# viscom-ulm/MCCNN

Hardware: AMD Instinct MI355X
Metric: MC-convolved points/sec (fwd+bwd), 100k-pt cloud r=0.1 (higher is better)
Workload: dtype f32; 1 GPU; ScanNet-like non-uniform room, 100000 pts/room, 1 room(s) on rank 0, absolute radius 0.1, KDE window 0.2, same-level conv 1to64 (Fin=1, Fout=64, combin), avg on; points_total=100000, points_per_gpu=100000, edges_per_gpu=4543198, layer=1to64, parallelism=cloud-per-GPU dp1, headline_mode=pipelined, rccl_world_size=1, collectives_warmed_before_warmup=False

## Files before the change

include/mccnn.h:

```cpp
#ifndef MCCNN_H_
#define MCCNN_H_

#include <stddef.h>

#ifdef __cplusplus
extern "C" {
#endif

typedef void* mccnn_stream_t;

#define MCCNN_OK 0
#define MCCNN_E_BADARG (-1)
#define MCCNN_E_BATCHID (-2)
#define MCCNN_E_TOOLARGE (-3)
#define MCCNN_E_WORKSPACE (-4)
#define MCCNN_E_SHAPE (-5)

int mccnn_block_size(void);
int mccnn_abi_version(void);
const char* mccnn_arch(void);
const char* mccnn_error_string(int code);

int mccnn_check_batch_ids(const int* batch_ids, int n, int batch_size, int* bad_count_dev,
                          mccnn_stream_t stream);
// ... 183 lines not shown
                        int avg, const int* order, void* rec_edges, int rec_ready, int* start_t, int* perm_t,
                        int tlist_ready, void* plan_buffer, void* ws, size_t ws_bytes, mccnn_stream_t stream);

int mccnn_spatial_conv_fwd_rows(const float* sorted_pts, const void* sorted_feats,
                                const int* sorted_batch_ids, const float* pdfs, const float* samples,
                                const int* start_idx, const int* packed, const float* aabb_min,
                                const float* aabb_max, const float* w1, const float* b1, const float* w2,
                                const float* b2, const float* w3, const float* b3, int n, int m, int e,
                                int num_feats, int batch_size, float radius, int scale_inv, int avg,
                                int bf16, const int* plan_vrow, const int* plan_vcode,
                                const int* slice_off, const int* vpos_row, const void* plan_rec,
                                const int* plan_other, void* out, float* scratch, const int* feat_index,
                                mccnn_stream_t stream);
size_t mccnn_spatial_conv_bwd_rows_workspace_bytes(int n, int e, int num_feats);
int mccnn_spatial_conv_bwd_rows(const float* sorted_pts, const void* sorted_feats,
                                const int* sorted_batch_ids, const float* pdfs, const float* samples,
                                const int* start_idx, const int* packed, const float* aabb_min,
                                const float* aabb_max, const float* w1, const float* b1, const float* w2,
                                const float* b2, const float* w3, const float* b3, const void* out_grad,
                                int n, int m, int e, int num_feats, int batch_size, float radius,
                                int scale_inv, int avg, int bf16, const int* start_t,
                                const int* plan_vrow, const int* plan_vcode, const int* slice_off,
                                const int* vpos_row, const void* plan_rec, const int* plan_other,
                                void* feat_grad, float* scratch, float* dw1, float* db1, float* dw2,
                                float* db2, float* dw3, float* db3, const int* feat_index, void* ws,
                                size_t ws_bytes, mccnn_stream_t stream);

#define MCCNN_E_CAPACITY (-6)
typedef struct mccnn_geometry mccnn_geometry_t;
mccnn_geometry_t* mccnn_geometry_create(void);
void mccnn_geometry_destroy(mccnn_geometry_t* g);
size_t mccnn_geometry_bytes(int n, int m, int batch_size, int num_cells, int e_capacity, int with_grid);
int mccnn_geometry_build(mccnn_geometry_t* g, const float* pts, const int* batch_ids, int n, const float* centres,
                         const int* centre_batch_ids, int m, const float* aabb_min, const float* aabb_max,
                         int batch_size, int num_cells, float radius, int scale_inv, float window, int use_pdf,
                         int e_capacity, const mccnn_geometry_t* grid_from, void* buffer, size_t buffer_bytes,
                         int* total_host, mccnn_stream_t stream);

typedef struct mccnn_geometry_request {
    mccnn_geometry_t* geometry;
    const float* pts; const int* batch_ids; int n;
    const float* centres; const int* centre_batch_ids; int m;
    const float* aabb_min; const float* aabb_max;
    int batch_size, num_cells;
    float radius; int scale_inv; float window; int use_pdf; int e_capacity;
    const mccnn_geometry_t* grid_from;
    void* buffer; size_t buffer_bytes;
    int* total_host;
} mccnn_geometry_request;
int mccnn_geometry_build_batch(const mccnn_geometry_request* requests, int count, mccnn_stream_t stream);
int mccnn_geometry_edges(mccnn_geometry_t* g, int wait_us);
int mccnn_geometry_info(const mccnn_geometry_t* g, long long out[16]);
int mccnn_geometry_attach(mccnn_geometry_t* g, int what, void* buffer, size_t bytes);
int mccnn_geometry_piece_bytes(mccnn_geometry_t* g, int what, long long* bytes, long long* ws_bytes);
int mccnn_geometry_piece_bound(int n, int m, int e_cap, int what, long long* bytes, long long* ws_bytes);
int mccnn_geometry_prebuild(mccnn_geometry_t* g, int what, int avg, void* ws, size_t ws_bytes, mccnn_stream_t stream);

size_t mccnn_geometry_prebuild_batch_ws_bytes(mccnn_geometry_t* const* geoms, const int* what, int count);
int mccnn_geometry_prebuild_batch(mccnn_geometry_t* const* geoms, const int* what, int count, int avg, void* ws, size_t ws_bytes,
                                  mccnn_stream_t stream);
int mccnn_conv_prepare(mccnn_geometry_t* g, const void* feats, int num_in_feats, int num_out_feats, int combin, int bf16,
                       int backward, int flags, int* need_mask, long long need_bytes[4], long long* ws_bytes,
                       long long* saved_bytes, int* edges);
int mccnn_conv_forward(mccnn_geometry_t* g, const void* feats, int num_in_feats, int num_out_feats, int combin, int avg,
                       int bf16, int flags, const float* w1, const float* b1, const float* w2, const float* b2,
                       const float* w3, const float* b3, void* out, void* saved, size_t saved_bytes, void* ws,
                       size_t ws_bytes, mccnn_stream_t stream);
int mccnn_conv_backward(mccnn_geometry_t* g, const void* feats, const void* saved, size_t saved_bytes,
                        const void* out_grad, int num_in_feats, int num_out_feats, int combin, int avg, int bf16,
                        int flags, const float* w1, const float* b1, const float* w2, const float* b2, const float* w3,
                        const float* b3, void* feat_grad, float* dw1, float* db1, float* dw2, float* db2, float* dw3,
                        float* db3, void* ws, size_t ws_bytes, mccnn_stream_t stream);

int mccnn_debug_conv_impl(int mask);

long long mccnn_debug_launch_count(void);
long long mccnn_debug_wait_ns(void);
int mccnn_debug_wait_accounting(int on);
int mccnn_background_launches(int on);
int mccnn_debug_f1_x4_min_edges(int edges);
int mccnn_debug_small_kernels(int on);

#ifdef __cplusplus
}
#endif
#endif
```

mccnn_amd/MCConvBuilder.py:

```python
import math

import os
import sys
import time
import torch

from . import _env


_NATIVE = None
_HIPOPS = None


def _native_mod():
    global _NATIVE
    if _NATIVE is None:
        from . import native
        _NATIVE = native
    return _NATIVE


def _hip_ops_mod():
    global _HIPOPS
    if _HIPOPS is None:
# ... 281 lines not shown
            self.register_parameter(name, p)
        elif tuple(p.shape) != tuple(shape):
            raise RuntimeError("variable %s exists with shape %s, requested %s" % (name, tuple(p.shape), shape))
        return p

    def forward(self, *args, **kwargs):
        return self.create_convolution(*args, **kwargs)

    def _add_to_collection(self, name, p):
        lst = self.collections_.setdefault(name, [])
        seen = self.__dict__.setdefault("_collection_ids", {}).setdefault(name, set())
        if id(p) not in seen:
            seen.add(id(p))
            lst.append(p)

    def __compute_dic_keys__(self, inPointHierarchy, outPointHierarchy, inPointLevel, outPointLevel, convRadius,
                             KDEWindow, relativeRadius, usePDF):
        memo = self.__dict__.setdefault("_keyMemo", {})
        k = (inPointHierarchy.hierarchyName_, outPointHierarchy.hierarchyName_, inPointLevel, outPointLevel, convRadius, KDEWindow,
             relativeRadius, usePDF)
        try:
            hit = memo.get(k)
        except TypeError:
            hit, k = None, None
        if hit is not None:
            return hit
        keyGrid = inPointHierarchy.hierarchyName_ + '|' + str(inPointLevel) + '|' + str(convRadius) + '|' + \
            str(relativeRadius)
        keyNeighs = keyGrid + '|' + outPointHierarchy.hierarchyName_ + '|' + str(outPointLevel)
        keyPDF = keyNeighs + '|' + str(KDEWindow) + '|' + str(usePDF)
        if k is not None and len(memo) < 4096:
            memo[k] = (keyGrid, keyNeighs, keyPDF)
        return keyGrid, keyNeighs, keyPDF

    def reset(self):
        state = self.__dict__
        k = state.get("hostStepsAhead_", None)
        if k is not None and _cuda_ok():
            evs = state.setdefault("stepEvents_", [])
            evs.append(_record_event())
            del evs[:-8]
            if len(evs) > k:
                _M = _hip_ops_mod()
                t0 = time.perf_counter()
                evs[-(int(k) + 1)].synchronize()
                dt = time.perf_counter() - t0
                _M.HOST_WAIT_S[0] += dt
                _M.HOST_LAG_WAIT_S[0] += dt
        state["cacheGrids_"], state["cacheNeighs_"], state["cachePDFs_"] = {}, {}, {}
        if self.geoSeen_:
            plan = []
            for key, ent in self.geoSeen_.items():
                geo = self.cacheGeo_.get(key)
                plan.append(ent + ((geo.have & 7) if geo is not None else 0, key))
            state["geoPlan_"], state["geoSeen_"] = plan, {}
        state["cacheGeo_"], state["cacheGeoGrid_"] = {}, {}
        if self.prefetchedGeo_:
            self.__install_prefetched_geometries__()
        pf, state["prefetched_"] = self.prefetched_, None
        if pf is not None:
            grids, neighs, pdfs, event = pf
            main = torch.cuda.current_stream()
            main.wait_event(event)
            for kN, h in list(neighs.items()):
                if hasattr(h, "finalize"):
                    st, pk, pdf = h.finalize()
                    neighs[kN] = (st, pk)
                    pdfs[h.keyPDF] = pdf
            for d in (grids, neighs, pdfs):
                for v in d.values():
                    for t in (v if isinstance(v, tuple) else (v,)):
                        t.record_stream(main)
            self.cacheGrids_, self.cacheNeighs_, self.cachePDFs_ = grids, neighs, pdfs
        state["resetEvent_"] = _record_event() if (_SIDE_EVENTS[0] and _cuda_ok()) else None
        if pf is not None:
            for kN, (kG, kP, centres, mn, mx, B, radius, rel) in self.prefetchTransposed_.items():
                if kN in neighs and kG in grids and getattr(self.ops_, "_ops", 0) is None:
                    _hip_ops = _hip_ops_mod()
                    self.sideStream_.wait_event(self.resetEvent_)
                    g = grids[kG]
                    _hip_ops.prefetch_transposed(neighs[kN][1], g[0].shape[0], self.sideStream_)
                    if kP in pdfs:
                        _hip_ops.prefetch_rowplan(neighs[kN][1], True, self.sideStream_, g[0], g[1], pdfs[kP], centres,
                                                  neighs[kN][0], neighs[kN][1], mn, mx, g[0].shape[0], centres.shape[0],
                                                  neighs[kN][1].shape[0], B, radius, rel, self.useAVG_)
            self.prefetchTransposed_ = {}

    def prefetch_geometry(self, inPointHierarchy, inPointLevel, convRadius, outPointHierarchy=None, outPointLevel=None,
                          KDEWindow=None, relativeRadius=None, usePDF=None, transposed=False):
        currKDEWindow = self.KDEWindow_ if KDEWindow is None else KDEWindow
        currRelativeRadius = self.relativeRadius_ if relativeRadius is None else relativeRadius
        currUsePDF = self.usePDF_ if usePDF is None else usePDF
        outPH = inPointHierarchy if outPointHierarchy is None else outPointHierarchy
        outLevel = inPointLevel if outPointLevel is None else outPointLevel
        keyGrid, keyNeighs, keyPDF = self.__compute_dic_keys__(inPointHierarchy, outPH, inPointLevel, outLevel, convRadius,
                                                               currKDEWindow, currRelativeRadius, currUsePDF)
        pts, bids = inPointHierarchy.points_[inPointLevel], inPointHierarchy.batchIds_[inPointLevel]
        mn, mx, B = inPointHierarchy.aabbMin_, inPointHierarchy.aabbMax_, inPointHierarchy.batchSize_
        if not pts.is_cuda:
            return
        if self.__prefetch_native__(inPointHierarchy, inPointLevel, convRadius, outPH, outLevel, currKDEWindow,
                                    currRelativeRadius, currUsePDF, keyGrid, keyNeighs, keyPDF, transposed):
            return
        if self.sideStream_ is None:
            self.sideStream_ = torch.cuda.Stream(device=pts.device)
        _SIDE_EVENTS[0] = True
        pf = self.prefetched_
# ... 67 lines not shown
            event.record(side)
        self.prefetched_ = (grids, neighs, pdfs, event)

    def _trace(self, *rec):
        if self.opTrace_ is not None:
            self.opTrace_.append(rec)

    def __layer_variables__(self, convName, inNumFeatures, currNumOutFeatures, currMultiFeatureConv, dev):
        blockSize = self.ops_.get_block_size()
        numOutNeurons = inNumFeatures * currNumOutFeatures if currMultiFeatureConv else inNumFeatures
        numBlocks = int(numOutNeurons / blockSize)
        if numOutNeurons % blockSize != 0:
            numBlocks = numBlocks + 1
        zeros = lambda t: t.zero_()
        nn = blockSize * numBlocks
        weights = self._get_variable(convName + '_weights', (3, nn), dev, lambda t: _fan_avg_uniform_(t, 3, nn))
        self._add_to_collection(self.decayLossCollection_, weights)
        biases = self._get_variable(convName + '_biases', (nn,), dev, zeros)
        weights2v = self._get_variable(convName + '_weights2', (numBlocks, blockSize, blockSize), dev,
                                       lambda t: _fan_avg_uniform_(t, numBlocks * blockSize, numBlocks * blockSize))
        self._add_to_collection(self.decayLossCollection_, weights2v)
        biases2v = self._get_variable(convName + '_biases2', (numBlocks, blockSize), dev, zeros)
        weights3v = self._get_variable(convName + '_weights3', (numBlocks, blockSize, blockSize), dev,
                                       lambda t: _fan_avg_uniform_(t, numBlocks * blockSize, numBlocks * blockSize))
        self._add_to_collection(self.decayLossCollection_, weights3v)
        biases3v = self._get_variable(convName + '_biases3', (numBlocks, blockSize), dev, zeros)
        return weights, biases, weights2v, biases2v, weights3v, biases3v, nn

    def __prefetch_native__(self, inPH, inLevel, convRadius, outPH, outLevel, KDEWindow, relativeRadius, usePDF, keyGrid,
                            keyNeighs, keyPDF, transposed, fork=True, pieces=0):
        _native = _native_mod()
        _hip_ops = _hip_ops_mod()
        if not (self.native_ and self.fuseSort_ and getattr(self.ops_, "_ops", 0) is None and _native.side_streams_available()
                and int(_hip_ops.PDF_MODE) == 1 and self.prefetched_ is None
                and _env.debug("native_prefetch", True)):
            return False
        inPts, inBids = inPH.points_[inLevel], inPH.batchIds_[inLevel]
        centres, cBids = outPH.points_[outLevel], outPH.batchIds_[outLevel]
        if inPts.requires_grad or inPts.shape[0] == 0 or centres.shape[0] == 0:
            return False
        for t, dt in ((inPts, torch.float32), (centres, torch.float32), (inBids, torch.int32), (cBids, torch.int32)):
            if t.dtype != dt or not t.is_contiguous() or not t.is_cuda:
                return False
        want = 0 if not transposed else (1 if transposed == "list" else 2)
        if keyPDF in self.prefetchedGeo_:
            ent = self.prefetchedGeo_[keyPDF]
            self.prefetchedGeo_[keyPDF] = ent[:4] + (max(ent[4], want),)
            return True
        mn, mx, B = inPH.aabbMin_, inPH.aabbMax_, inPH.batchSize_
        nc = _hip_ops._num_cells(mn, mx, B, convRadius, relativeRadius)
        owners = self.__dict__.setdefault("prefetchedGridOwner_", {})
        owner = owners.get(keyGrid)
        k = len(self.prefetchedGeo_)
        geo = _native.build_geometry(inPts, inBids, centres, cBids, mn, mx, B, nc, convRadius, relativeRadius, KDEWindow,
                                     usePDF, owner, side=k, fork=fork, background=True,
                                     after=(inPH.prefetchFuture_ if inPH is outPH else None))
        geo.uses = 0
        if owner is None:
            owners[keyGrid] = geo
        if pieces:
            geo.prebuild_async(pieces, self.useAVG_)
        self.prefetchedGeo_[keyPDF] = (geo, keyGrid, keyNeighs, usePDF, want)
        return True

    def prefetch_step(self, pointHierarchy):
        started = 0
        name, levels = pointHierarchy.hierarchyName_, len(pointHierarchy.points_)
        pieces = _env.debug("plan_prefetch", True)
        _native = _native_mod()
        _native.begin_batch()
        try:
            started = self.__prefetch_step_entries__(pointHierarchy, name, levels, pieces)
        finally:
            _native.end_batch()
        return started

    def __prefetch_step_entries__(self, pointHierarchy, name, levels, pieces):
        started = 0
        for ent in self.geoPlan_:
            hname, inLevel, outLevel, radius, window, rel, usePDF, have = ent[:8]
            if hname != name or inLevel >= levels or outLevel >= levels:
                continue
            keyGrid, keyNeighs, keyPDF = self.__compute_dic_keys__(pointHierarchy, pointHierarchy, inLevel, outLevel, radius,
                                                                   window, rel, usePDF)
            if keyPDF in self.prefetchedGeo_:
                continue
            if self.__prefetch_native__(pointHierarchy, inLevel, radius, pointHierarchy, outLevel, window, rel, usePDF, keyGrid,
                                        keyNeighs, keyPDF, False, fork=(started == 0), pieces=(have if pieces else 0)):
                started += 1
        return started

    def __install_prefetched_geometries__(self):
        _native = _native_mod()
        parked, self.prefetchedGeo_ = self.prefetchedGeo_, {}
        self.__dict__["prefetchedGridOwner_"] = {}
        for keyPDF, (geo, keyGrid, keyNeighs, usePDF, transposed) in parked.items():
            geo.unverified = True
            self.cacheGeo_[keyPDF] = geo
            if geo.grid_owner is None:
                self.cacheGeoGrid_[keyGrid] = geo
                self.cacheGrids_[keyGrid] = _LazyEntry(geo, geo.grid)
            self.cacheNeighs_[keyNeighs] = _LazyEntry(geo, geo.neighbors)
            self.cachePDFs_[keyPDF] = _LazyEntry(geo, geo.pdfs)
            if transposed:
                geo.prebuild((_native.NEED_PLAN_FWD | _native.NEED_PLAN_TR) if transposed == 2 else _native.NEED_TLIST,
                             self.useAVG_, 0, geo.buf)

    def __prebuild_geometries__(self, ph):
        _native = _native_mod()
        _hip_ops = _hip_ops_mod()
        plan, name = self.geoPlan_, ph.hierarchyName_
        levels = len(ph.points_)
        mn, mx, B = ph.aabbMin_, ph.aabbMax_, ph.batchSize_
        if int(_hip_ops.PDF_MODE) != 1:
            return
        k = 0
        pieces = _env.debug("plan_prefetch", True)
        for (hname, inLevel, outLevel, radius, window, rel, usePDF, have, _key) in plan:
            if hname != name or inLevel >= levels or outLevel >= levels:
                continue
            keyGrid, keyNeighs, keyPDF = self.__compute_dic_keys__(ph, ph, inLevel, outLevel, radius, window, rel, usePDF)
            if keyPDF in self.cacheGeo_:
                continue
            inPts, inBids = ph.points_[inLevel], ph.batchIds_[inLevel]
            centres, cBids = ph.points_[outLevel], ph.batchIds_[outLevel]
            if inPts.shape[0] == 0 or centres.shape[0] == 0 or inPts.requires_grad:
                continue
            ok = True
            for t, dt in ((inPts, torch.float32), (centres, torch.float32), (inBids, torch.int32), (cBids, torch.int32)):
                if t.dtype != dt or not t.is_contiguous() or not t.is_cuda:
                    ok = False
            if not ok:
                continue
            nc = _hip_ops._num_cells(mn, mx, B, radius, rel)
            owner = self.cacheGeoGrid_.get(keyGrid)
            geo = _native.build_geometry(inPts, inBids, centres, cBids, mn, mx, B, nc, radius, rel, window, usePDF, owner,
                                         side=k, fork=(k == 0), after=ph.prefetchFuture_)
            k += 1
            geo.uses = 0
            if have and pieces and geo.e_cap <= _PLAN_PREFETCH_MAX_E:
                geo.prebuild_async(have, self.useAVG_)
            self.cacheGeo_[keyPDF] = geo
            if owner is None:
                self.cacheGeoGrid_[keyGrid] = geo
                self.cacheGrids_[keyGrid] = _LazyEntry(geo, geo.grid)
                self._trace("sort_points_step1", keyGrid)
                self._trace("sort_points_step2", keyGrid)
            self.cacheNeighs_[keyNeighs] = _LazyEntry(geo, geo.neighbors)
            self.cachePDFs_[keyPDF] = _LazyEntry(geo, geo.pdfs)
            self._trace("find_neighbors", keyNeighs)
            if usePDF:
                self._trace("compute_pdf", keyPDF)

    def __native_convolution__(self, convName, inPH, inLevel, inFeatures, inNumFeatures, convRadius, outPH, outLevel,
                               multiFeatureConv, numOutFeatures, KDEWindow, relativeRadius, usePDF, useAVG, keyGrid,
                               keyNeighs, keyPDF):
        _native = _native_mod()
        _hip_ops = _hip_ops_mod()
        if (not self.cacheGeo_ and self.geoPrefetch_ and len(self.geoPlan_) >= _GEO_PREFETCH_MIN and inPH is outPH and self.prefetched_ is None
                and not self.cacheGrids_ and _native.side_streams_available()):
            self.__prebuild_geometries__(inPH)
        geo = self.cacheGeo_.get(keyPDF)
        if geo is not None and getattr(geo, "unverified", False):
            a = geo.args
            cen = outPH.points_[outLevel]
            pin = inPH.points_[inLevel]
            if (a[0] is pin or (a[0].data_ptr() == pin.data_ptr() and a[0].shape == pin.shape)) and \
                    (a[2] is cen or (a[2].data_ptr() == cen.data_ptr() and a[2].shape == cen.shape)):
                geo.unverified = False
            else:
                if _GEO_TRACE:
                    print("native conv %s: parked geometry %s not for this hierarchy (built from %s / %s, asked %s / %s)" % (
                        convName, keyPDF, tuple(a[0].shape), tuple(a[2].shape), tuple(pin.shape), tuple(cen.shape)), file=sys.stderr)
                self.cacheGeo_.pop(keyPDF, None)
                self.cachePDFs_.pop(keyPDF, None)
                self.cacheNeighs_.pop(keyNeighs, None)
                if self.cacheGeoGrid_.get(keyGrid) is geo:
                    self.cacheGeoGrid_.pop(keyGrid, None)
                    self.cacheGrids_.pop(keyGrid, None)
                geo = None
        if geo is None:
            if keyGrid in self.cacheGrids_ and keyGrid not in self.cacheGeoGrid_:
                if _GEO_TRACE:
                    print("native conv %s: grid %s owned by the op path" % (convName, keyGrid), file=sys.stderr)
                return None
            if keyNeighs in self.cacheNeighs_ or keyPDF in self.cachePDFs_:
                if _GEO_TRACE:
                    print("native conv %s: list %s / pdf %s cached without a geometry (%s %s); geometries: %s" % (
                        convName, keyNeighs, keyPDF, keyNeighs in self.cacheNeighs_, keyPDF in self.cachePDFs_,
                        sorted(self.cacheGeo_)), file=sys.stderr)
# ... 194 lines not shown
```

mccnn_amd/_lib.py:

```python
import ctypes as C
import os

import torch

_PKG = os.path.dirname(os.path.abspath(__file__))
LIB_PATH = os.path.join(_PKG, "lib", os.environ.get("MCCNN_LIB_NAME", "libmccnn_hip.so"))

_vp, _i, _f, _sz = C.c_void_p, C.c_int, C.c_float, C.c_size_t

SIGNATURES = {
    "mccnn_block_size": (_i, []),
    "mccnn_abi_version": (_i, []),
    "mccnn_arch": (C.c_char_p, []),
    "mccnn_error_string": (C.c_char_p, [_i]),
    "mccnn_check_batch_ids": (_i, [_vp, _i, _i, _vp, _vp]),
    "mccnn_debug_conv_impl": (_i, [_i]),
    "mccnn_debug_launch_count": (C.c_longlong, []),
    "mccnn_debug_wait_ns": (C.c_longlong, []),
    "mccnn_debug_wait_accounting": (_i, [_i]),
    "mccnn_debug_small_kernels": (_i, [_i]),
    "mccnn_debug_f1_x4_min_edges": (_i, [_i]),
    "mccnn_background_launches": (_i, [_i]),
    "mccnn_compute_aabb_workspace_bytes": (_sz, [_i]),
    "mccnn_compute_aabb": (_i, [_vp, _vp, _i, _i, _i, _vp, _vp, _vp, _sz, _vp]),
# ... 15 lines not shown
    "mccnn_transform_indexs_dn": (_i, [_vp, _i, _vp, _vp, _i, _vp, _vp, _vp, _sz, _vp]),
    "mccnn_permute_gather": (_i, [_vp, _vp, _i, _i, _vp, _vp]),
    "mccnn_permute_scatter": (_i, [_vp, _vp, _i, _i, _vp, _i, _i, _vp]),
    "mccnn_transform_indexs_workspace_bytes": (_sz, [_i]),
    "mccnn_transform_indexs": (_i, [_vp, _i, _vp, _i, _vp, _vp, _sz, _vp]),
    "mccnn_find_neighbors_workspace_bytes": (_sz, [_i, _i]),
    "mccnn_find_neighbors_count": (_i, [_vp, _vp, _i, _vp, _i, _vp, _vp, _vp, _i, _i, _f, _i, _vp, _vp, _vp, _vp, _sz, _vp]),
    "mccnn_find_neighbors_count2": (_i, [_vp, _vp, _i, _vp, _i, _vp, _vp, _vp, _i, _i, _f, _i, _vp, _vp, _vp, _vp, _vp, _sz, _vp]),
    "mccnn_find_neighbors_fill": (_i, [_vp, _vp, _i, _vp, _i, _vp, _vp, _vp, _i, _i, _f, _i, _vp, _vp, _i, _vp, _vp, _sz, _vp]),
    "mccnn_invert_permutation": (_i, [_vp, _i, _vp, _vp]),
    "mccnn_compute_pdf_workspace_bytes": (_sz, [_i, _i]),
    "mccnn_compute_pdf": (_i, [_vp, _vp, _vp, _i, _vp, _i, _vp, _vp, _i, _f, _f, _i, _i, _vp, _vp, _sz, _vp]),
    "mccnn_compute_pdf_dn": (_i, [_vp, _vp, _vp, _i, _vp, _i, _vp, _vp, _vp, _i, _f, _f, _i, _vp, _vp, _sz, _vp]),
    "mccnn_poisson_sampling_workspace_bytes": (_sz, [_i, _i, _i]),
    "mccnn_poisson_sampling_count": (_i, [_vp, _vp, _i, _vp, _vp, _vp, _i, _i, _f, _i, _i, _vp, _vp, _sz, _vp]),
    "mccnn_poisson_sampling_fill": (_i, [_vp, _i, _vp, _i, _i, _i, _vp, _vp, _vp, _vp, _sz, _vp]),
    "mccnn_spatial_conv_fwd_workspace_bytes": (_sz, [_i, _i, _i, _i, _i]),
    "mccnn_spatial_conv_state_bytes": (_sz, [_i, _i, _i, _i, _i]),
    "mccnn_spatial_conv_fwd": (_i, [_vp] * 15 + [_i, _i, _i, _i, _i, _i, _i, _f, _i, _i, _vp, _vp, _vp, _sz, _vp]),
    "mccnn_spatial_conv_bwd_workspace_bytes": (_sz, [_i, _i, _i, _i, _i, _i]),
    "mccnn_spatial_conv_bwd": (_i, [_vp] * 16 + [_i, _i, _i, _i, _i, _i, _i, _f, _i, _i] + [_vp] * 10 + [_vp, _sz, _vp]),
    "mccnn_spatial_conv_fwd_bf16": (_i, [_vp] * 15 + [_i, _i, _i, _i, _i, _f, _i, _i, _vp, _vp, _sz, _vp]),
    "mccnn_spatial_conv_bwd_bf16": (_i, [_vp] * 16 + [_i, _i, _i, _i, _i, _f, _i, _i] + [_vp] * 9 + [_vp, _sz, _vp]),
    "mccnn_rowplan_sizes": (_i, [_i, _i, C.POINTER(_i), C.POINTER(C.c_longlong), C.POINTER(C.c_longlong)]),
    "mccnn_rowplan_workspace_bytes": (_sz, [_i, _i]),
    "mccnn_rowplan_layout": (_i, [_vp, _i, _i, _vp, _vp, _vp, _vp, _vp, _vp, _sz, _vp]),
    "mccnn_edge_records": (_i, [_vp] * 8 + [_i, _i, _i, _i, _f, _i, _i, _vp, _vp]),
    "mccnn_rowplan_fill": (_i, [_i, _vp, _vp, _i, _i] + [_vp] * 6 + [_vp, _vp, _vp]),
    "mccnn_rowplan_buffer": (_i, [_i, _i, C.POINTER(C.c_longlong), C.POINTER(C.c_longlong), C.POINTER(_i),
                                  C.POINTER(C.c_longlong), C.POINTER(C.c_longlong)]),
    "mccnn_rowplan_build_workspace_bytes": (_sz, [_i, _i, _i]),
    "mccnn_rowplan_bound": (_i, [_i, _i, _i, C.POINTER(C.c_longlong), C.POINTER(C.c_longlong)]),
    "mccnn_rowplan_inline_records": (_i, [_i, _i]),
    "mccnn_rowplan_build": (_i, [_i] + [_vp] * 8 + [_i, _i, _i, _i, _f, _i, _i, _vp, _vp, _i, _vp, _vp, _i, _vp, _vp, _sz, _vp]),
    "mccnn_spatial_conv_fwd_rows": (_i, [_vp] * 15 + [_i, _i, _i, _i, _i, _f, _i, _i, _i] + [_vp] * 6 + [_vp, _vp, _vp, _vp]),
    "mccnn_spatial_conv_bwd_rows_workspace_bytes": (_sz, [_i, _i, _i]),
    "mccnn_spatial_conv_bwd_rows": (_i, [_vp] * 16 + [_i, _i, _i, _i, _i, _f, _i, _i, _i] + [_vp] * 7 + [_vp] * 8 + [_vp, _vp, _sz, _vp]),
    "mccnn_transpose_neighbors_workspace_bytes": (_sz, [_i, _i]),
    "mccnn_transpose_neighbors": (_i, [_vp, _i, _i, _vp, _vp, _vp, _sz, _vp]),
    "mccnn_spatial_conv_bwd_points_workspace_bytes": (_sz, [_i, _i]),
    "mccnn_spatial_conv_bwd_points": (_i, [_vp, _vp, _i] + [_vp] * 14 + [_i, _i, _i, _i, _i, _i, _i, _f, _i, _i]
                                      + [_vp] * 5 + [_sz, _vp]),
    "mccnn_compute_pdf_bwd_points_workspace_bytes": (_sz, [_i, _i]),
    "mccnn_compute_pdf_bwd_points": (_i, [_vp, _vp, _vp, _i, _vp, _i, _vp, _vp, _i, _f, _f, _i, _vp, _i, _vp, _vp, _vp, _sz,
                                          _vp]),
    "mccnn_edge_grad_reduce": (_i, [_vp, _vp, _vp, _i, _i, _vp, _vp]),
    "mccnn_geometry_create": (_vp, []),
    "mccnn_geometry_destroy": (None, [_vp]),
    "mccnn_geometry_bytes": (_sz, [_i, _i, _i, _i, _i, _i]),
    "mccnn_geometry_build": (_i, [_vp, _vp, _vp, _i, _vp, _vp, _i, _vp, _vp, _i, _i, _f, _i, _f, _i, _i, _vp, _vp, _sz, _vp, _vp]),
    "mccnn_geometry_edges": (_i, [_vp, _i]),
    "mccnn_geometry_info": (_i, [_vp, C.POINTER(C.c_longlong)]),
    "mccnn_geometry_attach": (_i, [_vp, _i, _vp, _sz]),
    "mccnn_geometry_piece_bytes": (_i, [_vp, _i, C.POINTER(C.c_longlong), C.POINTER(C.c_longlong)]),
    "mccnn_geometry_piece_bound": (_i, [_i, _i, _i, _i, C.POINTER(C.c_longlong), C.POINTER(C.c_longlong)]),
    "mccnn_geometry_prebuild": (_i, [_vp, _i, _i, _vp, _sz, _vp]),
    "mccnn_conv_prepare": (_i, [_vp, _vp, _i, _i, _i, _i, _i, _i, C.POINTER(_i), C.POINTER(C.c_longlong),
                                C.POINTER(C.c_longlong), C.POINTER(C.c_longlong), C.POINTER(_i)]),
    "mccnn_conv_forward": (_i, [_vp, _vp, _i, _i, _i, _i, _i, _i] + [_vp] * 6 + [_vp, _vp, _sz, _vp, _sz, _vp]),
    "mccnn_conv_backward": (_i, [_vp, _vp, _vp, _sz, _vp, _i, _i, _i, _i, _i, _i] + [_vp] * 6 + [_vp] * 7 + [_vp, _sz, _vp]),
}


class MCCNNError(RuntimeError):
    """Raised for any non-zero return code of the C-ABI (the reference raised
    errors::InvalidArgument for shape errors and exit()ed on CUDA errors)."""


_lib = None


def load():
    global _lib
    if _lib is not None:
        return _lib
    if not os.path.exists(LIB_PATH):
        raise MCCNNError(
            "libmccnn_hip.so not found at %s -- build it with `python -m mccnn_amd.build` "
            "(there is no CPU / PyTorch fallback for the MC-convolution ops)" % LIB_PATH)
    mode = C.RTLD_GLOBAL if os.environ.get("MCCNN_LIB_NAME") else C.DEFAULT_MODE
    lib = C.CDLL(LIB_PATH, mode=mode)
    for name, (res, args) in SIGNATURES.items():
        fn = getattr(lib, name)
        fn.restype = res
        fn.argtypes = args
    _lib = lib
    return lib


def check(rc, what):
    if rc != 0:
        msg = load().mccnn_error_string(rc).decode()
        raise MCCNNError("%s failed: %s (code %d)" % (what, msg, rc))


def ptr(t):
    return None if t is None else t.data_ptr()


_raw_stream = getattr(torch._C, "_cuda_getCurrentRawStream", None)
_cur_device = getattr(torch._C, "_cuda_getDevice", None)


def stream_handle():
    if _raw_stream is not None and _cur_device is not None:
        return _raw_stream(_cur_device())
# ... 2 lines not shown
```

mccnn_amd/csrc/conv.hip:

```cpp
#include "conv_mfma.h"
#include "batch.h"
#include <cstdlib>
#include <type_traits>

namespace mccnn {

__device__ __forceinline__ float relu(float x) { return fmaxf(x, 0.0f); }
__device__ __forceinline__ float wave_sum(float v) {
#pragma unroll
    for (int d = 32; d >= 1; d >>= 1) v += __shfl_xor(v, d, 64);
    return v;
}

struct EdgeCtx {
    int j, i;
    float d0, d1, d2, inv;
};

__device__ __forceinline__ EdgeCtx load_edge(const ConvArgs& a, int t) {
    EdgeCtx c;
    int2 pr = a.packed[t];
    c.j = pr.x;
    c.i = pr.y;
    int b = clamp_batch(a.bids[c.j], a.B);
// ... 985 lines not shown

std::atomic<int>& conv_impl_override() {
    static std::atomic<int> v{(debug_int("force_valu", 0) ? 1 : 0) | (debug_int("no_f1", 0) ? 2 : 0)};
    return v;
}

bool transpose_small(int e, int n) {
    return e <= MCCNN_TR_SMALL_E && n <= MCCNN_TR_SMALL_N && (long long)e * e / n <= (1LL << 20) && small_kernels_on();
}
size_t transpose_count_bytes(int n) { return align_up((size_t)n * 4) + scan_workspace_bytes(n); }
int transpose_count(const int2* pk, int e, int n, int* start_t, char* blk, int* slot, hipStream_t s) {
    const size_t cntBytes = align_up((size_t)n * 4);
    int* cnt = (int*)blk;
    {
        int rc = launch_clear_spans(clear_span(blk, cntBytes + scan_status_bytes(n)), no_span(), no_span(), s);
        if (rc) return rc;
    }
    if (n <= MCCNN_TR_LDS_BINS && e >= 4 * n) tr_count_lds<<<ceil_div(e, 256), 256, 0, s>>>(pk, e, n, cnt, slot);
    else tr_count<<<ceil_div(e, 256), 256, 0, s>>>(pk, e, cnt, slot);
    MCCNN_LAUNCHED();
    return exclusive_scan_i32(cnt, start_t, n, start_t + n, blk + cntBytes, s, true);
}
int transpose_fill(const int2* pk, int e, const int* start_t, const int* slot, int* tmp, hipStream_t s) {
    tr_fill<<<ceil_div(e, 256), 256, 0, s>>>(pk, e, start_t, slot, tmp);
    MCCNN_LAUNCHED();
    return 0;
}

}

using namespace mccnn;

template <bool TR>
static int launch_conv_stream(const ConvArgs& a, bool combin, bool vec, bool bf16, float* out, const float4* rec,
                              const int* permT, hipStream_t s, float4* recOut = nullptr) {
    typedef void (*Kern)(ConvArgs, float*, int, const float4*, const int*, float4*);
    Kern fn;
    if (bf16) fn = TR ? conv_stream<false, 4, true> : conv_stream<false, 4, false>;
    else if (TR) fn = vec ? conv_stream<false, 2, true> : conv_stream<false, 0, true>;
    else if (combin) fn = (a.Fin == 1) ? conv_stream<true, 1, false> : (a.Fin <= 4 ? conv_stream<true, 3, false> : conv_stream<true, 0, false>);
    else fn = vec ? conv_stream<false, 2, false> : conv_stream<false, 0, false>;
    const size_t lds = ((size_t)a.nb * MCCNN_WQ_FWD + 4 * (size_t)a.nb * 8) * sizeof(float);
    const int numCU = num_cus();
    const int perCU = cached_blocks_per_cu(reinterpret_cast<const void*>(fn), lds);
    const long long chunks = ((long long)a.e + 63) / 64;
    long long W = (long long)numCU * perCU * 4;
    if (W > (chunks + 1) / 2) W = (chunks + 1) / 2;
    if (W < 1) W = 1;
    fn<<<(int)((W + 3) / 4), 256, lds, s>>>(a, out, (int)W, rec, permT, recOut);
    MCCNN_LAUNCHED();
    return 0;
}

extern "C" {

int mccnn_debug_conv_impl(int mask) { return conv_impl_override().exchange(mask & 3); }

static bool f1_shape(int num_in_feats, int num_out_feats, int combin) {
    return combin && num_in_feats == 1 && num_out_feats > 0 && (num_out_feats + 7) / 8 <= MCCNN_LDS_MAX_NB &&
           (conv_impl_override().load(std::memory_order_relaxed) & 3) == 0;
}

static size_t state_record_bytes(int e) { return align_up((size_t)(e > 0 ? e : 0) * sizeof(float4)); }
size_t mccnn_spatial_conv_state_bytes(int m, int e, int num_in_feats, int num_out_feats, int combin) {
    if (m <= 0 || e <= 0 || num_in_feats <= 0 || num_out_feats <= 0) return 0;
    if (f1_shape(num_in_feats, num_out_feats, combin)) return state_record_bytes(e) + f1_state_bytes(m, (num_out_feats + 7) / 8);
    const long long neurons = combin ? (long long)num_in_feats * num_out_feats : num_in_feats;
    const bool mfma = (!combin || (neurons + 7) / 8 <= MCCNN_LDS_MAX_NB) && (conv_impl_override().load(std::memory_order_relaxed) & 1) == 0;
    return mfma ? state_record_bytes(e) : 0;
}

size_t mccnn_spatial_conv_fwd_workspace_bytes(int m, int e, int num_in_feats, int num_out_feats, int combin) {
    (void)e;
    if (m > 0 && f1_shape(num_in_feats, num_out_feats, combin)) return f1_fwd_workspace_bytes(m, (num_out_feats + 7) / 8);
    return 256;
}

static bool use_mfma(const ConvArgs& a, bool combin) {
    return (a.nb <= MCCNN_LDS_MAX_NB || !combin) && (conv_impl_override().load(std::memory_order_relaxed) & 1) == 0;
}
#define MCCNN_TILE_FWD 64
#define MCCNN_TILE_BWD 48
static void tile_split(int nb, int maxTile, int& tiles, int& per) {
    tiles = (nb + maxTile - 1) / maxTile;
    per = (nb + tiles - 1) / tiles;
}
static ConvArgs tile_args(const ConvArgs& a, int q0, int nbT, size_t elem) {
    ConvArgs t = a;
    t.feats = reinterpret_cast<const float*>(reinterpret_cast<const char*>(a.feats) + (size_t)q0 * 8 * elem);
    t.w1 = a.w1 + (size_t)q0 * 24; t.b1 = a.b1 + (size_t)q0 * 8;
    t.w2 = a.w2 + (size_t)q0 * 64; t.b2 = a.b2 + (size_t)q0 * 8;
    t.w3 = a.w3 + (size_t)q0 * 64; t.b3 = a.b3 + (size_t)q0 * 8;
    t.nb = nbT;
    t.neuronsOut = a.neuronsOut - q0 * 8 < nbT * 8 ? a.neuronsOut - q0 * 8 : nbT * 8;
    return t;
}
static float* col_offset(float* p, int q0, size_t elem) { return reinterpret_cast<float*>(reinterpret_cast<char*>(p) + (size_t)q0 * 8 * elem); }
static const float* col_offset_c(const float* p, int q0, size_t elem) { return col_offset(const_cast<float*>(p), q0, elem); }

static bool bf16_shape_ok(const ConvArgs& a, int combin, const void* p0, const void* p1) {
    return !combin && a.Fin % 8 == 0 && ((((uintptr_t)p0 | (uintptr_t)p1) & 15) == 0) &&
           (conv_impl_override().load(std::memory_order_relaxed) & 1) == 0;
}

static int conv_fwd_impl(const float* sorted_pts, const float* sorted_feats, const int* sorted_batch_ids,
                         const float* pdfs, const float* samples, const int* start_idx, const int* packed,
                         const float* aabb_min, const float* aabb_max, const float* w1, const float* b1,
                         const float* w2, const float* b2, const float* w3, const float* b3, int n, int m, int e,
                         int num_in_feats, int num_out_feats, int combin, int batch_size, float radius,
                         int scale_inv, int avg, float* out, void* state, void* ws, size_t ws_bytes,
                         mccnn_stream_t stream, int bf16) {
    ConvArgs a;
    int rc = fill_args(a, sorted_pts, sorted_feats, sorted_batch_ids, pdfs, samples, start_idx, packed, aabb_min,
                       aabb_max, w1, b1, w2, b2, w3, b3, n, m, e, num_in_feats, num_out_feats, combin, batch_size,
                       radius, scale_inv, avg);
    if (rc) return rc;
    if (m == 0) return 0;
    if (!out) return MCCNN_E_BADARG;
    hipStream_t s = (hipStream_t)stream;
    bool vec = !combin && (a.Fin % 8 == 0) && ((((uintptr_t)sorted_feats) & 15) == 0);
    if (bf16 && !bf16_shape_ok(a, combin, sorted_feats, out)) return MCCNN_E_SHAPE;
    float4* recOut = state ? reinterpret_cast<float4*>(state) : nullptr;
    if (e > 0 && f1_shape(num_in_feats, num_out_feats, combin))
        return f1_forward(a, out, recOut, state ? (char*)state + state_record_bytes(e) : nullptr, ws, ws_bytes, s);
    if (use_mfma(a, combin != 0) && e > 0) {
        if (combin || a.nb <= MCCNN_TILE_FWD) return launch_conv_stream<false>(a, combin != 0, vec, bf16 != 0, out, nullptr, nullptr, s, recOut);
        int tiles, per;
        tile_split(a.nb, MCCNN_TILE_FWD, tiles, per);
        const size_t elem = bf16 ? 2 : sizeof(float);
        for (int q0 = 0; q0 < a.nb; q0 += per) {
            const ConvArgs t = tile_args(a, q0, a.nb - q0 < per ? a.nb - q0 : per, elem);
            int rc2 = launch_conv_stream<false>(t, false, vec, bf16 != 0, col_offset(out, q0, elem), nullptr, nullptr, s,
                                                q0 == 0 ? recOut : nullptr);
            if (rc2) return rc2;
        }
        return 0;
    }
    if (e == 0) {
        return launch_zero_words(out, (size_t)m * a.outF * (bf16 ? 2 : sizeof(float)) / 4, s);
    }
    int G = 2048 / a.outF;
    if (G > 32) G = 32;
    if (G < 1) G = 1;
    a.G = G;
    size_t lds = (size_t)4 * G * a.outF * sizeof(float);
    if (lds > 64 * 1024) return MCCNN_E_TOOLARGE;
    int blocks = ceil_div(m, 4 * G);
    if (combin) {
        if (a.Fin == 1) conv_fwd_valu<true, 1><<<blocks, 256, lds, s>>>(a, out);
        else conv_fwd_valu<true, 0><<<blocks, 256, lds, s>>>(a, out);
    } else {
        if (vec) conv_fwd_valu<false, 2><<<blocks, 256, lds, s>>>(a, out);
        else conv_fwd_valu<false, 0><<<blocks, 256, lds, s>>>(a, out);
    }
    MCCNN_LAUNCHED();
    return 0;
}

int mccnn_spatial_conv_fwd(const float* sorted_pts, const float* sorted_feats, const int* sorted_batch_ids,
                           const float* pdfs, const float* samples, const int* start_idx, const int* packed,
                           const float* aabb_min, const float* aabb_max, const float* w1, const float* b1,
                           const float* w2, const float* b2, const float* w3, const float* b3, int n, int m, int e,
                           int num_in_feats, int num_out_feats, int combin, int batch_size, float radius,
                           int scale_inv, int avg, float* out, void* state, void* ws, size_t ws_bytes,
                           mccnn_stream_t stream) {
    return conv_fwd_impl(sorted_pts, sorted_feats, sorted_batch_ids, pdfs, samples, start_idx, packed, aabb_min, aabb_max,
                         w1, b1, w2, b2, w3, b3, n, m, e, num_in_feats, num_out_feats, combin, batch_size, radius, scale_inv,
                         avg, out, state, ws, ws_bytes, stream, 0);
}

int mccnn_spatial_conv_fwd_bf16(const float* sorted_pts, const void* sorted_feats_bf16, const int* sorted_batch_ids,
                                const float* pdfs, const float* samples, const int* start_idx, const int* packed,
                                const float* aabb_min, const float* aabb_max, const float* w1, const float* b1,
                                const float* w2, const float* b2, const float* w3, const float* b3, int n, int m, int e,
                                int num_feats, int batch_size, float radius, int scale_inv, int avg, void* out_bf16,
                                void* ws, size_t ws_bytes, mccnn_stream_t stream) {
    return conv_fwd_impl(sorted_pts, (const float*)sorted_feats_bf16, sorted_batch_ids, pdfs, samples, start_idx, packed,
// ... 27 lines not shown
int mccnn_transpose_neighbors(const int* packed, int e, int n, int* start_t, int* perm_t, void* ws, size_t ws_bytes,
                              mccnn_stream_t stream) {
    if (e < 0 || n < 0 || !start_t) return MCCNN_E_BADARG;
    hipStream_t s = (hipStream_t)stream;
    if (e == 0 || n == 0) {
        return launch_zero_words(start_t, (size_t)n + 1, s);
    }
    if (!packed || !perm_t) return MCCNN_E_BADARG;
    if (!ws || ws_bytes < mccnn_transpose_neighbors_workspace_bytes(n, e)) return MCCNN_E_WORKSPACE;
    Arena ar(ws, ws_bytes);
    const size_t cntBytes = align_up((size_t)n * 4);
    char* blk = ar.take<char>(cntBytes + scan_workspace_bytes(n));
    int* slot = ar.take<int>((size_t)e);
    int* tmp = ar.take<int>((size_t)e);
    if (!blk || !slot || !tmp) return MCCNN_E_WORKSPACE;
    int* cnt = (int*)blk;
    const int2* pk = reinterpret_cast<const int2*>(packed);
    if (transpose_small(e, n)) {
        tr_small<<<1, 1024, 0, s>>>(pk, e, n, cnt, slot, tmp, start_t, perm_t);
        MCCNN_LAUNCHED();
        return 0;
    }
    int rc = transpose_count(pk, e, n, start_t, blk, slot, s);
    if (rc) return rc;
    rc = transpose_fill(pk, e, start_t, slot, tmp, s);
    if (rc) return rc;
    tr_rank<<<ceil_div(e, 256), 256, 0, s>>>(pk, e, start_t, tmp, perm_t);
    MCCNN_LAUNCHED();
    return 0;
}

size_t mccnn_spatial_conv_bwd_workspace_bytes(int n, int m, int e, int num_in_feats, int num_out_feats, int combin) {
    if (e <= 0 || num_in_feats <= 0 || num_out_feats <= 0) return 256;
    long long neurons = combin ? (long long)num_in_feats * num_out_feats : num_in_feats;
    long long nb = (neurons + 7) / 8;
    if (m > 0 && f1_shape(num_in_feats, num_out_feats, combin)) return f1_bwd_workspace_bytes(m, e, (int)nb);
    int cpw, waves;
    bwd_partition(e, cpw, waves);
    size_t bytes = align_up((size_t)(((long long)waves + 3) / 4 * 4 * nb * 176) * sizeof(float));
    bytes += align_up((size_t)e * sizeof(float4));
    if (combin) bytes += align_up((size_t)e * num_in_feats * df_planes(num_in_feats, (int)nb) * sizeof(float));
    else bytes += align_up((size_t)(n + 1) * 4) + align_up((size_t)e * 4) +
                  mccnn_transpose_neighbors_workspace_bytes(n, e);
    return bytes + 256;
}

static int conv_bwd_impl(const float* sorted_pts, const float* sorted_feats, const int* sorted_batch_ids,
                         const float* pdfs, const float* samples, const int* start_idx, const int* packed,
                         const float* aabb_min, const float* aabb_max, const float* w1, const float* b1,
                         const float* w2, const float* b2, const float* w3, const float* b3, const float* out_grad,
                         int n, int m, int e, int num_in_feats, int num_out_feats, int combin, int batch_size,
                         float radius, int scale_inv, int avg, const void* state, const int* start_t,
                         const int* perm_t, float* feat_grad, float* dw1, float* db1, float* dw2, float* db2, float* dw3, float* db3,
                         void* ws, size_t ws_bytes, mccnn_stream_t stream, int bf16) {
    ConvArgs a;
    int rc = fill_args(a, sorted_pts, sorted_feats, sorted_batch_ids, pdfs, samples, start_idx, packed, aabb_min,
                       aabb_max, w1, b1, w2, b2, w3, b3, n, m, e, num_in_feats, num_out_feats, combin, batch_size,
                       radius, scale_inv, avg);
    if (rc) return rc;
    if (!dw1 || !db1 || !dw2 || !db2 || !dw3 || !db3 || (n > 0 && !feat_grad)) return MCCNN_E_BADARG;
    hipStream_t s = (hipStream_t)stream;
    size_t nn = (size_t)a.nb * 8;
    bool vec = !combin && (a.Fin % 8 == 0) && ((((uintptr_t)sorted_feats | (uintptr_t)out_grad) & 15) == 0);
    int tilesB = 1, perB = a.nb;
    if (!combin) tile_split(a.nb, MCCNN_TILE_BWD, tilesB, perB);
    size_t lds = ((size_t)perB * MCCNN_WQ_BWD + 4 * 192) * sizeof(float);
    bool mfma = use_mfma(a, combin != 0) && lds <= 64 * 1024 && m > 0 && e > 0;
    if (bf16 && (!bf16_shape_ok(a, combin, sorted_feats, out_grad) || (((uintptr_t)feat_grad) & 15))) return MCCNN_E_SHAPE;
    bool dfeatT = mfma && !combin;
    const bool f1Clears = mfma && m > 0 && e > 0 && f1_shape(num_in_feats, num_out_feats, combin);
    const bool gatherT = mfma && combin && a.Fin >= 2 && a.Fin <= 4 && start_t && perm_t && m > 0 && e > 0;
    const size_t fgBytes = (size_t)n * a.Fin * (bf16 ? 2 : sizeof(float));
    ClearSpan fgSpan = no_span();
    if (n > 0 && !dfeatT && !f1Clears && !gatherT) {
        const bool scatterPath = mfma && m > 0 && e > 0 && combin && a.Fin > 1;
        if (scatterPath && (((uintptr_t)feat_grad) & 15) == 0 && fgBytes % 16 == 0) {
            fgSpan = clear_span(feat_grad, fgBytes);
        } else {
            int rc = launch_zero_words(feat_grad, fgBytes / 4, s);
            if (rc) return rc;
        }
    }
    if (!mfma || m == 0 || e == 0) {
        float* gp[6] = {dw1, db1, dw2, db2, dw3, db3};
        const size_t gn[6] = {3 * nn, nn, 8 * nn, nn, 8 * nn, nn};
        for (int k = 0; k < 6; ++k) {
            int rc = launch_zero_words(gp[k], gn[k], s);
            if (rc) return rc;
        }
    }
    if (m == 0 || e == 0) return 0;
    if (!out_grad) return MCCNN_E_BADARG;
    const float4* recIn = state ? reinterpret_cast<const float4*>(state) : nullptr;
    if (mfma && f1_shape(num_in_feats, num_out_feats, combin))
        return f1_backward(a, out_grad, recIn, state ? (const char*)state + state_record_bytes(e) : nullptr, feat_grad, dw1, db1,
                           dw2, db2, dw3, db3, ws, ws_bytes, s);
    if (mfma) {
        if (!ws || ws_bytes < mccnn_spatial_conv_bwd_workspace_bytes(n, m, e, num_in_feats, num_out_feats, combin))
            return MCCNN_E_WORKSPACE;
        int cpw, waves;
        bwd_partition(e, cpw, waves);
        int blocks = (waves + 3) / 4;
        Arena ar(ws, ws_bytes);
        float* partials = ar.take<float>((size_t)blocks * 4 * a.nb * 176);
        float4* rec = ar.take<float4>((size_t)e);
        float* dfE = combin ? ar.take<float>((size_t)e * a.Fin * df_planes(a.Fin, a.nb)) : nullptr;
        if (!partials || !rec || (combin && !dfE)) return MCCNN_E_WORKSPACE;
        a.G = 0;
        if (recIn) {
            rec = const_cast<float4*>(recIn);
        } else {
            edge_records<<<ceil_div(e, 256), 256, 0, s>>>(a, rec);
            MCCNN_LAUNCHED();
        }
        const size_t elem = bf16 ? 2 : sizeof(float);
        for (int q0 = 0; q0 < a.nb; q0 += perB) {
            const int nbT = a.nb - q0 < perB ? a.nb - q0 : perB;
            const ConvArgs t = combin ? a : tile_args(a, q0, nbT, elem);
            const float* og = combin ? out_grad : col_offset_c(out_grad, q0, elem);
            const size_t ldsT = ((size_t)nbT * MCCNN_WQ_BWD + 4 * 192) * sizeof(float);
            const bool coop = !combin && nbT >= 4;
            const int rows = coop ? blocks : waves;
            if (combin) {
                if (a.Fin == 1) conv_bwd_mfma<true, 1, false><<<blocks, 256, ldsT, s>>>(t, rec, og, feat_grad, dfE, cpw, partials);
                else if (a.Fin <= 4) conv_bwd_mfma<true, 3, false><<<blocks, 256, ldsT, s>>>(t, rec, og, feat_grad, dfE, cpw, partials);
                else conv_bwd_mfma<true, 0, false><<<blocks, 256, ldsT, s>>>(t, rec, og, feat_grad, dfE, cpw, partials);
            } else if (bf16) {
                if (coop) conv_bwd_mfma<false, 4, true><<<blocks, 256, ldsT, s>>>(t, rec, og, feat_grad, dfE, cpw, partials);
                else conv_bwd_mfma<false, 4, false><<<blocks, 256, ldsT, s>>>(t, rec, og, feat_grad, dfE, cpw, partials);
            } else if (coop) {
                if (vec) conv_bwd_mfma<false, 2, true><<<blocks, 256, ldsT, s>>>(t, rec, og, feat_grad, dfE, cpw, partials);
                else conv_bwd_mfma<false, 0, true><<<blocks, 256, ldsT, s>>>(t, rec, og, feat_grad, dfE, cpw, partials);
            } else {
                if (vec) conv_bwd_mfma<false, 2, false><<<blocks, 256, ldsT, s>>>(t, rec, og, feat_grad, dfE, cpw, partials);
                else conv_bwd_mfma<false, 0, false><<<blocks, 256, ldsT, s>>>(t, rec, og, feat_grad, dfE, cpw, partials);
            }
            MCCNN_LAUNCHED();
            reduce_partials<<<ceil_div((long long)nbT * 176, 16), 1024, 0, s>>>(
                partials, rows, nbT, dw1 + (size_t)q0 * 24, db1 + (size_t)q0 * 8, dw2 + (size_t)q0 * 64, db2 + (size_t)q0 * 8,
                dw3 + (size_t)q0 * 64, db3 + (size_t)q0 * 8, q0 == 0 ? fgSpan : no_span());
            MCCNN_LAUNCHED();
        }
        if (combin && a.Fin > 1) {
            long long total = (long long)e * a.Fin;
            const int planes = df_planes(a.Fin, a.nb);
            if (start_t && perm_t && a.Fin <= 4) {
                const int gblocks = ceil_div((long long)n * 16, 256);
                if (a.Fin == 2) gather_edge_featgrad<2><<<gblocks, 256, 0, s>>>(start_t, perm_t, dfE, total, planes, n, e, feat_grad);
                else if (a.Fin == 3) gather_edge_featgrad<3><<<gblocks, 256, 0, s>>>(start_t, perm_t, dfE, total, planes, n, e, feat_grad);
// ... 18 lines not shown
            bool vecD = (a.Fin % 8 == 0) && ((((uintptr_t)out_grad) & 15) == 0);
            int tilesF, perF;
            tile_split(a.nb, MCCNN_TILE_FWD, tilesF, perF);
            for (int q0 = 0; q0 < a.nb; q0 += perF) {
                ConvArgs t = a;
                t.feats = out_grad;
                t = tile_args(t, q0, a.nb - q0 < perF ? a.nb - q0 : perF, elem);
                t.start = start_t;
                t.m = n;
                int rc3 = launch_conv_stream<true>(t, false, vecD, bf16 != 0, col_offset(feat_grad, q0, elem), rec, perm_t, s);
                if (rc3) return rc3;
            }
        } else {
            return MCCNN_E_TOOLARGE;
        }
        return 0;
    }
    a.G = 32;
    int blocks = ceil_div(m, 4 * a.G);
    if (combin) conv_bwd_valu<true><<<blocks, 256, 0, s>>>(a, out_grad, feat_grad, dw1, db1, dw2, db2, dw3, db3);
    else conv_bwd_valu<false><<<blocks, 256, 0, s>>>(a, out_grad, feat_grad, dw1, db1, dw2, db2, dw3, db3);
    MCCNN_LAUNCHED();
    return 0;
}

int mccnn_spatial_conv_bwd(const float* sorted_pts, const float* sorted_feats, const int* sorted_batch_ids,
                           const float* pdfs, const float* samples, const int* start_idx, const int* packed,
                           const float* aabb_min, const float* aabb_max, const float* w1, const float* b1,
                           const float* w2, const float* b2, const float* w3, const float* b3, const float* out_grad,
                           int n, int m, int e, int num_in_feats, int num_out_feats, int combin, int batch_size,
                           float radius, int scale_inv, int avg, const void* state, const int* start_t,
                           const int* perm_t, float* feat_grad, float* dw1, float* db1, float* dw2, float* db2, float* dw3, float* db3,
                           void* ws, size_t ws_bytes, mccnn_stream_t stream) {
    return conv_bwd_impl(sorted_pts, sorted_feats, sorted_batch_ids, pdfs, samples, start_idx, packed, aabb_min, aabb_max,
                         w1, b1, w2, b2, w3, b3, out_grad, n, m, e, num_in_feats, num_out_feats, combin, batch_size, radius,
                         scale_inv, avg, state, start_t, perm_t, feat_grad, dw1, db1, dw2, db2, dw3, db3, ws, ws_bytes, stream, 0);
}

int mccnn_spatial_conv_bwd_bf16(const float* sorted_pts, const void* sorted_feats_bf16, const int* sorted_batch_ids,
                                const float* pdfs, const float* samples, const int* start_idx, const int* packed,
                                const float* aabb_min, const float* aabb_max, const float* w1, const float* b1,
                                const float* w2, const float* b2, const float* w3, const float* b3,
                                const void* out_grad_bf16, int n, int m, int e, int num_feats, int batch_size, float radius,
                                int scale_inv, int avg, const int* start_t, const int* perm_t, void* feat_grad_bf16,
                                float* dw1, float* db1, float* dw2, float* db2, float* dw3, float* db3, void* ws,
                                size_t ws_bytes, mccnn_stream_t stream) {
    return conv_bwd_impl(sorted_pts, (const float*)sorted_feats_bf16, sorted_batch_ids, pdfs, samples, start_idx, packed,
                         aabb_min, aabb_max, w1, b1, w2, b2, w3, b3, (const float*)out_grad_bf16, n, m, e, num_feats, num_feats,
                         0, batch_size, radius, scale_inv, avg, nullptr, start_t, perm_t, (float*)feat_grad_bf16, dw1, db1,
                         dw2, db2, dw3, db3, ws, ws_bytes, stream, 1);
}

}
```

mccnn_amd/csrc/conv_f1.hip:

```cpp
#include "conv_mfma.h"

namespace mccnn {

__device__ __forceinline__ float wave_seg_scan1(float v, float m1, float m2, float m4, float m8, float mA, float mB) {
    asm("s_nop 1\n"
        "v_fmac_f32_dpp %0, %0, %1 row_shr:1 row_mask:0xf bank_mask:0xf bound_ctrl:1\n s_nop 1\n"
        "v_fmac_f32_dpp %0, %0, %2 row_shr:2 row_mask:0xf bank_mask:0xf bound_ctrl:1\n s_nop 1\n"
        "v_fmac_f32_dpp %0, %0, %3 row_shr:4 row_mask:0xf bank_mask:0xf bound_ctrl:1\n s_nop 1\n"
        "v_fmac_f32_dpp %0, %0, %4 row_shr:8 row_mask:0xf bank_mask:0xf bound_ctrl:1\n s_nop 1\n"
        "v_fmac_f32_dpp %0, %0, %5 row_bcast:15 row_mask:0xa bank_mask:0xf\n s_nop 1\n"
        "v_fmac_f32_dpp %0, %0, %6 row_bcast:31 row_mask:0xc bank_mask:0xf\n s_nop 1\n"
        : "+v"(v)
        : "v"(m1), "v"(m2), "v"(m4), "v"(m8), "v"(mA), "v"(mB));
    return v;
}

__global__ __launch_bounds__(256) void f1_fwd_edges(ConvArgs a, float* __restrict__ A, float* __restrict__ S,
                                                    int numWaves, float4* __restrict__ recOut) {
    extern __shared__ float lds[];
    const int wave = threadIdx.x >> 6, lane = threadIdx.x & 63, i4 = lane & 3;
    const int rowA = a.nb * 8;
    float* wl = lds;
    float* carry = lds + a.nb * MCCNN_WQ_FWD + (size_t)wave * rowA;
    stage_weights<MCCNN_WQ_FWD>(a, wl);
    __syncthreads();
    const int w = blockIdx.x * 4 + wave;
    if (w >= numWaves) return;
    const int tA = (int)(((long long)a.e * w) / numWaves);
    const int tB = (int)(((long long)a.e * (w + 1)) / numWaves);
    const int cA = (w == 0) ? 0 : wave_lower_bound(a.start, a.m, a.e, tA, lane);
    const int cB = (w == numWaves - 1) ? a.m : wave_lower_bound(a.start, a.m, a.e, tB, lane);
    if (cA >= cB) return;
    const int eBeg = a.start[cA];
    const int eEnd = (cB < a.m) ? a.start[cB] : a.e;

    auto zero_rows = [&](int c0, int c1) {
        for (int c = c0; c < c1; ++c) {
            for (int f = 0; f < rowA; ++f) A[(size_t)c * rowA + f] = 0.0f;
            S[c] = 0.0f;
        }
    };

    int keyLast = cA;
    int carryKey = -1;
    float carryS = 0.f;
    int2 prN = make_int2(0, cA);
    float pdfN = 1.0f;
    if (eBeg + lane < eEnd) { prN = a.packed[eBeg + lane]; pdfN = a.pdfs[eBeg + lane]; }
    for (int base = eBeg; base < eEnd; base += 64) {
        const int t = base + lane;
        const int nIn = min(64, eEnd - base);
        const bool in = lane < nIn;
        const int2 pr = prN;
        const float pdf = pdfN;
        if (t + 64 < eEnd) { prN = a.packed[t + 64]; pdfN = a.pdfs[t + 64]; }
        const int ci = pr.y, j = pr.x;
        float invR = a.invRadius;
        if (a.scaleInv) invR = 1.0f / (a.radius * max_extent(a.mn, a.mx, clamp_batch(a.bids[j], a.B)));
        const float* pp = a.pts + (size_t)j * 3;
        const float* cc = a.samples + (size_t)ci * 3;
        const float R = a.scaleInv ? a.radius * max_extent(a.mn, a.mx, clamp_batch(a.bids[j], a.B)) : a.radius;
        const float d0 = div_exact(pp[0] - cc[0], R, invR), d1 = div_exact(pp[1] - cc[1], R, invR), d2 = div_exact(pp[2] - cc[2], R, invR);
        float K = 1.0f;
        if (a.avg) K = (float)(((ci + 1 < a.m) ? a.start[ci + 1] : a.e) - a.start[ci]);
        const float inv = in ? __builtin_amdgcn_rcpf(pdf * K) : 0.0f;
        const float s = in ? a.feats[j] * inv : 0.0f;
        if (recOut && in) recOut[t] = make_float4(d0, d1, d2, inv);
        const int key = in ? ci + 1 : 0;
        const int cLast = __builtin_amdgcn_readlane(ci, nIn - 1);
        const int rowEnd = (cLast + 1 < a.m) ? a.start[cLast + 1] : a.e;
        const bool cont = rowEnd > base + 64;
        int keyPrev = __shfl_up(key, 1, 64);
        if (lane == 0) keyPrev = keyLast;
        int keyNext = __shfl_down(key, 1, 64);
        const bool tail = in && ((lane == nIn - 1) ? !cont : (key != keyNext));
        if (in && key - keyPrev > 1) zero_rows(keyPrev, ci);
        const float m1 = (key != 0 && dpp_i<DPP_ROW_SHR(1)>(key) == key) ? 1.f : 0.f;
        const float m2 = (key != 0 && dpp_i<DPP_ROW_SHR(2)>(key) == key) ? 1.f : 0.f;
        const float m4 = (key != 0 && dpp_i<DPP_ROW_SHR(4)>(key) == key) ? 1.f : 0.f;
        const float m8 = (key != 0 && dpp_i<DPP_ROW_SHR(8)>(key) == key) ? 1.f : 0.f;
        const float mA = (key != 0 && dpp_rows_i<DPP_ROW_BCAST15, 0xA>(key) == key) ? 1.f : 0.f;
        const float mB = (key != 0 && dpp_rows_i<DPP_ROW_BCAST31, 0xC>(key) == key) ? 1.f : 0.f;
        const bool haveCarry = carryKey >= 0;
        const float mC = (haveCarry && key == carryKey) ? 1.f : 0.f;

        float sv = wave_seg_scan1(s, m1, m2, m4, m8, mA, mB);
        sv = fmaf(mC, carryS, sv);
        if (tail) S[ci] = sv;
        carryS = __shfl(sv, 63, 64);
        float* arow = A + (size_t)ci * rowA;

        for (int q = 0; q < a.nb; ++q) {
            float pre1[8], a1[8], pre2[8], a2[8], c[8];
            MCCNN_PHASE();
            mlp_block_l12(wl + q * MCCNN_WQ_FWD, i4, d0, d1, d2, pre1, a1, pre2, a2);
#pragma unroll
            for (int k = 0; k < 8; ++k) c[k] = s * a2[k];
            float* cq = carry + q * 8;
            f32x4 cv0 = {0.f, 0.f, 0.f, 0.f}, cv1 = cv0;
            if (haveCarry) { cv0 = *reinterpret_cast<f32x4*>(cq); cv1 = *reinterpret_cast<f32x4*>(cq + 4); }
            wave_seg_scan8(c, m1, m2, m4, m8, mA, mB);
#pragma unroll
            for (int k = 0; k < 8; ++k) c[k] = fmaf(mC, k < 4 ? cv0[k & 3] : cv1[k & 3], c[k]);
            if (cont && lane == 63) {
                *reinterpret_cast<f32x4*>(cq) = (f32x4){c[0], c[1], c[2], c[3]};
                *reinterpret_cast<f32x4*>(cq + 4) = (f32x4){c[4], c[5], c[6], c[7]};
            }
            if (tail) {
                float4* dst = reinterpret_cast<float4*>(arow + q * 8);
                dst[0] = make_float4(c[0], c[1], c[2], c[3]);
                dst[1] = make_float4(c[4], c[5], c[6], c[7]);
            }
        }
        carryKey = cont ? cLast + 1 : -1;
        keyLast = cLast + 1;
    }
    if (lane == 0) zero_rows(keyLast, cB);
}

#define DPP_WAVE_SHR1 0x138
#define DPP_WAVE_SHL1 0x130
struct L12Regs {
    f32x4 w1lo, w1hi;
    float w2lo[8], w2hi[8], b2lo, b2hi;
};
__device__ __forceinline__ void load_l12(const float* __restrict__ wq, int i4, L12Regs& w) {
    const f32x4* w4 = reinterpret_cast<const f32x4*>(wq);
    w.w1lo = w4[i4];
    w.w1hi = w4[4 + i4];
    const f32x4 a0 = w4[10 + 2 * i4], a1 = w4[10 + 2 * i4 + 1], b0 = w4[10 + 2 * (4 + i4)], b1 = w4[10 + 2 * (4 + i4) + 1];
    w.w2lo[0] = a0.x; w.w2lo[1] = a0.y; w.w2lo[2] = a0.z; w.w2lo[3] = a0.w; w.w2lo[4] = a1.x; w.w2lo[5] = a1.y; w.w2lo[6] = a1.z; w.w2lo[7] = a1.w;
    w.w2hi[0] = b0.x; w.w2hi[1] = b0.y; w.w2hi[2] = b0.z; w.w2hi[3] = b0.w; w.w2hi[4] = b1.x; w.w2hi[5] = b1.y; w.w2hi[6] = b1.z; w.w2hi[7] = b1.w;
    w.b2lo = wq[104 + i4];
    w.b2hi = wq[104 + 4 + i4];
}

#ifndef MCCNN_F1_X4_OCC
#define MCCNN_F1_X4_OCC 1
#endif
#ifndef MCCNN_F1_X4_GROUP
#define MCCNN_F1_X4_GROUP 4
#endif
#ifdef MCCNN_F1_X4_NOPHASE
#define X4_PHASE()
#else
#define X4_PHASE() MCCNN_PHASE()
#endif
__global__ __launch_bounds__(256, MCCNN_F1_X4_OCC) void f1_fwd_edges4(ConvArgs a, float* __restrict__ A, float* __restrict__ S,
                                                     int numWaves, float4* __restrict__ recOut) {
    extern __shared__ float lds[];
    const int wave = threadIdx.x >> 6, lane = threadIdx.x & 63, i4 = lane & 3;
    const int rowA = a.nb * 8;
    float* wl = lds;
    float* carry = lds + a.nb * MCCNN_WQ_FWD + (size_t)wave * rowA;
    float4* recStage = reinterpret_cast<float4*>(lds + a.nb * MCCNN_WQ_FWD + 4 * (size_t)rowA) + (size_t)wave * 256;
    stage_weights<MCCNN_WQ_FWD>(a, wl);
    __syncthreads();
    const int w = blockIdx.x * 4 + wave;
    if (w >= numWaves) return;
    const int tA = (int)(((long long)a.e * w) / numWaves);
    const int tB = (int)(((long long)a.e * (w + 1)) / numWaves);
    const int cA = (w == 0) ? 0 : wave_lower_bound(a.start, a.m, a.e, tA, lane);
    const int cB = (w == numWaves - 1) ? a.m : wave_lower_bound(a.start, a.m, a.e, tB, lane);
    if (cA >= cB) return;
    const int eBeg = a.start[cA];
    const int eEnd = (cB < a.m) ? a.start[cB] : a.e;

    auto zero_rows = [&](int c0, int c1) {
        for (int c = c0; c < c1; ++c) {
            for (int f = 0; f < rowA; ++f) A[(size_t)c * rowA + f] = 0.0f;
            S[c] = 0.0f;
        }
    };

    int keyLast = cA;
    int carryKey = -1;
    float carryS = 0.f;
    int2 prN[4];
    float pdfN[4];
#pragma unroll
    for (int u = 0; u < 4; ++u) {
        const int t = min(eBeg + 4 * lane + u, a.e - 1);
        prN[u] = a.packed[t];
        pdfN[u] = a.pdfs[t];
    }
    for (int base = eBeg; base < eEnd; base += 256) {
        const int lastPos = min(base + 256, eEnd) - 1;
        float d0[4], d1[4], d2[4], sE[4];
        int key[4], ci[4];
        bool in[4];
#pragma unroll
        for (int u = 0; u < 4; ++u) {
            const int t = base + 4 * lane + u;
            in[u] = t < eEnd;
            const int2 pr = prN[u];
            const float pdf = pdfN[u];
            const int j = pr.x;
            ci[u] = pr.y;
            float invR = a.invRadius, R = a.radius;
            if (a.scaleInv) {
                R = a.radius * max_extent(a.mn, a.mx, clamp_batch(a.bids[j], a.B));
                invR = 1.0f / R;
            }
            const float* pp = a.pts + (size_t)j * 3;
            const float* cc = a.samples + (size_t)pr.y * 3;
            d0[u] = div_exact(pp[0] - cc[0], R, invR);
            d1[u] = div_exact(pp[1] - cc[1], R, invR);
            d2[u] = div_exact(pp[2] - cc[2], R, invR);
            float K = 1.0f;
            if (a.avg) K = (float)(((pr.y + 1 < a.m) ? a.start[pr.y + 1] : a.e) - a.start[pr.y]);
            const float inv = in[u] ? __builtin_amdgcn_rcpf(pdf * K) : 0.0f;
            sE[u] = in[u] ? a.feats[j] * inv : 0.0f;
            if (recOut) recStage[4 * lane + u] = make_float4(d0[u], d1[u], d2[u], inv);
            key[u] = in[u] ? pr.y + 1 : 0;
        }
        if (recOut) {
#pragma unroll
            for (int k = 0; k < 4; ++k) {
                const int t = base + 64 * k + lane;
                if (t < eEnd) recOut[t] = recStage[64 * k + lane];
            }
        }
        if (base + 256 < eEnd) {
#pragma unroll
            for (int u = 0; u < 4; ++u) {
                const int t = min(base + 256 + 4 * lane + u, a.e - 1);
                prN[u] = a.packed[t];
                pdfN[u] = a.pdfs[t];
            }
        }
        const int lp = lastPos - base;
        const int lu = lp & 3;
        const int kSel = (lu == 0) ? key[0] : (lu == 1) ? key[1] : (lu == 2) ? key[2] : key[3];
        const int keyEnd = __builtin_amdgcn_readlane(kSel, lp >> 2);
        const int rowEnd = (keyEnd < a.m) ? a.start[keyEnd] : a.e;
        const bool cont = rowEnd > lastPos + 1;
        const int kPrev = __builtin_amdgcn_update_dpp(keyLast, key[3], DPP_WAVE_SHR1, 0xf, 0xf, false);
        const int kNext = __builtin_amdgcn_update_dpp(0, key[0], DPP_WAVE_SHL1, 0xf, 0xf, true);
        const bool haveCarry = carryKey >= 0;
        float nh[4], op[4];
        bool tail[4];
#pragma unroll
        for (int u = 0; u < 4; ++u) {
            const int kp = (u == 0) ? kPrev : key[u - 1];
            const int kn = (u == 3) ? kNext : key[u + 1];
            if (in[u] && key[u] - kp > 1) zero_rows(kp, ci[u]);
            nh[u] = (key[u] != 0 && key[u] == kp) ? 1.f : 0.f;
            op[u] = (key[u] != 0 && key[u] == kPrev && lane != 0) ? 1.f : 0.f;
            const int t = base + 4 * lane + u;
            tail[u] = in[u] && ((t == lastPos) ? !cont : (key[u] != kn));
        }
        const int k3 = key[3];
        const float m1 = (k3 != 0 && dpp_i<DPP_ROW_SHR(1)>(k3) == k3) ? 1.f : 0.f;
        const float m2 = (k3 != 0 && dpp_i<DPP_ROW_SHR(2)>(k3) == k3) ? 1.f : 0.f;
        const float m4 = (k3 != 0 && dpp_i<DPP_ROW_SHR(4)>(k3) == k3) ? 1.f : 0.f;
        const float m8 = (k3 != 0 && dpp_i<DPP_ROW_SHR(8)>(k3) == k3) ? 1.f : 0.f;
        const float mA = (k3 != 0 && dpp_rows_i<DPP_ROW_BCAST15, 0xA>(k3) == k3) ? 1.f : 0.f;
        const float mB = (k3 != 0 && dpp_rows_i<DPP_ROW_BCAST31, 0xC>(k3) == k3) ? 1.f : 0.f;
        const float mC = (haveCarry && lane == 0) ? 1.f : 0.f;

        {
            float r0 = fmaf(mC, carryS, sE[0]);
            float r1 = fmaf(r0, nh[1], sE[1]);
            float r2 = fmaf(r1, nh[2], sE[2]);
            float r3 = fmaf(r2, nh[3], sE[3]);
            r3 = wave_seg_scan1(r3, m1, m2, m4, m8, mA, mB);
            const float cin = __builtin_bit_cast(float, __builtin_amdgcn_update_dpp(0, __builtin_bit_cast(int, r3), DPP_WAVE_SHR1, 0xf, 0xf, true));
            r0 = fmaf(op[0], cin, r0);
            r1 = fmaf(op[1], cin, r1);
            r2 = fmaf(op[2], cin, r2);
            if (tail[0]) S[ci[0]] = r0;
            if (tail[1]) S[ci[1]] = r1;
            if (tail[2]) S[ci[2]] = r2;
            if (tail[3]) S[ci[3]] = r3;
            carryS = __shfl(r3, 63, 64);
        }

        for (int q = 0; q < a.nb; ++q) {
            L12Regs wr;
            load_l12(wl + q * MCCNN_WQ_FWD, i4, wr);
            float c[4][8];
// ... 343 lines not shown
        int w = sl;
        for (; w + 192 < rows; w += 256) {
            s0 += src[(size_t)w * stride];
            s1 += src[(size_t)(w + 64) * stride];
            s2 += src[(size_t)(w + 128) * stride];
            s3 += src[(size_t)(w + 192) * stride];
        }
        for (; w < rows; w += 64) s0 += src[(size_t)w * stride];
    }
    acc[sl][kk] = (s0 + s1) + (s2 + s3);
    __syncthreads();
    if (sl == 0 && k < K) {
        float v = 0.f;
#pragma unroll
        for (int i = 0; i < 64; ++i) v += acc[i][kk];
        if (r < 24) dw1[q * 24 + r] = v;
        else if (r < 32) db1[q * 8 + r - 24] = v;
        else if (r < 96) dw2[q * 64 + r - 32] = v;
        else if (r < 104) db2[q * 8 + r - 96] = v;
        else if (r < 168) dw3[q * 64 + r - 104] = v;
        else db3[q * 8 + r - 168] = v;
    }
}

static void f1_bwd_partition(int e, int& cpw, int& waves) {
    const long long chunks = ((long long)e + 63) / 64;
    const long long resident = (long long)num_cus() * 4 * MCCNN_F1_OCC;
    cpw = (int)((chunks + resident - 1) / resident);
    if (cpw > 48) {
        const long long rounds = (cpw + 31) / 32;
        cpw = (int)((chunks + resident * rounds - 1) / (resident * rounds));
    }
    static const int minChunks = debug_int("bwd_min_chunks", 2);
    if (cpw < minChunks) cpw = minChunks < 1 ? 1 : minChunks;
    waves = (int)((chunks + cpw - 1) / cpw);
    if (waves < 1) waves = 1;
}
#ifndef MCCNN_F1_CENTRE_WAVES
#define MCCNN_F1_CENTRE_WAVES 1024
#endif
static void f1_centre_partition(int m, int& cPerWave, int& waves) {
    cPerWave = (m + MCCNN_F1_CENTRE_WAVES - 1) / MCCNN_F1_CENTRE_WAVES;
    cPerWave = (cPerWave + 63) / 64 * 64;
    waves = (m + cPerWave - 1) / cPerWave;
}

size_t f1_state_bytes(int m, int nb) { return align_up((size_t)m * nb * 8 * sizeof(float)) + align_up((size_t)m * sizeof(float)); }

static void f1_state_split(void* state, int m, int nb, float*& A, float*& S) {
    A = (float*)state;
    S = (float*)((char*)state + align_up((size_t)m * nb * 8 * sizeof(float)));
}

static int f1_run_edges(const ConvArgs& a, float* A, float* S, float4* recOut, hipStream_t s) {
    const size_t lds = ((size_t)a.nb * MCCNN_WQ_FWD + 4 * (size_t)a.nb * 8) * sizeof(float);
    if (a.e >= g_f1_x4_min_edges.load(std::memory_order_relaxed)) {
        const size_t lds4 = lds + 4 * 256 * sizeof(float4);
        const int perCU4 = cached_blocks_per_cu(reinterpret_cast<const void*>(f1_fwd_edges4), lds4);
        const long long iters = ((long long)a.e + 255) / 256;
        static const int wpc = debug_int("f1_x4_waves_per_cu", 0);
        long long W4 = (long long)num_cus() * (wpc > 0 ? wpc : perCU4 * 4);
        if (W4 > (iters + 1) / 2) W4 = (iters + 1) / 2;
        if (W4 < 1) W4 = 1;
        f1_fwd_edges4<<<(int)((W4 + 3) / 4), 256, lds4, s>>>(a, A, S, (int)W4, recOut);
        MCCNN_LAUNCHED();
        return 0;
    }
    const int perCU = cached_blocks_per_cu(reinterpret_cast<const void*>(f1_fwd_edges), lds);
    const long long chunks = ((long long)a.e + 63) / 64;
    long long W = (long long)num_cus() * perCU * 4;
    if (W > (chunks + 1) / 2) W = (chunks + 1) / 2;
    if (W < 1) W = 1;
    f1_fwd_edges<<<(int)((W + 3) / 4), 256, lds, s>>>(a, A, S, (int)W, recOut);
    MCCNN_LAUNCHED();
    return 0;
}

size_t f1_fwd_workspace_bytes(int m, int nb) { return f1_state_bytes(m, nb) + 256; }

int f1_forward(const ConvArgs& a, float* out, float4* rec_out, void* state, void* ws, size_t ws_bytes, hipStream_t s) {
    if (!state) {
        if (!ws || ws_bytes < f1_fwd_workspace_bytes(a.m, a.nb)) return MCCNN_E_WORKSPACE;
        state = ws;
    }
    float *A, *S;
    f1_state_split(state, a.m, a.nb, A, S);
    int rc = f1_run_edges(a, A, S, rec_out, s);
    if (rc) return rc;
    f1_fwd_centres<<<ceil_div((long long)a.m * a.nb, 256), 256, (size_t)a.nb * 72 * sizeof(float), s>>>(a, A, S, out);
    MCCNN_LAUNCHED();
    return 0;
}

size_t f1_bwd_workspace_bytes(int m, int e, int nb) {
    int cpw, wavesE, cpwC, wavesC;
    f1_bwd_partition(e, cpw, wavesE);
    f1_centre_partition(m, cpwC, wavesC);
    size_t b = f1_state_bytes(m, nb);
    b += align_up((size_t)m * nb * 8 * sizeof(float)) + align_up((size_t)m * sizeof(float));
    b += align_up((size_t)e * sizeof(float4)) + align_up((size_t)e * sizeof(float));
    b += align_up((size_t)(wavesE + 3) / 4 * 4 * nb * MCCNN_F1_ROW * sizeof(float));
    b += align_up((size_t)(wavesC + 3) / 4 * 4 * nb * MCCNN_F1_ROWC * sizeof(float));
    return b + 256;
}

int f1_backward(const ConvArgs& a, const float* out_grad, const float4* rec_in, const void* state, float* feat_grad, float* dw1, float* db1,
                float* dw2, float* db2, float* dw3, float* db3, void* ws, size_t ws_bytes, hipStream_t s) {
    if (!ws || ws_bytes < f1_bwd_workspace_bytes(a.m, a.e, a.nb)) return MCCNN_E_WORKSPACE;
    int cpw, wavesE, cPerWave, wavesC;
    f1_bwd_partition(a.e, cpw, wavesE);
    f1_centre_partition(a.m, cPerWave, wavesC);
    const int blocksE = (wavesE + 3) / 4, blocksC = (wavesC + 3) / 4;
    Arena ar(ws, ws_bytes);
    void* own = ar.take<char>(f1_state_bytes(a.m, a.nb));
    float* G = ar.take<float>((size_t)a.m * a.nb * 8);
    float* gb = ar.take<float>((size_t)a.m);
    float4* rec = ar.take<float4>((size_t)a.e);
    float* dfE = ar.take<float>((size_t)a.e);
    float* pe = ar.take<float>((size_t)blocksE * 4 * a.nb * MCCNN_F1_ROW);
    float* pc = ar.take<float>((size_t)blocksC * 4 * a.nb * MCCNN_F1_ROWC);
    if (!own || !G || !gb || !rec || !dfE || !pe || !pc) return MCCNN_E_WORKSPACE;
    float *A, *S;
    if (state) {
        f1_state_split(const_cast<void*>(state), a.m, a.nb, A, S);
    } else {
        f1_state_split(own, a.m, a.nb, A, S);
        int rc = f1_run_edges(a, A, S, nullptr, s);
        if (rc) return rc;
    }
    f1_bwd_centres<<<ceil_div((long long)wavesC * (a.nb + 1), 4), 256, 0, s>>>(a, out_grad, A, S, cPerWave, wavesC, G, gb, pc, feat_grad);
    MCCNN_LAUNCHED();
    const float4* recUse = rec;
    if (rec_in) {
        recUse = rec_in;
    } else {
        f1_edge_records<<<ceil_div(a.e, 256), 256, 0, s>>>(a, rec);
        MCCNN_LAUNCHED();
    }
    const size_t ldsE = (size_t)a.nb * MCCNN_WQ_BWD * sizeof(float);
    f1_bwd_edges<<<blocksE, 256, ldsE, s>>>(a, recUse, G, gb, feat_grad, dfE, cpw, pe);
    MCCNN_LAUNCHED();
    f1_reduce<<<ceil_div((long long)a.nb * 176, 16), 1024, 0, s>>>(pe, wavesE, pc, wavesC, a.nb, dw1, db1, dw2, db2, dw3, db3);
    MCCNN_LAUNCHED();
    return 0;
}

}
```

mccnn_amd/csrc/conv_mfma.h:

```cpp
#pragma once
#include "common.h"
#include <atomic>
#include <mutex>

namespace mccnn {

struct ConvArgs {
    const float* pts;
    const float* feats;
    const int* bids;
    const float* pdfs;
    const float* samples;
    const int* start;
    const int2* packed;
    const float* mn;
    const float* mx;
    const float *w1, *b1, *w2, *b2, *w3, *b3;
    int n, m, e, Fin, Fout, nb, neuronsOut, outF;
    float radius, invRadius;
    int scaleInv, avg, G, B;
};

#define MCCNN_LDS_MAX_NB 64
#define MCCNN_WQ_FWD 184
// ... 309 lines not shown

template <int FIN, int R0>
__device__ __forceinline__ void combin_fold_t(const float* g, const float* o, float* sf) {
#pragma unroll
    for (int n = 0; n < 8; ++n) sf[(R0 + n) % FIN] = fmaf(g[n], o[n], sf[(R0 + n) % FIN]);
}
__device__ __forceinline__ void combin_fold(int Fin, int r0, const float* g, const float* o, float* sf) {
    switch (Fin * 4 + r0) {
        case 2 * 4 + 0: combin_fold_t<2, 0>(g, o, sf); break;
        case 2 * 4 + 1: combin_fold_t<2, 1>(g, o, sf); break;
        case 3 * 4 + 0: combin_fold_t<3, 0>(g, o, sf); break;
        case 3 * 4 + 1: combin_fold_t<3, 1>(g, o, sf); break;
        case 3 * 4 + 2: combin_fold_t<3, 2>(g, o, sf); break;
        case 4 * 4 + 0: combin_fold_t<4, 0>(g, o, sf); break;
        case 4 * 4 + 1: combin_fold_t<4, 1>(g, o, sf); break;
        case 4 * 4 + 2: combin_fold_t<4, 2>(g, o, sf); break;
        default: combin_fold_t<4, 3>(g, o, sf); break;
    }
}

inline int cached_blocks_per_cu(const void* fn, size_t lds) {
    struct Entry { const void* fn; size_t lds; int n; };
    static Entry cache[32];
    static int used = 0;
    static std::mutex mu;
    {
        std::lock_guard<std::mutex> g(mu);
        for (int i = 0; i < used; ++i)
            if (cache[i].fn == fn && cache[i].lds == lds) return cache[i].n;
    }
    int n = 0;
    if (hipOccupancyMaxActiveBlocksPerMultiprocessor(&n, fn, 256, lds) != hipSuccess || n < 1) n = 1;
    std::lock_guard<std::mutex> g(mu);
    if (used < 32) cache[used++] = {fn, lds, n};
    return n;
}

inline int num_cus() {
    static const int n = [] {
        int dev = 0, v = 0;
        if (hipGetDevice(&dev) != hipSuccess ||
            hipDeviceGetAttribute(&v, hipDeviceAttributeMultiprocessorCount, dev) != hipSuccess || v < 1)
            v = 256;
        return v;
    }();
    return n;
}

std::atomic<int>& conv_impl_override();

size_t f1_state_bytes(int m, int nb);
size_t f1_fwd_workspace_bytes(int m, int nb);
size_t f1_bwd_workspace_bytes(int m, int e, int nb);
int f1_forward(const ConvArgs& a, float* out, float4* rec_out, void* state, void* ws, size_t ws_bytes, hipStream_t s);
int f1_backward(const ConvArgs& a, const float* out_grad, const float4* rec_in, const void* state, float* feat_grad, float* dw1, float* db1,
                float* dw2, float* db2, float* dw3, float* db3, void* ws, size_t ws_bytes, hipStream_t s);

__device__ __forceinline__ void reduce_partials_body(int bid, const float* __restrict__ partials, int numWaves, int nb,
                                                        float* __restrict__ dw1, float* __restrict__ db1,
                                                        float* __restrict__ dw2, float* __restrict__ db2,
                                                        float* __restrict__ dw3, float* __restrict__ db3) {
    __shared__ float acc[64][17];
    const int K = nb * 176;
    const int kk = threadIdx.x & 15, sl = threadIdx.x >> 4;
    const int k = bid * 16 + kk;
    float s0 = 0.f, s1 = 0.f, s2 = 0.f, s3 = 0.f;
    if (k < K) {
        int w = sl;
        for (; w + 192 < numWaves; w += 256) {
            s0 += partials[(size_t)w * K + k];
            s1 += partials[(size_t)(w + 64) * K + k];
            s2 += partials[(size_t)(w + 128) * K + k];
            s3 += partials[(size_t)(w + 192) * K + k];
        }
        for (; w < numWaves; w += 64) s0 += partials[(size_t)w * K + k];
    }
    acc[sl][kk] = (s0 + s1) + (s2 + s3);
    __syncthreads();
    if (sl == 0 && k < K) {
        float v = 0.f;
#pragma unroll
        for (int i = 0; i < 64; ++i) v += acc[i][kk];
        int q = k / 176, r = k - q * 176;
        if (r < 24) dw1[q * 24 + r] = v;
        else if (r < 32) db1[q * 8 + r - 24] = v;
        else if (r < 96) dw2[q * 64 + r - 32] = v;
        else if (r < 104) db2[q * 8 + r - 96] = v;
        else if (r < 168) dw3[q * 64 + r - 104] = v;
        else db3[q * 8 + r - 168] = v;
    }
}


}
```

mccnn_amd/csrc/exec.hip:

```cpp
#include "batch.h"

#include <chrono>
#include <cstdlib>
#include <cstring>
#include <new>
#include <thread>

namespace mccnn {
std::atomic<int>& conv_impl_override();
ClearSpan grid_head_span(int n, int batch_size, int num_cells, void* ws, size_t ws_bytes);
int build_grid_fused(const float* pts, const int* batch_ids, const float* aabb_min, const float* aabb_max, int n,
                     int batch_size, int num_cells, int* new_idx, float* out_pts, int* out_batch_ids, int* cell_indexs,
                     int* inv_idx, void* ws, size_t ws_bytes, hipStream_t s, const int* n_dev, bool cleared, ClearSpan x1,
                     ClearSpan x2);
size_t visiting_order_workspace_bytes(int m, int batch_size, int num_cells);
ClearSpan visiting_order_head_span(int m, int batch_size, int num_cells, void* ws, size_t ws_bytes);
int visiting_order(const float* pts, const int* batch_ids, const float* aabb_min, const float* aabb_max, int m, int batch_size,
                   int num_cells, int* order, void* ws, size_t ws_bytes, hipStream_t s, bool cleared);
bool plan_batchable(int rows, int e, int transposed);
size_t plan_batch_tr_ws_bytes(int n, int e);
int plan_batch_items(int transposed, const float* sorted_pts, const int* sorted_batch_ids, const float* pdfs, const float* samples,
                     const int* start_idx, const int* packed, const float* aabb_min, const float* aabb_max, int n, int m, int e,
                     int batch_size, float radius, int scale_inv, int avg, const int* order, int* start_t, int* perm_t,
                     int tlist_ready, void* plan_buffer, void* tws, size_t tws_bytes, TrSmallItem* tr, bool* use_tr,
                     PlanSmallItem& lay, SellFillItem& fill);
bool transpose_small(int e, int n);
int find_neighbors_chain(const float* centres, const int* centre_batch_ids, int m, const float* sorted_pts, int n,
                         const int* cell_indexs, const float* aabb_min, const float* aabb_max, int batch_size, int num_cells,
                         float radius, int scale_inv, const int* centre_order, int* start_idx, int e_capacity, int* packed,
                         int* total_dev, int* total_host, void* ws, size_t ws_bytes, mccnn_stream_t stream);
}

using namespace mccnn;

namespace {

struct Plan {
    char* buf = nullptr;
    size_t bytes = 0;
    bool built = false;
    int avg = -1;
    long long off[6] = {0, 0, 0, 0, 0, 0};
    long long total = 0, slots = 0, scratch_rows = 0;
    int S = 0;
};

inline size_t al(size_t x) { return align_up(x); }

}

struct mccnn_geometry {
    const float* pts = nullptr;
    const int* bids = nullptr;
    const float* centres = nullptr;
    const int* cbids = nullptr;
    const float* mn = nullptr;
    const float* mx = nullptr;
    int n = 0, m = 0, B = 0, nc = 0, scale_inv = 0, use_pdf = 1, same_level = 0;
    float radius = 0.f, window = 0.f;
    char* buf = nullptr;
    size_t bytes = 0;
    float* s_pts = nullptr;
    int *s_bids = nullptr, *cells = nullptr, *new_idx = nullptr, *inv_idx = nullptr;
    int *start = nullptr, *packed = nullptr, *total_dev = nullptr, *order = nullptr, *order_buf = nullptr;
    float* pdfs = nullptr;
    void* ws = nullptr;
    size_t ws_bytes = 0;
    const mccnn_geometry* grid_of = nullptr;
    int e_cap = 0;
    int e = -1;
    volatile int* total_host = nullptr;
    bool built = false;
    Plan plan[2];
    char* tl_buf = nullptr;
    size_t tl_bytes = 0;
    bool tl_built = false;
    char* rec_buf = nullptr;
    size_t rec_bytes = 0;
    int rec_avg = -1;
};

namespace {

enum { NEED_PLAN_FWD = 1, NEED_PLAN_TR = 2, NEED_TLIST = 4, NEED_RECORDS = 8 };

struct GeoLayout {
    size_t s_pts, s_bids, cells, new_idx, inv_idx, start, packed, pdfs, total, order, ws, ws_bytes, total_bytes;
};

size_t cells_of(int B, int nc) { return (size_t)B * nc * nc * nc; }
constexpr int MCCNN_ORDER_MIN_M = 16384;

GeoLayout geo_layout(int n, int m, int B, int nc, int e_cap, bool with_grid) {
    GeoLayout L;
    memset(&L, 0, sizeof(L));
    const size_t n1 = n > 0 ? n : 1, m1 = m > 0 ? m : 1, e1 = e_cap > 0 ? e_cap : 1;
    size_t o = 0;
    if (with_grid) {
        L.s_pts = o; o += al(n1 * 12);
        L.s_bids = o; o += al(n1 * 4);
        L.cells = o; o += al(cells_of(B, nc) * 8);
        L.new_idx = o; o += al(n1 * 4);
        L.inv_idx = o; o += al(n1 * 4);
    }
    L.start = o; o += al(m1 * 4);
    L.packed = o; o += al(e1 * 8);
    L.pdfs = o; o += al(e1 * 4);
    L.total = o; o += 256;
    L.order = o; o += al(m1 * 4);
    size_t w = mccnn_find_neighbors_workspace_bytes(m, n);
    size_t head = 0;
    if (with_grid) {
        const size_t g = mccnn_build_grid_workspace_bytes(n, B, nc);
        if (g == 0) return L;
        head += al(g);
    }
    if (m >= MCCNN_ORDER_MIN_M) {
        const size_t c = visiting_order_workspace_bytes(m, B, nc);
        if (c == 0) return L;
        head += al(c);
    }
    if (head > w) w = head;
    if (mccnn_sort_step1_workspace_bytes(m, B, nc) == 0) return L;
    const size_t p = mccnn_compute_pdf_workspace_bytes(e_cap, 1);
    if (p > w) w = p;
    L.ws = o;
    L.ws_bytes = al(w) + 256;
    o += L.ws_bytes;
    L.total_bytes = o;
    return L;
}

// ... 74 lines not shown

int plan_prepare(mccnn_geometry* g, int tr, int e) {
    Plan& p = g->plan[tr];
    const int rows = tr ? g->n : g->m;
    return mccnn_rowplan_buffer(rows, e, p.off, &p.total, &p.S, &p.slots, &p.scratch_rows);
}

size_t tlist_bytes(int n, int e) { return al((size_t)(n + 1) * 4) + al((size_t)(e > 0 ? e : 1) * 4); }
int* tl_start(const mccnn_geometry* g) { return reinterpret_cast<int*>(g->tl_buf); }
int* tl_perm(const mccnn_geometry* g) { return reinterpret_cast<int*>(g->tl_buf + al((size_t)(g->n + 1) * 4)); }

int ensure_tlist(mccnn_geometry* g, int e, void* ws, size_t ws_bytes, mccnn_stream_t stream) {
    if (g->tl_built) return 0;
    if (!g->tl_buf || g->tl_bytes < tlist_bytes(g->n, e)) return MCCNN_E_WORKSPACE;
    int rc = mccnn_transpose_neighbors(g->packed, e, g->n, tl_start(g), tl_perm(g), ws, ws_bytes, stream);
    if (rc) return rc;
    g->tl_built = true;
    return 0;
}

int ensure_plan(mccnn_geometry* g, int tr, int e, int avg, void* ws, size_t ws_bytes, mccnn_stream_t stream) {
    Plan& p = g->plan[tr];
    if (p.built && p.avg == avg) return 0;
    int rc = plan_prepare(g, tr, e);
    if (rc) return rc;
    if (!p.buf || p.bytes < (size_t)p.total) return MCCNN_E_WORKSPACE;
    const int rows = tr ? g->n : g->m;
    const bool inl = mccnn_rowplan_inline_records(rows, e) != 0;
    int rec_ready = 1;
    void* rec = nullptr;
    if (!inl) {
        if (!g->rec_buf || g->rec_bytes < (size_t)e * 16) return MCCNN_E_WORKSPACE;
        rec = g->rec_buf;
        rec_ready = g->rec_avg == avg ? 1 : 0;
    }
    int tready = 1;
    int *st = nullptr, *pt = nullptr;
    if (tr) {
        if (!g->tl_buf || g->tl_bytes < tlist_bytes(g->n, e)) return MCCNN_E_WORKSPACE;
        st = tl_start(g);
        pt = tl_perm(g);
        tready = g->tl_built ? 1 : 0;
    }
    const mccnn_geometry* go = grid_owner(g);
    const int* order = tr ? nullptr : (g->same_level ? go->inv_idx : (g->order ? g->order : nullptr));
    rc = mccnn_rowplan_build(tr, go->s_pts, go->s_bids, g->pdfs, g->centres, g->start, g->packed, g->mn, g->mx, g->n, g->m, e,
                             g->B, g->radius, g->scale_inv, avg, order, rec, rec_ready, st, pt, tready, p.buf, ws, ws_bytes,
                             stream);
    if (rc) return rc;
    if (!inl) g->rec_avg = avg;
    if (tr) g->tl_built = true;
    p.built = true;
    p.avg = avg;
    return 0;
}

size_t max3(size_t a, size_t b, size_t c) { return a > b ? (a > c ? a : c) : (b > c ? b : c); }

}

extern "C" {

mccnn_geometry_t* mccnn_geometry_create(void) { return new (std::nothrow) mccnn_geometry(); }
void mccnn_geometry_destroy(mccnn_geometry_t* g) { delete g; }

size_t mccnn_geometry_bytes(int n, int m, int batch_size, int num_cells, int e_capacity, int with_grid) {
    if (n < 0 || m < 0 || batch_size <= 0 || num_cells <= 0 || e_capacity < 0) return 0;
    if (cells_of(batch_size, num_cells) > 0x7fffffffULL) return 0;
    return geo_layout(n, m, batch_size, num_cells, e_capacity, with_grid != 0).total_bytes;
}

}
namespace {
int geometry_setup(mccnn_geometry_t* g, const float* pts, const int* batch_ids, int n, const float* centres,
                   const int* centre_batch_ids, int m, const float* aabb_min, const float* aabb_max, int batch_size, int num_cells,
                   float radius, int scale_inv, float window, int use_pdf, int e_capacity, const mccnn_geometry_t* grid_from,
                   void* buffer, size_t buffer_bytes, int* total_host, bool in_batch) {
    if (!g || !pts || !batch_ids || !centres || !centre_batch_ids || !aabb_min || !aabb_max || !buffer || !total_host)
        return MCCNN_E_BADARG;
    if (n <= 0 || m <= 0 || batch_size <= 0 || num_cells <= 0 || !(radius > 0.f) || e_capacity <= 0) return MCCNN_E_BADARG;
    if (use_pdf && !(window > 0.f)) return MCCNN_E_BADARG;
    if (grid_from && (grid_from->n != n || grid_from->nc != num_cells || grid_from->B != batch_size ||
                      !(grid_owner(grid_from)->built || (in_batch && grid_owner(grid_from)->s_pts))))
        return MCCNN_E_BADARG;
    const bool with_grid = grid_from == nullptr;
    const GeoLayout L = geo_layout(n, m, batch_size, num_cells, e_capacity, with_grid);
    if (L.total_bytes == 0) return MCCNN_E_TOOLARGE;
    if (buffer_bytes < L.total_bytes || (((uintptr_t)buffer) & 255)) return MCCNN_E_WORKSPACE;
    *g = mccnn_geometry();
    g->pts = pts; g->bids = batch_ids; g->centres = centres; g->cbids = centre_batch_ids; g->mn = aabb_min; g->mx = aabb_max;
    g->n = n; g->m = m; g->B = batch_size; g->nc = num_cells; g->scale_inv = scale_inv ? 1 : 0; g->use_pdf = use_pdf ? 1 : 0;
    g->radius = radius; g->window = window;
    g->same_level = (centres == pts && m == n) ? 1 : 0;
    g->buf = (char*)buffer; g->bytes = buffer_bytes;
    char* b = g->buf;
    if (with_grid) {
        g->s_pts = (float*)(b + L.s_pts); g->s_bids = (int*)(b + L.s_bids); g->cells = (int*)(b + L.cells);
        g->new_idx = (int*)(b + L.new_idx); g->inv_idx = (int*)(b + L.inv_idx);
    } else {
        g->grid_of = grid_owner(grid_from);
    }
    g->start = (int*)(b + L.start); g->packed = (int*)(b + L.packed); g->pdfs = (float*)(b + L.pdfs);
    g->total_dev = (int*)(b + L.total);
    g->order_buf = (int*)(b + L.order);
    g->ws = b + L.ws; g->ws_bytes = L.ws_bytes;
    g->e_cap = e_capacity; g->e = -1; g->total_host = total_host;
// ... 148 lines not shown
    int nc = 0, sorts = 0;
    auto flush = [&]() -> int {
        int rc = nc ? geometry_issue_chunk(chunk, nc, stream) : 0;
        nc = 0; sorts = 0;
        return rc;
    };
    for (int k = 0; k < count; ++k) {
        mccnn_geometry_t* g = req[k].geometry;
        const bool with_grid = g->grid_of == nullptr, own_order = !g->same_level && g->m >= MCCNN_ORDER_MIN_M;
        const bool ok = grid_batch_eligible(with_grid ? g->n : 1, g->B, g->nc) && (!own_order || grid_batch_eligible(g->m, g->B, g->nc)) &&
                        neigh_batch_eligible(g->m, g->n);
        if (!ok) {
            int rc = flush();
            if (!rc) rc = geometry_issue_single(g, stream);
            if (rc) return rc;
            continue;
        }
        const int need = (with_grid ? 1 : 0) + (own_order ? 1 : 0);
        if (nc == MCCNN_BATCH_MAX || sorts + need > MCCNN_BATCH_MAX) {
            int rc = flush();
            if (rc) return rc;
        }
        chunk[nc++] = g;
        sorts += need;
    }
    return flush();
}

long long mccnn_debug_wait_ns(void) { return g_wait_ns.load(std::memory_order_relaxed); }

int mccnn_debug_wait_accounting(int on) {
    const int prev = t_count_waits ? 1 : 0;
    t_count_waits = on != 0;
    return prev;
}

int mccnn_geometry_edges(mccnn_geometry_t* g, int wait_us) {
    if (!g || !g->built) return MCCNN_E_BADARG;
    const int e = wait_edges(g, wait_us);
    return e < 0 ? -1 : e;
}

int mccnn_geometry_info(const mccnn_geometry_t* g, long long out[16]) {
    if (!g || !g->built || !out) return MCCNN_E_BADARG;
    const mccnn_geometry* go = grid_owner(g);
    out[0] = (long long)(uintptr_t)go->s_pts; out[1] = (long long)(uintptr_t)go->s_bids; out[2] = (long long)(uintptr_t)go->cells;
    out[3] = (long long)(uintptr_t)go->new_idx; out[4] = (long long)(uintptr_t)go->inv_idx;
    out[5] = (long long)(uintptr_t)g->start; out[6] = (long long)(uintptr_t)g->packed; out[7] = (long long)(uintptr_t)g->pdfs;
    out[8] = g->n; out[9] = g->m; out[10] = g->nc; out[11] = g->e_cap; out[12] = g->e; out[13] = g->B;
    out[14] = (long long)(uintptr_t)g->total_dev; out[15] = g->grid_of ? 0 : 1;
    return 0;
}

int mccnn_geometry_attach(mccnn_geometry_t* g, int what, void* buffer, size_t bytes) {
    if (!g || !g->built || !buffer || (((uintptr_t)buffer) & 255)) return MCCNN_E_BADARG;
    switch (what) {
        case NEED_PLAN_FWD: g->plan[0] = Plan(); g->plan[0].buf = (char*)buffer; g->plan[0].bytes = bytes; return 0;
        case NEED_PLAN_TR: g->plan[1] = Plan(); g->plan[1].buf = (char*)buffer; g->plan[1].bytes = bytes; return 0;
        case NEED_TLIST: g->tl_buf = (char*)buffer; g->tl_bytes = bytes; g->tl_built = false; return 0;
        case NEED_RECORDS: g->rec_buf = (char*)buffer; g->rec_bytes = bytes; g->rec_avg = -1; return 0;
        default: return MCCNN_E_BADARG;
    }
}

}
namespace {
size_t piece_bytes(mccnn_geometry* g, int what, int e) {
    switch (what) {
        case NEED_PLAN_FWD: return plan_prepare(g, 0, e) ? 0 : (size_t)g->plan[0].total;
        case NEED_PLAN_TR: return plan_prepare(g, 1, e) ? 0 : (size_t)g->plan[1].total;
        case NEED_TLIST: return tlist_bytes(g->n, e);
        case NEED_RECORDS: return al((size_t)e * 16);
        default: return 0;
    }
}
}
extern "C" {

int mccnn_geometry_piece_bytes(mccnn_geometry_t* g, int what, long long* bytes, long long* ws_bytes) {
    if (!g || !g->built || !bytes || !ws_bytes) return MCCNN_E_BADARG;
    const int e = wait_edges(g, -1);
    if (e < 0) return MCCNN_E_BADARG;
    if (e > g->e_cap) return MCCNN_E_CAPACITY;
    *bytes = (long long)piece_bytes(g, what, e);
    size_t w = 256;
    if (what == NEED_TLIST) w = mccnn_transpose_neighbors_workspace_bytes(g->n, e);
    if (what == NEED_PLAN_FWD) w = mccnn_rowplan_build_workspace_bytes(g->m, e, 0);
    if (what == NEED_PLAN_TR) w = mccnn_rowplan_build_workspace_bytes(g->n, e, 1);
    *ws_bytes = (long long)(al(w) + 512);
    return *bytes > 0 ? 0 : MCCNN_E_BADARG;
}

int mccnn_geometry_piece_bound(int n, int m, int e_cap, int what, long long* bytes, long long* ws_bytes) {
    if (n < 0 || m < 0 || e_cap < 0 || !bytes || !ws_bytes) return MCCNN_E_BADARG;
    long long b = 0, w = 256;
    int rc = 0;
    switch (what) {
        case NEED_PLAN_FWD: rc = mccnn_rowplan_bound(m, e_cap, 0, &b, &w); break;
        case NEED_PLAN_TR: rc = mccnn_rowplan_bound(n, e_cap, 1, &b, &w); break;
        case NEED_TLIST: b = (long long)tlist_bytes(n, e_cap); w = (long long)mccnn_transpose_neighbors_workspace_bytes(n, e_cap); break;
        case NEED_RECORDS: b = (long long)al((size_t)(e_cap > 0 ? e_cap : 1) * 16); break;
        default: return MCCNN_E_BADARG;
    }
    if (rc) return rc;
    *bytes = (long long)al((size_t)b);
    *ws_bytes = (long long)(al((size_t)w) + 512);
    return 0;
}

int mccnn_geometry_prebuild(mccnn_geometry_t* g, int what, int avg, void* ws, size_t ws_bytes, mccnn_stream_t stream) {
    if (!g || !g->built || !ws) return MCCNN_E_BADARG;
    const int e = wait_edges(g, -1);
    if (e < 0) return MCCNN_E_BADARG;
    if (e > g->e_cap) return MCCNN_E_CAPACITY;
    if (e == 0) return 0;
    avg = avg ? 1 : 0;
    int rc = 0;
    if (what & NEED_PLAN_FWD) rc = ensure_plan(g, 0, e, avg, ws, ws_bytes, stream);
    if (!rc && (what & NEED_PLAN_TR)) rc = ensure_plan(g, 1, e, avg, ws, ws_bytes, stream);
    if (!rc && (what & NEED_TLIST)) rc = ensure_tlist(g, e, ws, ws_bytes, stream);
    return rc;
}

size_t mccnn_geometry_prebuild_batch_ws_bytes(mccnn_geometry_t* const* geoms, const int* what, int count) {
    if (!geoms || !what || count < 0) return 0;
    size_t single = 256, trs = 0;
    for (int k = 0; k < count; ++k) {
        mccnn_geometry_t* g = geoms[k];
        if (!g || !g->built) return 0;
        const int e = wait_edges(g, -1);
        if (e <= 0 || e > g->e_cap) continue;
        for (int bit = 1; bit <= 4; bit <<= 1) {
            if (!(what[k] & bit)) continue;
            long long b = 0, w = 0;
            if (mccnn_geometry_piece_bytes(g, bit, &b, &w) == 0 && (size_t)w > single) single = (size_t)w;
        }
        if ((what[k] & 6) && !g->tl_built)
            trs += transpose_small(e, g->n) ? al(plan_batch_tr_ws_bytes(g->n, e)) : al(mccnn_transpose_neighbors_workspace_bytes(g->n, e));
        for (int tr = 0; tr < 2; ++tr)
            if ((what[k] & (tr ? 2 : 1)) && plan_large_batchable(tr ? g->n : g->m, e, g->n, tr, 0))
                trs += al(plan_large_ws_bytes(tr ? g->n : g->m, e, g->n, tr, 0));
    }
    return al(single) + trs + 512;
}

int mccnn_geometry_prebuild_batch(mccnn_geometry_t* const* geoms, const int* what, int count, int avg, void* ws, size_t ws_bytes,
                                  mccnn_stream_t stream) {
    if (!geoms || !what || count < 0 || !ws) return MCCNN_E_BADARG;
    hipStream_t s = (hipStream_t)stream;
    avg = avg ? 1 : 0;
    Arena ar(ws, ws_bytes);
    size_t single = 256;
    for (int k = 0; k < count; ++k) {
        mccnn_geometry_t* g = geoms[k];
        if (!g || !g->built) return MCCNN_E_BADARG;
        const int e = wait_edges(g, -1);
        if (e < 0) return MCCNN_E_BADARG;
        if (e == 0 || e > g->e_cap) continue;
        for (int bit = 1; bit <= 4; bit <<= 1) {
            if (!(what[k] & bit)) continue;
            long long b = 0, w = 0;
            if (mccnn_geometry_piece_bytes(g, bit, &b, &w) == 0 && (size_t)w > single) single = (size_t)w;
        }
    }
    char* sws = ar.take<char>(al(single));
    if (!sws) return MCCNN_E_WORKSPACE;
    TrSmallBatch trB;
    TrChainBatch chB;
    ScanBatch chScan;
    SpanBatch chSpans;
    chSpans.count = 0;
    PlanSmallBatch layB;
    SellFillBatch fwdB, trfB;
// ... 98 lines not shown
            if (tr) ++nTrf; else ++nFwd;
            if (tr) g->tl_built = true;
            p.built = true;
            p.avg = avg;
            rest &= ~bit;
            if (tr) rest &= ~4;
        }
        for (int tr = 0; tr < 2; ++tr) {
            const int bit = tr ? 2 : 1;
            if (!(rest & bit)) continue;
            Plan& p = g->plan[tr];
            const int rows = tr ? g->n : g->m;
            if (!plan_large_batchable(rows, e, g->n, tr, g->tl_built ? 1 : 0)) continue;
            if (plan_prepare(g, tr, e)) continue;
            if (!p.buf || p.bytes < (size_t)p.total) continue;
            if (!g->rec_buf || g->rec_bytes < (size_t)e * 16) continue;
            if (tr && (!g->tl_buf || g->tl_bytes < tlist_bytes(g->n, e))) continue;
            if (nLg + 1 > MCCNN_LARGE_BATCH_MAX || nCh + 1 > MCCNN_PLAN_BATCH_MAX || chSpans.count + 3 > 3 * MCCNN_BATCH_MAX) {
                int rc = flush();
                if (rc) return rc;
            }
            const size_t wb = al(plan_large_ws_bytes(rows, e, g->n, tr, g->tl_built ? 1 : 0));
            char* w = ar.take<char>(wb);
            if (!w) continue;
            const int* order = tr ? nullptr : (g->same_level ? go->inv_idx : (g->order ? g->order : nullptr));
            bool use_chain = false;
            const int spans0 = chSpans.count;
            int rc = plan_large_item(tr, go->s_pts, go->s_bids, g->pdfs, g->centres, g->start, g->packed, g->mn, g->mx, g->n, g->m, e, g->B,
                                     g->radius, g->scale_inv, avg, order, g->rec_buf, g->rec_avg == avg ? 1 : 0, tr ? tl_start(g) : nullptr,
                                     tr ? tl_perm(g) : nullptr, g->tl_built ? 1 : 0, p.buf, w, wb, lgB.it[nLg], &chB.it[nCh], &chScan.it[nCh],
                                     &use_chain, chSpans);
            if (rc) { chSpans.count = spans0; continue; }
            ++nLg;
            if (use_chain) ++nCh;
            g->rec_avg = avg;
            if (tr) g->tl_built = true;
            p.built = true;
            p.avg = avg;
            rest &= ~bit;
            if (tr) rest &= ~4;
        }
        if (rest && nLater < 256) later[nLater++] = Later{g, rest};
    }
    int rc = flush();
    if (rc) return rc;
    for (int k = 0; k < nLater; ++k) {
        mccnn_geometry_t* g = later[k].g;
        const int e = g->e, w = later[k].what;
        if (w & NEED_PLAN_FWD) rc = ensure_plan(g, 0, e, avg, sws, al(single), stream);
        if (!rc && (w & NEED_PLAN_TR)) rc = ensure_plan(g, 1, e, avg, sws, al(single), stream);
        if (!rc && (w & NEED_TLIST)) rc = ensure_tlist(g, e, sws, al(single), stream);
        if (rc) return rc;
    }
    return 0;
}

struct Req {
    int mask;
    long long need_bytes[4];
    size_t ws, saved;
};
static int requirements(mccnn_geometry* g, const Shape& s, const void* feats, int backward, int flags, int e, Req& r) {
    const int n = g->n, m = g->m;
    const FwdMode f = fwd_mode(g, s, feats, e);
    int mask = 0;
    for (int k = 0; k < 4; ++k) r.need_bytes[k] = 0;
    size_t ws = 256, saved = 0;
    auto want_plan = [&](int tr) -> int {
        Plan& p = g->plan[tr];
        int rc = plan_prepare(g, tr, e);
        if (rc) return rc;
        if (!p.buf || p.bytes < (size_t)p.total) { mask |= tr ? NEED_PLAN_TR : NEED_PLAN_FWD; r.need_bytes[tr] = p.total; }
        const int rows = tr ? n : m;
        if (!mccnn_rowplan_inline_records(rows, e) && (!g->rec_buf || g->rec_bytes < (size_t)e * 16)) {
            mask |= NEED_RECORDS;
            r.need_bytes[3] = (long long)al((size_t)e * 16);
        }
        const size_t b = mccnn_rowplan_build_workspace_bytes(rows, e, tr);
        if (b > ws) ws = b;
        return 0;
    };
    auto want_tlist = [&]() {
        if (!g->tl_buf || g->tl_bytes < tlist_bytes(n, e)) { mask |= NEED_TLIST; r.need_bytes[2] = (long long)tlist_bytes(n, e); }
        if (!g->tl_built) {
            const size_t b = mccnn_transpose_neighbors_workspace_bytes(n, e);
            if (b > ws) ws = b;
        }
    };
    if (!backward) {
        if (!f.unsorted) saved += al((size_t)n * s.fin * s.elem);
        if (f.rows_fwd) {
            int rc = want_plan(0);
            if (rc) return rc;
            const size_t scratch = al((size_t)g->plan[0].scratch_rows * s.outF * 4);
            ws = max3(ws, scratch, 256);
        } else if (!s.bf16) {
            const size_t w = mccnn_spatial_conv_fwd_workspace_bytes(m, e, s.fin, s.fout, s.combin);
            if (w > ws) ws = w;
            if (flags & 1) saved += al(mccnn_spatial_conv_state_bytes(m, e, s.fin, s.fout, s.combin));
        }
    } else {
        const bool rows_bwd = f.rows_bwd && m > 0;
        size_t fg_sorted = f.unsorted && rows_bwd ? 0 : al((size_t)n * s.fin * s.elem);
        size_t sort_again = 0;
        if (rows_bwd) {
            int rc = want_plan(1);
            if (rc) return rc;
            want_tlist();
            const size_t w = al(mccnn_spatial_conv_bwd_rows_workspace_bytes(n, e, s.fin)) + al((size_t)g->plan[1].scratch_rows * s.fin * 4);
            ws = max3(ws, w + fg_sorted, 256);
            const size_t w2 = al(mccnn_spatial_conv_bwd_workspace_bytes(n, m, e, s.fin, s.fout, s.combin));
            const size_t tb = e > 0 ? al(mccnn_transpose_neighbors_workspace_bytes(n, e)) : 0;
            const size_t full = al((size_t)n * s.fin * s.elem);
            ws = max3(ws, (w2 > tb ? w2 : tb) + full + (f.unsorted ? full : 0), 256);
        } else {
            if (f.unsorted) sort_again = al((size_t)n * s.fin * s.elem);
            size_t tb = 0;
            if (e > 0 && (!s.combin || ((flags & 2) && s.fin >= 2 && s.fin <= 4))) {
                want_tlist();
                tb = al(mccnn_transpose_neighbors_workspace_bytes(n, e));
            }
            const size_t w = al(mccnn_spatial_conv_bwd_workspace_bytes(n, m, e, s.fin, s.fout, s.combin));
            ws = max3(ws, (w > tb ? w : tb) + fg_sorted + sort_again, 256);
        }
    }
    r.mask = mask;
    r.ws = ws + 512;
    r.saved = saved;
    return 0;
}

int mccnn_conv_prepare(mccnn_geometry_t* g, const void* feats, int num_in_feats, int num_out_feats, int combin, int bf16,
                       int backward, int flags, int* need_mask, long long need_bytes[4], long long* ws_bytes,
                       long long* saved_bytes, int* edges) {
    if (!g || !g->built || !need_mask || !need_bytes || !ws_bytes || !saved_bytes || !edges) return MCCNN_E_BADARG;
    Shape s;
    if (!make_shape(s, num_in_feats, num_out_feats, combin, bf16)) return MCCNN_E_SHAPE;
    const int e = wait_edges(g, -1);
    if (e < 0) return MCCNN_E_BADARG;
    *edges = e;
    if (e > g->e_cap) return MCCNN_E_CAPACITY;
    Req r;
    int rc = requirements(g, s, feats, backward, flags, e, r);
    if (rc) return rc;
    *need_mask = r.mask;
    for (int k = 0; k < 4; ++k) need_bytes[k] = r.need_bytes[k];
    *ws_bytes = (long long)r.ws;
    *saved_bytes = (long long)r.saved;
    return 0;
}

int mccnn_conv_forward(mccnn_geometry_t* g, const void* feats, int num_in_feats, int num_out_feats, int combin, int avg,
                       int bf16, int flags, const float* w1, const float* b1, const float* w2, const float* b2,
                       const float* w3, const float* b3, void* out, void* saved, size_t saved_bytes, void* ws,
                       size_t ws_bytes, mccnn_stream_t stream) {
    if (!g || !g->built || !feats || !out || !ws) return MCCNN_E_BADARG;
    Shape s;
    if (!make_shape(s, num_in_feats, num_out_feats, combin, bf16)) return MCCNN_E_SHAPE;
    const int e = wait_edges(g, -1);
    if (e < 0) return MCCNN_E_BADARG;
    if (e > g->e_cap) return MCCNN_E_CAPACITY;
    const int n = g->n, m = g->m;
    const mccnn_geometry* go = grid_owner(g);
    const FwdMode f = fwd_mode(g, s, feats, e);
    avg = avg ? 1 : 0;
    {
        Req r;
        int rc = requirements(g, s, feats, 0, flags, e, r);
        if (rc) return rc;
        if (r.mask || ws_bytes < r.ws || (r.saved && (!saved || saved_bytes < r.saved))) return MCCNN_E_WORKSPACE;
    }
    const void* rows_in = feats;
    char* sv = (char*)saved;
    size_t sv_off = 0;
    if (!f.unsorted) {
        const size_t b = al((size_t)n * s.fin * s.elem);
        if (!saved || saved_bytes < b) return MCCNN_E_WORKSPACE;
        int rc = mccnn_permute_scatter((const float*)feats, go->new_idx, n, s.words, (float*)sv, n, 0, stream);
        if (rc) return rc;
        rows_in = sv;
        sv_off = b;
    }
    if (f.rows_fwd) {
        int rc = ensure_plan(g, 0, e, avg, ws, ws_bytes, stream);
        if (rc) return rc;
        const Plan& p = g->plan[0];
        if (ws_bytes < (size_t)p.scratch_rows * s.outF * 4) return MCCNN_E_WORKSPACE;
        char* pb = p.buf;
        return mccnn_spatial_conv_fwd_rows(go->s_pts, rows_in, go->s_bids, g->pdfs, g->centres, g->start, g->packed, g->mn, g->mx,
                                           w1, b1, w2, b2, w3, b3, n, m, e, s.fin, g->B, g->radius, g->scale_inv, avg, s.bf16,
                                           (const int*)(pb + p.off[0]), (const int*)(pb + p.off[1]), (const int*)(pb + p.off[2]),
                                           (const int*)(pb + p.off[3]), pb + p.off[5], (const int*)(pb + p.off[4]), out,
                                           (float*)ws, f.unsorted ? go->inv_idx : nullptr, stream);
    }
    if (s.bf16)
        return mccnn_spatial_conv_fwd_bf16(go->s_pts, rows_in, go->s_bids, g->pdfs, g->centres, g->start, g->packed, g->mn, g->mx, w1,
                                           b1, w2, b2, w3, b3, n, m, e, s.fin, g->B, g->radius, g->scale_inv, avg, out, ws, ws_bytes,
                                           stream);
    void* state = nullptr;
    if (flags & 1) {
        const size_t sb = mccnn_spatial_conv_state_bytes(m, e, s.fin, s.fout, s.combin);
        if (sb) {
            if (!saved || saved_bytes < sv_off + sb) return MCCNN_E_WORKSPACE;
            state = sv + sv_off;
        }
    }
    return mccnn_spatial_conv_fwd(go->s_pts, (const float*)rows_in, go->s_bids, g->pdfs, g->centres, g->start, g->packed, g->mn,
                                  g->mx, w1, b1, w2, b2, w3, b3, n, m, e, s.fin, s.fout, s.combin, g->B, g->radius, g->scale_inv,
                                  avg, (float*)out, state, ws, ws_bytes, stream);
}

int mccnn_conv_backward(mccnn_geometry_t* g, const void* feats, const void* saved, size_t saved_bytes, const void* out_grad,
                        int num_in_feats, int num_out_feats, int combin, int avg, int bf16, int flags, const float* w1,
                        const float* b1, const float* w2, const float* b2, const float* w3, const float* b3,
                        void* feat_grad, float* dw1, float* db1, float* dw2, float* db2, float* dw3, float* db3, void* ws,
                        size_t ws_bytes, mccnn_stream_t stream) {
    if (!g || !g->built || !feats || !out_grad || !feat_grad || !ws) return MCCNN_E_BADARG;
    Shape s;
    if (!make_shape(s, num_in_feats, num_out_feats, combin, bf16)) return MCCNN_E_SHAPE;
    const int e = wait_edges(g, -1);
    if (e < 0) return MCCNN_E_BADARG;
    if (e > g->e_cap) return MCCNN_E_CAPACITY;
    const int n = g->n, m = g->m;
    const mccnn_geometry* go = grid_owner(g);
    const FwdMode f = fwd_mode(g, s, feats, e);
    avg = avg ? 1 : 0;
    {
        Req r;
        int rc = requirements(g, s, feats, 1, flags, e, r);
        if (rc) return rc;
        if (r.mask || ws_bytes < r.ws) return MCCNN_E_WORKSPACE;
    }
    const size_t rows_b = al((size_t)n * s.fin * s.elem);
    const char* sv = (const char*)saved;
    size_t sv_off = 0;
    const void* rows_in = feats;
    if (!f.unsorted) {
        if (!saved || saved_bytes < rows_b) return MCCNN_E_WORKSPACE;
        rows_in = sv;
        sv_off = rows_b;
    }
    Arena a(ws, ws_bytes);
    const bool rows_bwd = f.rows_bwd && m > 0 && ((((uintptr_t)out_grad) & 15) == 0);
    int rc;
    if (rows_bwd) {
        rc = ensure_plan(g, 1, e, avg, ws, ws_bytes, stream);
        if (rc) return rc;
        const Plan& p = g->plan[1];
        void* fg = feat_grad;
        if (!f.unsorted) {
            fg = a.take<char>(rows_b);
            if (!fg) return MCCNN_E_WORKSPACE;
        }
        float* scratch = a.take<float>((size_t)p.scratch_rows * s.fin);
        const size_t wb = mccnn_spatial_conv_bwd_rows_workspace_bytes(n, e, s.fin);
        char* w = a.take<char>(wb);
        if (!scratch || !w) return MCCNN_E_WORKSPACE;
        char* pb = p.buf;
        rc = mccnn_spatial_conv_bwd_rows(go->s_pts, rows_in, go->s_bids, g->pdfs, g->centres, g->start, g->packed, g->mn, g->mx, w1,
                                         b1, w2, b2, w3, b3, out_grad, n, m, e, s.fin, g->B, g->radius, g->scale_inv, avg, s.bf16,
                                         tl_start(g), (const int*)(pb + p.off[0]), (const int*)(pb + p.off[1]),
                                         (const int*)(pb + p.off[2]), (const int*)(pb + p.off[3]), pb + p.off[5],
                                         (const int*)(pb + p.off[4]), fg, scratch, dw1, db1, dw2, db2, dw3, db3,
                                         f.unsorted ? go->inv_idx : nullptr, w, wb, stream);
        if (rc) return rc;
        if (!f.unsorted)
            return mccnn_permute_gather((const float*)fg, go->new_idx, n, s.words, (float*)feat_grad, stream);
        return 0;
    }
    if (f.unsorted) {
        char* sorted = a.take<char>(rows_b);
        if (!sorted) return MCCNN_E_WORKSPACE;
        rc = mccnn_permute_scatter((const float*)feats, go->new_idx, n, s.words, (float*)sorted, n, 0, stream);
        if (rc) return rc;
        rows_in = sorted;
    }
    char* fg = a.take<char>(rows_b);
    if (!fg) return MCCNN_E_WORKSPACE;
    const int *st = nullptr, *pt = nullptr;
    if (e > 0 && (!s.combin || ((flags & 2) && s.fin >= 2 && s.fin <= 4) || (s.combin && s.fin >= 2 && s.fin <= 4 && g->tl_built))) {
        const size_t tb = mccnn_transpose_neighbors_workspace_bytes(n, e);
        if (!g->tl_built) {
            char* tw = a.base + a.off;
            if (a.cap - a.off < tb) return MCCNN_E_WORKSPACE;
            rc = ensure_tlist(g, e, tw, a.cap - a.off, stream);
            if (rc) return rc;
        }
        st = tl_start(g);
        pt = tl_perm(g);
    }
    const size_t wb = mccnn_spatial_conv_bwd_workspace_bytes(n, m, e, s.fin, s.fout, s.combin);
    char* w = a.take<char>(wb);
    if (!w) return MCCNN_E_WORKSPACE;
    if (s.bf16) {
        rc = mccnn_spatial_conv_bwd_bf16(go->s_pts, rows_in, go->s_bids, g->pdfs, g->centres, g->start, g->packed, g->mn, g->mx, w1,
                                         b1, w2, b2, w3, b3, out_grad, n, m, e, s.fin, g->B, g->radius, g->scale_inv, avg, st, pt,
                                         fg, dw1, db1, dw2, db2, dw3, db3, w, wb, stream);
    } else {
        const void* state = nullptr;
        if (flags & 1) {
            const size_t sb = mccnn_spatial_conv_state_bytes(m, e, s.fin, s.fout, s.combin);
            if (sb && saved && saved_bytes >= sv_off + sb && !f.unsorted && !f.rows_fwd) state = sv + sv_off;
        }
        rc = mccnn_spatial_conv_bwd(go->s_pts, (const float*)rows_in, go->s_bids, g->pdfs, g->centres, g->start, g->packed, g->mn,
                                    g->mx, w1, b1, w2, b2, w3, b3, (const float*)out_grad, n, m, e, s.fin, s.fout, s.combin, g->B,
                                    g->radius, g->scale_inv, avg, state, st, pt, (float*)fg, dw1, db1, dw2, db2, dw3, db3, w, wb,
                                    stream);
    }
    if (rc) return rc;
    return mccnn_permute_gather((const float*)fg, go->new_idx, n, s.words, (float*)feat_grad, stream);
}

}
```

mccnn_amd/csrc/torch_ext.cpp:

```cpp
#include <torch/extension.h>
#include <execinfo.h>
#include <torch/csrc/autograd/function.h>
#include <torch/csrc/autograd/functions/utils.h>
#include <torch/csrc/autograd/saved_variable.h>
#include <c10/hip/HIPStream.h>
#include <ATen/hip/impl/HIPGuardImplMasqueradingAsCUDA.h>
#include <ATen/hip/impl/HIPStreamMasqueradingAsCUDA.h>
#include <hip/hip_runtime_api.h>

#include <atomic>
#include <chrono>
#include <condition_variable>
#include <cstdlib>
#include <deque>
#include <functional>
#include <map>
#include <thread>
#include <memory>
#include <mutex>
#include <string>
#include <vector>

#include "mccnn.h"
#include "debug_opts.h"

namespace {

using at::Tensor;

struct CapacityError : std::runtime_error {
    int edges;
    CapacityError(int e) : std::runtime_error("neighbour list longer than the geometry's capacity"), edges(e) {}
};

void check(int rc, const char* what) {
    if (rc == 0) return;
    throw std::runtime_error(std::string(what) + " failed: " + mccnn_error_string(rc) + " (code " + std::to_string(rc) + ")");
}

struct DevGuard {
    int prev = 0;
    bool changed = false;
    explicit DevGuard(int d) {
        if (hipGetDevice(&prev) == hipSuccess && d != prev && d >= 0) changed = hipSetDevice(d) == hipSuccess;
    }
    ~DevGuard() {
        if (changed) (void)hipSetDevice(prev);
    }
    DevGuard(const DevGuard&) = delete;
    DevGuard& operator=(const DevGuard&) = delete;
};

void* cur_stream(const Tensor& t) { return (void*)c10::hip::getCurrentHIPStream(t.device().index()).stream(); }
c10::Stream as_torch_stream(void* s, int dev) {
    return c10::hip::getStreamFromExternalMasqueradingAsCUDA((hipStream_t)s, (c10::DeviceIndex)dev).unwrap();
}

hipEvent_t take_event_fwd();
void give_event_fwd(hipEvent_t e);

Tensor& scratch(size_t bytes, const Tensor& like, void* stream) {
    thread_local std::map<std::pair<int, void*>, Tensor> pool;
// ... 256 lines not shown
        }
    }
    ~Geo() {
        wait_issued_nothrow();
        const bool total_pending = slot.defined() && e.load(std::memory_order_relaxed) < 0 &&
                                   *reinterpret_cast<volatile int*>(slot.data_ptr()) < 0;
        hipEvent_t slot_ev = nullptr;
        if (event && build_rc == 0 && side >= 0 && grid_owner && grid_owner->own_pool && grid_owner->side != side)
            (void)hipStreamWaitEvent((hipStream_t)grid_owner->alloc_stream, event, 0);
        if (event) {
            if (needs_wait && buf.defined() && build_rc == 0) {
                (void)hipStreamWaitEvent((hipStream_t)alloc_stream, event, 0);
                order_caller_behind(event);
            }
            if (total_pending && build_rc == 0) slot_ev = event;
            else give_event(event);
        } else if (total_pending && build_rc == 0 && buf.defined()) {
            try {
                slot_ev = take_event();
                if (hipEventRecord(slot_ev, (hipStream_t)alloc_stream) != hipSuccess) { give_event(slot_ev); slot_ev = nullptr; }
            } catch (const std::exception&) {
                slot_ev = nullptr;
            }
        }
        if (plan_event) {
            if (plan_wait && buf.defined()) {
                (void)hipStreamWaitEvent((hipStream_t)alloc_stream, plan_event, 0);
                order_caller_behind(plan_event);
            }
            give_event(plan_event);
        }
        if (tr_event) {
            if (tr_wait && buf.defined()) {
                (void)hipStreamWaitEvent((hipStream_t)alloc_stream, tr_event, 0);
                order_caller_behind(tr_event);
            }
            give_event(tr_event);
        }
        if (h) mccnn_geometry_destroy(h);
        if (slot.defined()) {
            if (!total_pending) give_slot(std::move(slot));
            else if (slot_ev) park_slot(std::move(slot), slot_ev);
            else if (build_rc != 0) give_slot(std::move(slot));
            else park_slot(std::move(slot), nullptr);
        }
    }
    hipEvent_t plan_event = nullptr;
    bool plan_wait = false;
    hipEvent_t tr_event = nullptr;
    bool tr_wait = false;
    int pre_avg = -1;
    int have = 0;
    int plan_side = -1;

    int issue_pieces(int what, bool avg, hipStream_t ss, void* ws, size_t wsb) {
        int rc = 0;
        if (what & 1) {
            rc = mccnn_geometry_prebuild(h, 1, avg ? 1 : 0, ws, wsb, (void*)ss);
            if (!rc) {
                if (!plan_event) plan_event = take_event();
                if (hipEventRecord(plan_event, ss) != hipSuccess) rc = (int)hipErrorUnknown;
                plan_wait = true;
            }
        }
        if (!rc && (what & 6)) {
            rc = mccnn_geometry_prebuild(h, what & 6, avg ? 1 : 0, ws, wsb, (void*)ss);
            if (!rc) {
                if (!tr_event) tr_event = take_event();
                if (hipEventRecord(tr_event, ss) != hipSuccess) rc = (int)hipErrorUnknown;
                tr_wait = true;
            }
        }
        pre_avg = avg ? 1 : 0;
        return rc;
    }

    void prebuild(int what, bool avg, int side_k, const Tensor& like) {
        const DevGuard device_guard((int)like.device().index());
        wait_issued();
        const int E = edges(-1);
        if (E <= 0 || E > e_cap) return;
        if (what & 3) what |= 8;
        if (what & 2) what |= 4;
        what &= ~have;
        if (!what) return;
        void* main_stream = cur_stream(like);
        hipStream_t ss = side >= 0 ? side_stream(side) : side_stream(side_k);
        if (!ss) return;
        size_t wsb = 256;
        for (int bit = 1; bit <= 8; bit <<= 1) {
            if (!(what & bit)) continue;
            long long bytes = 0, w = 0;
            check(mccnn_geometry_piece_bytes(h, bit, &bytes, &w), "geometry_piece_bytes");
            Tensor t;
            if (own_pool) {
                const c10::hip::HIPStreamGuardMasqueradingAsCUDA own(as_torch_stream((void*)ss, (int)like.device().index()));
                t = at::empty({(int64_t)(bytes > 256 ? bytes : 256)}, like.options().dtype(at::kByte));
            } else {
                t = at::empty({(int64_t)(bytes > 256 ? bytes : 256)}, like.options().dtype(at::kByte));
            }
            check(mccnn_geometry_attach(h, bit, t.data_ptr(), (size_t)t.numel()), "geometry_attach");
            attached.push_back(std::move(t));
            have |= bit;
            if ((size_t)w > wsb) wsb = (size_t)w;
        }
        Tensor& ws = scratch(wsb, like, (void*)ss);
        if (!own_pool) {
            static thread_local hipEvent_t fork_ev = nullptr;
            if (!fork_ev) hip_check(hipEventCreateWithFlags(&fork_ev, hipEventDisableTiming), "hipEventCreate");
            hip_check(hipEventRecord(fork_ev, (hipStream_t)main_stream), "hipEventRecord");
            hip_check(hipStreamWaitEvent(ss, fork_ev, 0), "hipStreamWaitEvent");
        }
        if (event && side < 0) hip_check(hipStreamWaitEvent(ss, event, 0), "hipStreamWaitEvent");
        check(issue_pieces(what & 7, avg, ss, ws.data_ptr(), (size_t)ws.numel()), "geometry_prebuild");
    }

    int edges(int wait_us) {
        wait_issued();
        if (e < 0 && h) {
            const int v = mccnn_geometry_edges(h, wait_us);
            if (v >= 0) e = v;
        }
        return e;
    }
    std::vector<int64_t> info() {
        wait_issued();
        long long out[16];
        check(mccnn_geometry_info(h, out), "geometry_info");
        return std::vector<int64_t>(out, out + 16);
    }
};

void check_dev(const Tensor& t, at::ScalarType dt, const char* name) {
    TORCH_CHECK(t.defined() && t.is_cuda() && t.scalar_type() == dt && t.is_contiguous(), name,
                ": expected a contiguous device tensor of the op's type");
}

struct HierFuture;
hipEvent_t hierarchy_ready_event(const std::shared_ptr<HierFuture>& f);
bool hierarchy_owns(const std::shared_ptr<HierFuture>& f, const Tensor& t);

struct BatchEntry {
    std::shared_ptr<Geo> g, grid_from;
    mccnn_geometry_request req;
};
struct PieceEntry {
    std::shared_ptr<Geo> g;
    int what;
    bool avg;
    char* base;
    long long off[4], len[4];
};
struct GeoBatch {
    bool active = false;
    int side = -1;
    bool background = false;
    std::vector<BatchEntry> entries;
    std::vector<PieceEntry> pieces;
    Tensor arena[2];
    int64_t arena_off[2] = {0, 0}, taken[2] = {0, 0};
};
thread_local GeoBatch t_geo_batch;
thread_local int64_t t_arena_want[2] = {0, 0};
Tensor arena_take(int k, int64_t bytes, const Tensor& like) {
    GeoBatch& b = t_geo_batch;
    const int64_t need = (bytes + 255) / 256 * 256;
    b.taken[k] += need;
    if (!b.active || t_arena_want[k] <= 0) return Tensor();
    if (!b.arena[k].defined()) {
        b.arena[k] = at::empty({t_arena_want[k] + t_arena_want[k] / 16 + 4096}, like.options().dtype(at::kByte));
        b.arena_off[k] = 0;
    }
    if (b.arena_off[k] + need > b.arena[k].numel()) return Tensor();
    Tensor t = b.arena[k].narrow(0, b.arena_off[k], bytes);
    b.arena_off[k] += need;
    return t;
}
void begin_geometry_batch() {
    t_geo_batch.active = Issuer::enabled();
    t_geo_batch.side = -1;
    t_geo_batch.entries.clear();
    t_geo_batch.pieces.clear();
    for (int k = 0; k < 2; ++k) { t_geo_batch.arena[k] = Tensor(); t_geo_batch.arena_off[k] = t_geo_batch.taken[k] = 0; }
}
void end_geometry_batch() {
    GeoBatch& b = t_geo_batch;
    b.active = false;
    for (int k = 0; k < 2; ++k) {
        if (b.taken[k] > 0) t_arena_want[k] = b.taken[k];
        b.arena[k] = Tensor();
    }
    if (b.entries.empty()) return;
    auto entries = std::make_shared<std::vector<BatchEntry>>(std::move(b.entries));
    b.entries.clear();
    hipStream_t stream = side_stream(b.side);
    const bool background = b.background;
    const int dev = (int)(*entries)[0].g->buf.device().index();
    Issuer::get().push([entries, stream, background, dev] {
        enter_device(dev);
        std::vector<mccnn_geometry_request> reqs;
        reqs.reserve(entries->size());
        for (BatchEntry& e : *entries) {
            bool inside = false;
            if (e.grid_from)
                for (BatchEntry& o : *entries) inside = inside || (o.g.get() == e.grid_from.get());
            if (e.grid_from && !inside) e.grid_from->wait_issued_nothrow();
            reqs.push_back(e.req);
        }
        const int prev = background ? mccnn_background_launches(1) : 0;
        int rc = mccnn_geometry_build_batch(reqs.data(), (int)reqs.size(), (void*)stream);
        if (background) mccnn_background_launches(prev);
        for (BatchEntry& e : *entries) {
            int r = rc;
            if (r == 0 && hipEventRecord(e.g->event, stream) != hipSuccess) r = (int)hipErrorUnknown;
            e.g->build_rc = r;
            e.g->issued.store(1, std::memory_order_release);
        }
    });
    if (b.pieces.empty()) return;
    auto pieces = std::make_shared<std::vector<PieceEntry>>(std::move(b.pieces));
    b.pieces.clear();
    const int pside = (*pieces)[0].g->plan_side;
    Issuer::get(2).push([pieces, pside, dev]() mutable {
        enter_device(dev);
        hipStream_t ss = side_stream(pside);
        std::vector<mccnn_geometry_t*> hs;
        std::vector<int> whats;
        std::vector<PieceEntry*> live;
        bool avg = (*pieces)[0].avg;
        hipEvent_t last = nullptr;
        for (PieceEntry& pe : *pieces) {
            Geo& g = *pe.g;
            g.wait_build_issued_nothrow();
            if (g.build_rc != 0) continue;
            const int prev = mccnn_debug_wait_accounting(0);
            const int E = mccnn_geometry_edges(g.h, -1);
            mccnn_debug_wait_accounting(prev);
            if (E >= 0) g.e.store(E, std::memory_order_relaxed);
            if (E <= 0 || E > g.e_cap) continue;
            int rc = 0;
            for (int k = 0; k < 4 && !rc; ++k)
                if (pe.what & (1 << k)) rc = mccnn_geometry_attach(g.h, 1 << k, pe.base + pe.off[k], (size_t)pe.len[k]);
            if (rc) continue;
            g.have |= pe.what;
            hs.push_back(g.h);
            whats.push_back(pe.what & 7);
            live.push_back(&pe);
            if (g.event) last = g.event;
        }
        int rc = 0;
        if (!hs.empty()) {
            if (last && hipStreamWaitEvent(ss, last, 0) != hipSuccess) rc = (int)hipErrorUnknown;
            if (!rc) {
                try {
                    const size_t wsb = mccnn_geometry_prebuild_batch_ws_bytes(hs.data(), whats.data(), (int)hs.size());
                    Tensor& ws = scratch(wsb, live[0]->g->buf, (void*)ss);
                    rc = mccnn_geometry_prebuild_batch(hs.data(), whats.data(), (int)hs.size(), avg ? 1 : 0, ws.data_ptr(), (size_t)ws.numel(), (void*)ss);
                } catch (const std::exception&) {
                    rc = (int)hipErrorUnknown;
                }
            }
            if (rc) fprintf(stderr, "mccnn: batch of row plans / transposed lists: error %d (the layers build what is missing)\n", rc);
            for (PieceEntry* pe : live) {
                Geo& g = *pe->g;
                if (pe->what & 1) {
                    if (!g.plan_event) g.plan_event = take_event();
                    if (hipEventRecord(g.plan_event, ss) == hipSuccess) g.plan_wait = true;
                }
                if (pe->what & 6) {
                    if (!g.tr_event) g.tr_event = take_event();
                    if (hipEventRecord(g.tr_event, ss) == hipSuccess) g.tr_wait = true;
                }
                g.pre_avg = avg ? 1 : 0;
            }
        }
        for (PieceEntry& pe : *pieces) pe.g->pieces_issued.store(1, std::memory_order_release);
    });
}

std::shared_ptr<Geo> build_geometry(const Tensor& pts, const Tensor& bids, const Tensor& centres, const Tensor& cbids,
                                    const Tensor& mn, const Tensor& mx, int64_t B, int64_t nc, double radius, bool scale_inv,
                                    double window, bool use_pdf, int64_t capacity, std::shared_ptr<Geo> grid_from,
                                    int64_t side, bool fork, bool background, std::shared_ptr<HierFuture> after) {
    check_dev(pts, at::kFloat, "points");
    check_dev(centres, at::kFloat, "sample points");
    check_dev(bids, at::kInt, "batch ids");
    check_dev(cbids, at::kInt, "sample batch ids");
    check_dev(mn, at::kFloat, "aabb_min");
    check_dev(mx, at::kFloat, "aabb_max");
    const DevGuard device_guard((int)pts.device().index());
    const int n = (int)pts.size(0), m = (int)centres.size(0);
    if (grid_from && grid_from->grid_owner) grid_from = grid_from->grid_owner;
    const size_t bytes = mccnn_geometry_bytes(n, m, (int)B, (int)nc, (int)capacity, grid_from ? 0 : 1);
    TORCH_CHECK(bytes > 0, "geometry: batch_size * num_cells^3 does not fit 32-bit keys");
    auto g = std::make_shared<Geo>();
    g->h = mccnn_geometry_create();
    TORCH_CHECK(g->h, "mccnn_geometry_create failed");
    g->slot = take_slot();
    g->keep = {pts, bids, centres, cbids, mn, mx};
    g->grid_owner = grid_from;
    g->n = n; g->m = m; g->nc = (int)nc; g->B = (int)B; g->e_cap = capacity;
    void* stream = cur_stream(pts);
    g->alloc_stream = stream;
    if (side >= 0 && grid_from && grid_from->side >= 0 && grid_from->needs_wait) side = grid_from->side;
    const bool batched = side >= 0 && t_geo_batch.active;
    const int asked_side = side >= 0 ? (int)(((side % kSideStreams) + kSideStreams) % kSideStreams) : -1;
    if (batched) {
        if (t_geo_batch.side < 0) { t_geo_batch.side = (int)(((side % kSideStreams) + kSideStreams) % kSideStreams); t_geo_batch.background = background; }
        side = t_geo_batch.side;
    }
    static const bool own_pools = mccnn::debug_int("geo_own_pool", 1) != 0;
    hipEvent_t ready = (side >= 0 && own_pools && Issuer::enabled()) ? hierarchy_ready_event(after) : nullptr;
    if (ready && grid_from && !grid_from->own_pool) ready = nullptr;
    if (ready)
        for (const Tensor* t : {&pts, &bids, &centres, &cbids, &mn, &mx})
            if (!hierarchy_owns(after, *t)) { ready = nullptr; break; }
    static thread_local bool fork_skipped = false;
    if (ready && side_stream((int)side)) {
        hipStream_t ss = side_stream((int)side);
        if (fork) fork_skipped = true;
        {
            const c10::hip::HIPStreamGuardMasqueradingAsCUDA own(as_torch_stream((void*)ss, (int)pts.device().index()));
            if (batched) g->buf = arena_take(0, (int64_t)bytes, pts);
            if (!g->buf.defined()) g->buf = at::empty({(int64_t)bytes}, pts.options().dtype(at::kByte));
        }
        g->own_pool = true;
        g->caller_stream = stream;
        g->has_caller = true;
        g->alloc_stream = (void*)ss;
        hip_check(hipStreamWaitEvent(ss, ready, 0), "hipStreamWaitEvent");
        const int sk = (int)(((side % kSideStreams) + kSideStreams) % kSideStreams);
        if (grid_from && grid_from->event && grid_from->side != sk) {
            grid_from->wait_issued();
            hip_check(hipStreamWaitEvent(ss, grid_from->event, 0), "hipStreamWaitEvent");
        }
        g->side = sk;
        stream = ss;
    } else if (side >= 0) {
        g->buf = at::empty({(int64_t)bytes}, pts.options().dtype(at::kByte));
        hipStream_t ss = side_stream((int)side);
        if (ss) {
            static thread_local hipEvent_t fork_ev = nullptr;
            if (!fork_ev) {
                hip_check(hipEventCreateWithFlags(&fork_ev, hipEventDisableTiming), "hipEventCreate");
                fork = true;
            }
            if (fork || fork_skipped) hip_check(hipEventRecord(fork_ev, (hipStream_t)stream), "hipEventRecord");
            fork_skipped = false;
            hip_check(hipStreamWaitEvent(ss, fork_ev, 0), "hipStreamWaitEvent");
            if (grid_from && grid_from->event && grid_from->side != (int)(((side % kSideStreams) + kSideStreams) % kSideStreams)) {
                grid_from->wait_issued();
                hip_check(hipStreamWaitEvent(ss, grid_from->event, 0), "hipStreamWaitEvent");
            }
            g->side = (int)(((side % kSideStreams) + kSideStreams) % kSideStreams);
            stream = ss;
        }
    } else {
        g->buf = at::empty({(int64_t)bytes}, pts.options().dtype(at::kByte));
        if (grid_from) grid_from->join(stream);
    }
    if (g->side >= 0 && Issuer::enabled()) {
        g->event = take_event();
        g->needs_wait = true;
        g->issued.store(0, std::memory_order_release);
        const float* p0 = pts.data_ptr<float>();
        const int* p1 = bids.data_ptr<int>();
        const float* p2 = centres.data_ptr<float>();
        const int* p3 = cbids.data_ptr<int>();
        const float* p4 = mn.data_ptr<float>();
        const float* p5 = mx.data_ptr<float>();
        void* bufp = g->buf.data_ptr();
        int* slotp = g->slot.data_ptr<int>();
        const int iB = (int)B, inc = (int)nc, icap = (int)capacity, isi = scale_inv ? 1 : 0, ipdf = use_pdf ? 1 : 0;
        const float fr = (float)radius, fw = (float)window;
        const int dev = (int)pts.device().index();
        if (batched && stream == (void*)side_stream(t_geo_batch.side)) {
            BatchEntry e;
            e.g = g;
            e.grid_from = grid_from;
            e.req = mccnn_geometry_request{g->h, p0, p1, n, p2, p3, m, p4, p5, iB, inc, fr, isi, fw, ipdf, icap,
                                           grid_from ? grid_from->h : nullptr, bufp, bytes, slotp};
            t_geo_batch.entries.push_back(std::move(e));
            g->plan_side = asked_side;
            return g;
        }
        Issuer::get().push([g, grid_from, p0, p1, p2, p3, p4, p5, bufp, slotp, n, m, iB, inc, icap, isi, ipdf, fr, fw, bytes, stream, background, dev] {
            enter_device(dev);
            if (grid_from) grid_from->wait_issued_nothrow();
            const int prev = background ? mccnn_background_launches(1) : 0;
            int rc = mccnn_geometry_build(g->h, p0, p1, n, p2, p3, m, p4, p5, iB, inc, fr, isi, fw, ipdf, icap,
                                          grid_from ? grid_from->h : nullptr, bufp, bytes, slotp, stream);
            if (background) mccnn_background_launches(prev);
            if (rc == 0 && hipEventRecord(g->event, (hipStream_t)stream) != hipSuccess) rc = (int)hipErrorUnknown;
            g->build_rc = rc;
            g->issued.store(1, std::memory_order_release);
        });
        return g;
    }
    if (grid_from) grid_from->wait_issued();
    const int prev_bg = (background && g->side >= 0) ? mccnn_background_launches(1) : 0;
    struct Restore {
        bool on; int prev;
        ~Restore() { if (on) mccnn_background_launches(prev); }
    } restore{background && g->side >= 0, prev_bg};
    check(mccnn_geometry_build(g->h, pts.data_ptr<float>(), bids.data_ptr<int>(), n, centres.data_ptr<float>(),
                               cbids.data_ptr<int>(), m, mn.data_ptr<float>(), mx.data_ptr<float>(), (int)B, (int)nc,
                               (float)radius, scale_inv ? 1 : 0, (float)window, use_pdf ? 1 : 0, (int)capacity,
                               grid_from ? grid_from->h : nullptr, g->buf.data_ptr(), bytes, g->slot.data_ptr<int>(),
                               stream),
          "geometry_build");
    if (g->side >= 0) {
        g->event = take_event();
        hip_check(hipEventRecord(g->event, (hipStream_t)stream), "hipEventRecord");
        g->needs_wait = true;
    }
    return g;
}

void prebuild_async(std::shared_ptr<Geo> g, int what, bool avg) {
    if (!g || g->side < 0 || !Issuer::enabled() || g->e_cap <= 0) return;
    const DevGuard device_guard((int)g->buf.device().index());
    if (what & 3) what |= 8;
    if (what & 2) what |= 4;
    what &= 15 & ~g->have;
    if (!what) return;
    long long off[4] = {0, 0, 0, 0}, len[4] = {0, 0, 0, 0}, total = 0, wsb = 256;
    for (int k = 0; k < 4; ++k) {
        if (!(what & (1 << k))) continue;
        long long b = 0, w = 0;
        check(mccnn_geometry_piece_bound(g->n, g->m, (int)g->e_cap, 1 << k, &b, &w), "geometry_piece_bound");
        off[k] = total;
        len[k] = b;
        total += (b + 255) / 256 * 256;
        if (w > wsb) wsb = w;
    }
    const bool batched = t_geo_batch.active && t_geo_batch.side >= 0 && g->plan_side >= 0;
    if (batched) g->plan_side = (t_geo_batch.side + 1) % kSideStreams;
    const bool other = g->plan_side >= 0 && g->plan_side != g->side;
    hipStream_t ss = side_stream(other ? g->plan_side : g->side);
    Tensor block;
    if (g->own_pool) {
        const c10::hip::HIPStreamGuardMasqueradingAsCUDA own(as_torch_stream((void*)ss, (int)g->buf.device().index()));
        if (batched) block = arena_take(1, (int64_t)total, g->buf);
        if (!block.defined()) block = at::empty({(int64_t)total}, g->buf.options());
    } else {
        block = at::empty({(int64_t)total}, g->buf.options());
    }
    g->attached.push_back(block);
    g->pieces_issued.store(0, std::memory_order_release);
    char* base = (char*)block.data_ptr();
    Tensor like = g->buf;
    if (batched) {
        PieceEntry pe;
        pe.g = g; pe.what = what; pe.avg = avg; pe.base = base;
        for (int k = 0; k < 4; ++k) { pe.off[k] = off[k]; pe.len[k] = len[k]; }
        t_geo_batch.pieces.push_back(std::move(pe));
        return;
    }
    Issuer::get(2).push([g, what, avg, base, off, len, wsb, ss, like, other]() mutable {
        enter_device((int)like.device().index());
        g->wait_build_issued_nothrow();
        if (g->build_rc == 0 && other && g->event && hipStreamWaitEvent(ss, g->event, 0) != hipSuccess) g->build_rc = (int)hipErrorUnknown;
        if (g->build_rc == 0) {
            const int prev = mccnn_debug_wait_accounting(0);
            const int E = mccnn_geometry_edges(g->h, -1);
            mccnn_debug_wait_accounting(prev);
            if (E >= 0) g->e.store(E, std::memory_order_relaxed);
            if (E > 0 && E <= g->e_cap) {
                int rc = 0;
                for (int k = 0; k < 4 && !rc; ++k)
                    if (what & (1 << k)) rc = mccnn_geometry_attach(g->h, 1 << k, base + off[k], (size_t)len[k]);
                if (!rc) {
                    g->have |= what;
                    try {
                        Tensor& ws = scratch((size_t)wsb, like, (void*)ss);
                        rc = g->issue_pieces(what & 7, avg, ss, ws.data_ptr(), (size_t)ws.numel());
                    } catch (const std::exception&) {
                        rc = (int)hipErrorUnknown;
                    }
                }
            }
        }
        g->pieces_issued.store(1, std::memory_order_release);
    });
}

struct Layer {
    int fin, fout, combin, avg, bf16, flags;
};

void prepare(Geo& g, const Tensor& feats, const Layer& L, int backward, int flags, long long& ws_bytes, long long& saved_bytes) {
    int mask = 0, edges = 0;
    long long need[4] = {0, 0, 0, 0};
    int rc = mccnn_conv_prepare(g.h, feats.data_ptr(), L.fin, L.fout, L.combin, L.bf16, backward, flags, &mask, need, &ws_bytes,
                                &saved_bytes, &edges);
    if (rc == MCCNN_E_CAPACITY) {
        g.e = edges;
        throw CapacityError(edges);
    }
    check(rc, "conv_prepare");
    g.e = edges;
    for (int k = 0; k < 4 && mask; ++k) {
        const int bit = 1 << k;
        if (!(mask & bit)) continue;
        Tensor t = at::empty({(int64_t)(need[k] > 256 ? need[k] : 256)}, feats.options().dtype(at::kByte));
        check(mccnn_geometry_attach(g.h, bit, t.data_ptr(), (size_t)t.numel()), "geometry_attach");
        g.attached.push_back(std::move(t));
        g.have |= bit;
    }
}

enum { T_FWD = 0, T_FWD_LIB, T_FWD_ALLOC, T_BWD, T_BWD_LIB, T_BWD_ALLOC, T_BWD_VIEWS, T_BWD_JOIN, T_N };
std::atomic<long long> g_t_ns[T_N], g_t_calls[T_N];
struct Tick {
    int k;
    std::chrono::steady_clock::time_point t0;
    explicit Tick(int k_) : k(k_), t0(std::chrono::steady_clock::now()) {}
    ~Tick() {
        g_t_ns[k].fetch_add(std::chrono::duration_cast<std::chrono::nanoseconds>(std::chrono::steady_clock::now() - t0).count(), std::memory_order_relaxed);
        g_t_calls[k].fetch_add(1, std::memory_order_relaxed);
    }
};

struct ConvBackward : public torch::autograd::Node {
    std::shared_ptr<Geo> geo;
    Tensor feats_, w1_, b1_, w2_, b2_, w3_, b3_;
    uint32_t versions[7] = {0, 0, 0, 0, 0, 0, 0};
    Tensor saved;
    Layer L;
// ... 47 lines not shown
            o += cnt;
            return t;
        };
        torch::autograd::variable_list out(7);
        out[0] = fg;
        out[1] = piece(n1, w1); out[2] = piece(n2, b1); out[3] = piece(n3, w2); out[4] = piece(n4, b2);
        out[5] = piece(n5, w3); out[6] = piece(n6, b3);
        return out;
    }

    void release_variables() override {
        feats_.reset(); w1_.reset(); b1_.reset(); w2_.reset(); b2_.reset(); w3_.reset(); b3_.reset();
        saved.reset();
        geo.reset();
    }
};

Tensor conv(std::shared_ptr<Geo> geo, const Tensor& feats, const Tensor& w1, const Tensor& b1, const Tensor& w2,
            const Tensor& b2, const Tensor& w3, const Tensor& b3, int64_t fout, bool combin, bool avg, bool deterministic) {
    TORCH_CHECK(geo && geo->h, "conv: no geometry");
    const DevGuard device_guard((int)feats.device().index());
    TORCH_CHECK(feats.defined() && feats.is_cuda() && feats.dim() == 2 && feats.size(0) == geo->n && feats.is_contiguous(),
                "SpatialConvOp expects as feature inputs the following dimensions (numPoints, numFeatures)");
    const bool bf = feats.scalar_type() == at::kBFloat16;
    TORCH_CHECK(bf || feats.scalar_type() == at::kFloat, "features must be float32 or bfloat16");
    for (const Tensor* t : {&w1, &b1, &w2, &b2, &w3, &b3}) check_dev(*t, at::kFloat, "kernel-MLP tensor");
    Layer L;
    L.fin = (int)feats.size(1); L.fout = (int)fout; L.combin = combin ? 1 : 0; L.avg = avg ? 1 : 0; L.bf16 = bf ? 1 : 0;
    const bool need_grad = at::GradMode::is_enabled() &&
                           (feats.requires_grad() || w1.requires_grad() || b1.requires_grad() || w2.requires_grad() ||
                            b2.requires_grad() || w3.requires_grad() || b3.requires_grad());
    L.flags = (need_grad ? 1 : 0) | (deterministic ? 2 : 0);
    Tensor out, saved;
    const Tick tick_all(T_FWD);
    {
        at::AutoDispatchBelowADInplaceOrView guard;
        geo->join(cur_stream(feats), geo->pre_avg != L.avg);
        if (geo->grid_owner) geo->grid_owner->join(cur_stream(feats));
        long long wsb = 0, svb = 0;
        prepare(*geo, feats, L, 0, L.flags, wsb, svb);
        {
            const Tick ta(T_FWD_ALLOC);
            out = at::empty({geo->m, combin ? fout : (int64_t)L.fin}, feats.options());
            if (svb > 0) saved = at::empty({(int64_t)svb}, feats.options().dtype(at::kByte));
        }
        void* st = cur_stream(feats);
        Tensor& ws = scratch((size_t)wsb, feats, st);
        const Tick tl(T_FWD_LIB);
        check(mccnn_conv_forward(geo->h, feats.data_ptr(), L.fin, L.fout, L.combin, L.avg, L.bf16, L.flags, w1.data_ptr<float>(),
                                 b1.data_ptr<float>(), w2.data_ptr<float>(), b2.data_ptr<float>(), w3.data_ptr<float>(),
                                 b3.data_ptr<float>(), out.data_ptr(), saved.defined() ? saved.data_ptr() : nullptr,
                                 (size_t)svb, ws.data_ptr(), (size_t)ws.numel(), st),
              "conv_forward");
    }
    if (need_grad) {
        auto node = std::shared_ptr<ConvBackward>(new ConvBackward(), torch::autograd::deleteNode);
        node->set_next_edges(torch::autograd::collect_next_edges(feats, w1, b1, w2, b2, w3, b3));
        node->geo = geo;
        node->feats_ = feats; node->w1_ = w1; node->b1_ = b1; node->w2_ = w2; node->b2_ = b2; node->w3_ = w3; node->b3_ = b3;
        {
            const Tensor* in[7] = {&feats, &w1, &b1, &w2, &b2, &w3, &b3};
            for (int k = 0; k < 7; ++k) node->versions[k] = in[k]->_version();
        }
        node->saved = saved;
        node->L = L;
        torch::autograd::set_history(out, node);
    }
    return out;
}

std::vector<Tensor> compute_aabb(const Tensor& pts, const Tensor& bids, int64_t B, bool scale_inv) {
    check_dev(pts, at::kFloat, "points");
    check_dev(bids, at::kInt, "batch ids");
    TORCH_CHECK(B > 0, "ComputeAabbOp expects a positive batch size");
    const DevGuard device_guard((int)pts.device().index());
    Tensor mn = at::empty({B, 3}, pts.options()), mx = at::empty({B, 3}, pts.options());
    void* st = cur_stream(pts);
    Tensor& ws = scratch(mccnn_compute_aabb_workspace_bytes((int)B), pts, st);
    check(mccnn_compute_aabb(pts.data_ptr<float>(), bids.data_ptr<int>(), (int)pts.size(0), (int)B, scale_inv ? 1 : 0, mn.data_ptr<float>(),
                             mx.data_ptr<float>(), ws.data_ptr(), (size_t)ws.numel(), st),
          "compute_aabb");
    return {mn, mx};
}

std::atomic<long long> g_wait_ns{0};
void count_wait(std::chrono::steady_clock::time_point t0) {
    if (t_helper_thread) return;
    g_wait_ns.fetch_add(std::chrono::duration_cast<std::chrono::nanoseconds>(std::chrono::steady_clock::now() - t0).count(),
                        std::memory_order_relaxed);
}

std::vector<std::vector<Tensor>> hierarchy_levels(const Tensor& pts, const Tensor& bids, const Tensor& mn, const Tensor& mx,
                                                  const std::vector<double>& radii, const std::vector<int64_t>& ncs,
                                                  int64_t B, bool scale_inv, int64_t pmode) {
    check_dev(pts, at::kFloat, "points");
    check_dev(bids, at::kInt, "batch ids");
    check_dev(mn, at::kFloat, "aabb_min");
    check_dev(mx, at::kFloat, "aabb_max");
    const DevGuard device_guard((int)pts.device().index());
    const int L = (int)radii.size();
    const int cap = (int)pts.size(0);
    TORCH_CHECK(L > 0 && (int)ncs.size() == L && cap > 0, "hierarchy_levels: bad arguments");
    void* st = cur_stream(pts);
    auto iopt = pts.options().dtype(at::kInt);
    Tensor sizes = at::empty({L + 1}, iopt);
    hip_check(hipMemcpyAsync(sizes.data_ptr(), &cap, sizeof(int), hipMemcpyHostToDevice, (hipStream_t)st), "hipMemcpyAsync");
// ... 331 lines not shown
        }
    }
    f->alloc_stream = (void*)ss;
    f->event = take_event();
    if (after_mode == 2 && after_event) {
        hip_check(hipStreamWaitEvent(ss, (hipEvent_t)(uintptr_t)after_event, 0), "hipStreamWaitEvent");
    } else if (after_mode != 1) {
        static thread_local hipEvent_t fork_ev = nullptr;
        if (!fork_ev) hip_check(hipEventCreateWithFlags(&fork_ev, hipEventDisableTiming), "hipEventCreate");
        hip_check(hipEventRecord(fork_ev, (hipStream_t)stream), "hipEventRecord");
        hip_check(hipStreamWaitEvent(ss, fork_ev, 0), "hipStreamWaitEvent");
    }
    if (Issuer::enabled()) {
        f->done.store(0, std::memory_order_release);
        Issuer::get(1).push([f, ss] { f->run(ss); });
    } else {
        f->run(ss);
    }
    return f;
}

}

PYBIND11_MODULE(TORCH_EXTENSION_NAME, mod) {
    mod.doc() = "PyTorch-ROCm side of the native step executor of libmccnn_hip.so";
    if (mccnn::debug_int("trace_terminate", 0)) {
        std::set_terminate([] {
            void* frames[64];
            const int n = backtrace(frames, 64);
            backtrace_symbols_fd(frames, n, 2);
            abort();
        });
    }
    static py::exception<CapacityError> cap_exc(mod, "CapacityError");
    py::register_exception_translator([](std::exception_ptr p) {
        try {
            if (p) std::rethrow_exception(p);
        } catch (const CapacityError& e) {
            PyErr_SetObject(cap_exc.ptr(), py::int_(e.edges).ptr());
        }
    });
    py::class_<Geo, std::shared_ptr<Geo>>(mod, "Geometry")
        .def_readonly("buf", &Geo::buf)
        .def_readonly("n", &Geo::n)
        .def_readonly("m", &Geo::m)
        .def_readonly("nc", &Geo::nc)
        .def_readonly("B", &Geo::B)
        .def_readonly("e_cap", &Geo::e_cap)
        .def_property_readonly("e", [](const Geo& g) { return g.e.load(std::memory_order_relaxed); })
        .def_readonly("grid_owner", &Geo::grid_owner)
        .def_readwrite("uses", &Geo::uses)
        .def_readonly("side", &Geo::side)
        .def_readonly("have", &Geo::have)
        .def("join", [](Geo& g, const at::Tensor& like) { g.join(cur_stream(like)); }, py::call_guard<py::gil_scoped_release>())
        .def("prebuild", &Geo::prebuild, py::arg("what"), py::arg("avg"), py::arg("side"), py::arg("like"),
             py::call_guard<py::gil_scoped_release>())
        .def("edges", &Geo::edges, py::arg("wait_us") = -1, py::call_guard<py::gil_scoped_release>())
        .def("info", &Geo::info, py::call_guard<py::gil_scoped_release>());
    mod.def("build_geometry", &build_geometry, py::arg("pts"), py::arg("bids"), py::arg("centres"), py::arg("cbids"),
            py::arg("mn"), py::arg("mx"), py::arg("B"), py::arg("nc"), py::arg("radius"), py::arg("scale_inv"),
            py::arg("window"), py::arg("use_pdf"), py::arg("capacity"), py::arg("grid_from").none(true),
            py::arg("side") = -1, py::arg("fork") = false, py::arg("background") = false,
            py::arg("after").none(true) = py::none(), py::call_guard<py::gil_scoped_release>());
    mod.def("sampled_features", &sampled_features, py::call_guard<py::gil_scoped_release>());
    mod.def("begin_geometry_batch", &begin_geometry_batch);
    mod.def("end_geometry_batch", &end_geometry_batch, py::call_guard<py::gil_scoped_release>());
    mod.def("prebuild_async", &prebuild_async, py::arg("geometry"), py::arg("what"), py::arg("avg"),
            py::call_guard<py::gil_scoped_release>());
    mod.def("conv", &conv, py::arg("geometry"), py::arg("feats"), py::arg("w1"), py::arg("b1"), py::arg("w2"), py::arg("b2"),
            py::arg("w3"), py::arg("b3"), py::arg("fout"), py::arg("combin"), py::arg("avg"), py::arg("deterministic") = false,
            py::call_guard<py::gil_scoped_release>());
    mod.def("compute_aabb", &compute_aabb);
    mod.def("hierarchy_levels", &hierarchy_levels, py::call_guard<py::gil_scoped_release>());
    py::class_<HierFuture, std::shared_ptr<HierFuture>>(mod, "HierarchyFuture")
        .def("result", &HierFuture::result)
        .def("done", [](HierFuture& f) { return f.done.load(std::memory_order_acquire) != 0; });
    mod.def("hierarchy_prefetch", &hierarchy_prefetch, py::arg("pts"), py::arg("bids"), py::arg("radii"), py::arg("B"),
            py::arg("scale_inv"), py::arg("pmode"), py::arg("after_mode") = 0, py::arg("after_event") = 0,
            py::arg("feats") = py::none(), py::call_guard<py::gil_scoped_release>());
    mod.def("shutdown_helpers", [] { for (int k = 0; k < 3; ++k) Issuer::get(k).retire(); },
            py::call_guard<py::gil_scoped_release>());
    mod.def("wait_ns", [] { return (long long)g_wait_ns.load(std::memory_order_relaxed); });
    mod.def("debug_counters", [] {
        py::dict d;
        d["caller_orderings"] = (long long)g_caller_orderings.load(std::memory_order_relaxed);
        return d;
    });
    mod.def("debug_times", [](bool reset) {
        static const char* names[T_N] = {"fwd", "fwd_lib", "fwd_alloc", "bwd", "bwd_lib", "bwd_alloc", "bwd_views", "bwd_join"};
        py::dict d;
        for (int k = 0; k < T_N; ++k) {
            d[names[k]] = py::make_tuple((long long)g_t_ns[k].load(), (long long)g_t_calls[k].load());
            if (reset) { g_t_ns[k].store(0); g_t_calls[k].store(0); }
        }
        return d;
    }, py::arg("reset") = false);
}
```

mccnn_amd/native.py:

```python
import os
import ctypes as C
import threading
import weakref

import torch

from . import _env, _lib
from ._lib import check, ptr, stream_handle

def _load_ext():
    import importlib.util
    import os
    from ._env import flag
    if not flag("TORCH_EXT"):
        return None
    path = os.path.join(os.path.dirname(os.path.abspath(__file__)), "lib", "_mccnn_torch.so")
    if not os.path.exists(path):
        return None
    _lib.load()
    try:
        spec = importlib.util.spec_from_file_location("_mccnn_torch", path)
        mod = importlib.util.module_from_spec(spec)
        spec.loader.exec_module(mod)
    except (ImportError, OSError) as err:
# ... 111 lines not shown
        self.attached = []
        self.grid_owner = None
        self.n = self.m = self.nc = self.B = self.e_cap = 0
        self.e = -1
        self.gkey = None
        self.args = None
        self.uses = 0

    def __del__(self):
        h, self.handle = self.handle, None
        if h is not None:
            try:
                _lib.load().mccnn_geometry_destroy(h)
            except Exception:
                pass
        if self.slot is not None:
            if self.e >= 0:
                _release_slot(self.slot)
            else:
                try:
                    _park_slot(self.slot)
                except Exception:
                    pass

    def edges(self):
        if self.e < 0:
            e = self.core.edges(-1) if self.core is not None else _lib.load().mccnn_geometry_edges(self.handle, -1)
            if e < 0:
                raise _lib.MCCNNError("geometry: edge total not available")
            self.e = e
            _remember(self.gkey, self.m, e)
            if e > self.e_cap:
                self._rebuild(e + e // 16 + 64)
        return self.e

    def _rebuild(self, capacity):
        inPts, inBids, centres, cbids, mn, mx, B, nc, radius, scaleInv, window, usePDF = self.args
        _build_into(self, inPts, inBids, centres, cbids, mn, mx, B, nc, radius, scaleInv, window, usePDF, capacity,
                    self.grid_owner)
        e = self.core.edges(-1) if self.core is not None else _lib.load().mccnn_geometry_edges(self.handle, -1)
        if e < 0 or e > self.e_cap:
            raise _lib.MCCNNError("geometry: rebuilt list still does not fit (%d > %d)" % (e, self.e_cap))
        self.e = e

    def prebuild(self, what, avg, side, like):
        if self.core is not None:
            self.edges()
            self.core.prebuild(int(what), bool(avg), int(side), like)

    @property
    def have(self):
        return int(self.core.have) if self.core is not None else 0

    def prebuild_async(self, what, avg):
        if self.core is not None:
            _EXT.prebuild_async(self.core, int(what), bool(avg))

    def _info(self):
        if self.core is not None:
            return self.core.info()
        out = (C.c_longlong * 16)()
        check(_lib.load().mccnn_geometry_info(self.handle, out), "geometry_info")
        return list(out)

    def _view(self, owner_buf, addr, nbytes, dtype, shape):
        off = addr - owner_buf.data_ptr()
        return owner_buf[off:off + nbytes].view(dtype).view(shape)

    def _join(self):
        for g in (self, self.grid_owner):
            if g is not None and g.core is not None and g.buf is not None:
                g.core.join(g.buf)

    def grid(self):
        self._join()
        i = self._info()
        ob = (self.grid_owner or self).buf
        n, nc, B = self.n, self.nc, self.B
        return (self._view(ob, i[0], n * 12, torch.float32, (n, 3)), self._view(ob, i[1], n * 4, torch.int32, (n, 1)),
                self._view(ob, i[2], B * nc ** 3 * 8, torch.int32, (B, nc, nc, nc, 2)),
                self._view(ob, i[3], n * 4, torch.int32, (n,)), self._view(ob, i[4], n * 4, torch.int32, (n,)))

    def neighbors(self):
        e = self.edges()
        self._join()
        i = self._info()
        return (self._view(self.buf, i[5], self.m * 4, torch.int32, (self.m, 1)),
                self._view(self.buf, i[6], e * 8, torch.int32, (e, 2)))

    def pdfs(self):
        e = self.edges()
        self._join()
        i = self._info()
        return self._view(self.buf, i[7], e * 4, torch.float32, (e, 1))


def _build_into(g, inPts, inBids, centres, cbids, mn, mx, B, nc, radius, scaleInv, window, usePDF, capacity, grid_from,
                side=-1, fork=False, background=False, after=None):
    n, m = inPts.shape[0], centres.shape[0]
    if _EXT is not None:
        uses = g.core.uses if g.core is not None else 0
        g.core = _EXT.build_geometry(inPts, inBids, centres, cbids, mn, mx, B, nc, float(radius), bool(scaleInv), float(window),
                                     bool(usePDF), capacity, grid_from.core if grid_from is not None else None, side, fork,
                                     background, after)
        g.core.uses = uses
        g.buf = g.core.buf
        g.grid_owner = grid_from
        g.n, g.m, g.nc, g.B, g.e_cap, g.e = n, m, nc, B, capacity, -1
        g.args = (inPts, inBids, centres, cbids, mn, mx, B, nc, radius, scaleInv, window, usePDF)
        return
    lib = _lib.load()
    dev = inPts.device
    with_grid = 0 if grid_from is not None else 1
    nbytes = lib.mccnn_geometry_bytes(n, m, B, nc, capacity, with_grid)
    if nbytes == 0:
        raise _lib.MCCNNError("geometry: batch_size * num_cells^3 does not fit 32-bit keys")
    if g.handle is None:
        g.handle = lib.mccnn_geometry_create()
        if not g.handle:
            raise MemoryError("mccnn_geometry_create")
    if g.slot is None:
        g.slot = _slot()
    g.buf = torch.empty(nbytes, dtype=torch.uint8, device=dev)
    g.attached = []
    g.keep = (inPts, inBids, centres, cbids, mn, mx)
    g.grid_owner = grid_from
    g.n, g.m, g.nc, g.B, g.e_cap, g.e = n, m, nc, B, capacity, -1
    g.args = (inPts, inBids, centres, cbids, mn, mx, B, nc, radius, scaleInv, window, usePDF)
    check(lib.mccnn_geometry_build(g.handle, ptr(inPts), ptr(inBids), n, ptr(centres), ptr(cbids), m, ptr(mn), ptr(mx), B, nc,
                                   float(radius), int(bool(scaleInv)), float(window), int(bool(usePDF)), capacity,
                                   grid_from.handle if grid_from is not None else None, g.buf.data_ptr(), nbytes,
                                   g.slot.data_ptr(), stream_handle()), "geometry_build")


def begin_batch():
    if _EXT is not None:
        _EXT.begin_geometry_batch()


def end_batch():
    if _EXT is not None:
        _EXT.end_geometry_batch()


def side_streams_available():
    return _EXT is not None


def build_geometry(inPts, inBids, centres, cbids, mn, mx, B, nc, radius, scaleInv, window, usePDF, grid_from=None,
                   side=-1, fork=False, background=False, after=None):
    n, m = inPts.shape[0], centres.shape[0]
    gkey = (inPts.device.index, n, m, float(radius), int(B), bool(scaleInv))
    g = Geometry()
    g.gkey = gkey
    if grid_from is not None and grid_from.grid_owner is not None:
        grid_from = grid_from.grid_owner
    _build_into(g, inPts, inBids, centres, cbids, mn, mx, B, nc, radius, scaleInv, window, usePDF,
                _capacity_guess(gkey, m), grid_from, side if _EXT is not None else -1, fork, background,
                after if _EXT is not None else None)
    return g


_I0 = C.c_int
_LL = C.c_longlong


def _prepare(geo, feats, fin, fout, combin, bf16, backward, flags):
    lib = _lib.load()
    mask, edges = _I0(0), _I0(0)
    need = (_LL * 4)()
    wsb, svb = _LL(0), _LL(0)
    rc = lib.mccnn_conv_prepare(geo.handle, feats.data_ptr(), fin, fout, combin, bf16, backward, flags, C.byref(mask), need,
                                C.byref(wsb), C.byref(svb), C.byref(edges))
    if rc == E_CAPACITY:
        geo.edges()
        rc = lib.mccnn_conv_prepare(geo.handle, feats.data_ptr(), fin, fout, combin, bf16, backward, flags, C.byref(mask),
                                    need, C.byref(wsb), C.byref(svb), C.byref(edges))
    check(rc, "conv_prepare")
    if geo.e < 0:
        geo.e = edges.value
        _remember(geo.gkey, geo.m, geo.e)
    if mask.value:
        for k, bit in enumerate((NEED_PLAN_FWD, NEED_PLAN_TR, NEED_TLIST, NEED_RECORDS)):
            if mask.value & bit:
                t = torch.empty(max(int(need[k]), 256), dtype=torch.uint8, device=feats.device)
                check(lib.mccnn_geometry_attach(geo.handle, bit, t.data_ptr(), t.numel()), "geometry_attach")
                geo.attached.append(t)
    return wsb.value, svb.value


E_WORKSPACE = -4
_SIZES = {}


class _Conv(torch.autograd.Function):

    @staticmethod
    def forward(ctx, feats, w1, b1, w2, b2, w3, b3, geo, fout, combin, avg, deterministic):
        lib = _lib.load()
        fin = feats.shape[1]
        bf16 = 1 if feats.dtype == torch.bfloat16 else 0
        need_grad = feats.requires_grad or w1.requires_grad or w3.requires_grad or w2.requires_grad or b1.requires_grad \
            or b2.requires_grad or b3.requires_grad
        flags = (1 if need_grad else 0) | (2 if deterministic else 0)
        combin = 1 if combin else 0
        avg = 1 if avg else 0
        dev = feats.device
        out = torch.empty((geo.m, fout if combin else fin), dtype=feats.dtype, device=dev)
        skey = (flags & 1, fin, fout, combin, bf16, geo.n, geo.m)
        wsb, svb = _SIZES.get(skey, (0, -1))
        if svb < 0:
            wsb, svb = _prepare(geo, feats, fin, fout, combin, bf16, 0, flags)
# ... 90 lines not shown
```

Measured before the change: 173.1 million points/s.

## Share per-edge geometry records across Fin=1 conv forward/backward via geometry plan

Adds a per-geometry record piece of normalized offsets and inverse PDF weights that is built during geometry prebuild. The plan remembers that the previous step used records, and the Fin=1 forward kernels then read these precomputed float4 records instead of recomputing distances, radii and neighbour counts. Backward reuses the same records, so the per-call state shrinks. This takes per-edge arithmetic and gathers out of the forward kernel, at the cost of extra side-stream work in the geometry build and more complex buffer management.

```diff
diff --git a/include/mccnn.h b/include/mccnn.h
--- a/include/mccnn.h
+++ b/include/mccnn.h
@@ -259,6 +259,7 @@
 int mccnn_geometry_edges(mccnn_geometry_t* g, int wait_us);
 int mccnn_geometry_info(const mccnn_geometry_t* g, long long out[16]);
 int mccnn_geometry_attach(mccnn_geometry_t* g, int what, void* buffer, size_t bytes);
+int mccnn_geometry_records_used(const mccnn_geometry_t* g);
 int mccnn_geometry_piece_bytes(mccnn_geometry_t* g, int what, long long* bytes, long long* ws_bytes);
 int mccnn_geometry_piece_bound(int n, int m, int e_cap, int what, long long* bytes, long long* ws_bytes);
 int mccnn_geometry_prebuild(mccnn_geometry_t* g, int what, int avg, void* ws, size_t ws_bytes, mccnn_stream_t stream);
diff --git a/mccnn_amd/MCConvBuilder.py b/mccnn_amd/MCConvBuilder.py
--- a/mccnn_amd/MCConvBuilder.py
+++ b/mccnn_amd/MCConvBuilder.py
@@ -357,7 +357,7 @@
             plan = []
             for key, ent in self.geoSeen_.items():
                 geo = self.cacheGeo_.get(key)
-                plan.append(ent + ((geo.have & 7) if geo is not None else 0, key))
+                plan.append(ent + ((((geo.have & 7) | (8 if geo.records_used else 0)) if geo is not None else 0), key))
             state["geoPlan_"], state["geoSeen_"] = plan, {}
         state["cacheGeo_"], state["cacheGeoGrid_"] = {}, {}
         if self.prefetchedGeo_:
@@ -531,9 +531,13 @@
         owners = self.__dict__.setdefault("prefetchedGridOwner_", {})
         owner = owners.get(keyGrid)
         k = len(self.prefetchedGeo_)
+        if not pieces and _env.debug("plan_prefetch", True):
+            for ent in self.geoPlan_:
+                if ent[-1] == keyPDF:
+                    pieces = ent[7] & 8
         geo = _native.build_geometry(inPts, inBids, centres, cBids, mn, mx, B, nc, convRadius, relativeRadius, KDEWindow,
                                      usePDF, owner, side=k, fork=fork, background=True,
-                                     after=(inPH.prefetchFuture_ if inPH is outPH else None))
+                                     after=(inPH.prefetchFuture_ if inPH is outPH else None), records=bool(pieces & 8))
         geo.uses = 0
         if owner is None:
             owners[keyGrid] = geo
@@ -614,7 +618,8 @@
             nc = _hip_ops._num_cells(mn, mx, B, radius, rel)
             owner = self.cacheGeoGrid_.get(keyGrid)
             geo = _native.build_geometry(inPts, inBids, centres, cBids, mn, mx, B, nc, radius, rel, window, usePDF, owner,
-                                         side=k, fork=(k == 0), after=ph.prefetchFuture_)
+                                         side=k, fork=(k == 0), after=ph.prefetchFuture_,
+                                         records=bool(have & 8 and pieces))
             k += 1
             geo.uses = 0
             if have and pieces and geo.e_cap <= _PLAN_PREFETCH_MAX_E:
diff --git a/mccnn_amd/_lib.py b/mccnn_amd/_lib.py
--- a/mccnn_amd/_lib.py
+++ b/mccnn_amd/_lib.py
@@ -91,6 +91,7 @@
     "mccnn_geometry_edges": (_i, [_vp, _i]),
     "mccnn_geometry_info": (_i, [_vp, C.POINTER(C.c_longlong)]),
     "mccnn_geometry_attach": (_i, [_vp, _i, _vp, _sz]),
+    "mccnn_geometry_records_used": (_i, [_vp]),
     "mccnn_geometry_piece_bytes": (_i, [_vp, _i, C.POINTER(C.c_longlong), C.POINTER(C.c_longlong)]),
     "mccnn_geometry_piece_bound": (_i, [_i, _i, _i, _i, C.POINTER(C.c_longlong), C.POINTER(C.c_longlong)]),
     "mccnn_geometry_prebuild": (_i, [_vp, _i, _i, _vp, _sz, _vp]),
diff --git a/mccnn_amd/csrc/conv.hip b/mccnn_amd/csrc/conv.hip
--- a/mccnn_amd/csrc/conv.hip
+++ b/mccnn_amd/csrc/conv.hip
@@ -1061,6 +1061,11 @@
     return 0;
 }
 
+struct SharedRecords {
+    const float4* in;
+    float4* out;
+};
+
 extern "C" {
 
 int mccnn_debug_conv_impl(int mask) { return conv_impl_override().exchange(mask & 3); }
@@ -1118,7 +1123,7 @@
                          const float* w2, const float* b2, const float* w3, const float* b3, int n, int m, int e,
                          int num_in_feats, int num_out_feats, int combin, int batch_size, float radius,
                          int scale_inv, int avg, float* out, void* state, void* ws, size_t ws_bytes,
-                         mccnn_stream_t stream, int bf16) {
+                         mccnn_stream_t stream, int bf16, const SharedRecords* shared = nullptr) {
     ConvArgs a;
     int rc = fill_args(a, sorted_pts, sorted_feats, sorted_batch_ids, pdfs, samples, start_idx, packed, aabb_min,
                        aabb_max, w1, b1, w2, b2, w3, b3, n, m, e, num_in_feats, num_out_feats, combin, batch_size,
@@ -1130,8 +1135,12 @@
     bool vec = !combin && (a.Fin % 8 == 0) && ((((uintptr_t)sorted_feats) & 15) == 0);
     if (bf16 && !bf16_shape_ok(a, combin, sorted_feats, out)) return MCCNN_E_SHAPE;
     float4* recOut = state ? reinterpret_cast<float4*>(state) : nullptr;
-    if (e > 0 && f1_shape(num_in_feats, num_out_feats, combin))
-        return f1_forward(a, out, recOut, state ? (char*)state + state_record_bytes(e) : nullptr, ws, ws_bytes, s);
+    if (e > 0 && f1_shape(num_in_feats, num_out_feats, combin)) {
+        if (shared)
+            return f1_forward(a, out, shared->in ? nullptr : shared->out, shared->in, state, ws, ws_bytes, s);
+        return f1_forward(a, out, recOut, nullptr, state ? (char*)state + state_record_bytes(e) : nullptr, ws, ws_bytes, s);
+    }
+    if (shared) return MCCNN_E_SHAPE;
     if (use_mfma(a, combin != 0) && e > 0) {
         if (combin || a.nb <= MCCNN_TILE_FWD) return launch_conv_stream<false>(a, combin != 0, vec, bf16 != 0, out, nullptr, nullptr, s, recOut);
         int tiles, per;
@@ -1265,7 +1274,7 @@
                          int n, int m, int e, int num_in_feats, int num_out_feats, int combin, int batch_size,
                          float radius, int scale_inv, int avg, const void* state, const int* start_t,
                          const int* perm_t, float* feat_grad, float* dw1, float* db1, float* dw2, float* db2, float* dw3, float* db3,
-                         void* ws, size_t ws_bytes, mccnn_stream_t stream, int bf16) {
+                         void* ws, size_t ws_bytes, mccnn_stream_t stream, int bf16, const SharedRecords* shared = nullptr) {
     ConvArgs a;
     int rc = fill_args(a, sorted_pts, sorted_feats, sorted_batch_ids, pdfs, samples, start_idx, packed, aabb_min,
                        aabb_max, w1, b1, w2, b2, w3, b3, n, m, e, num_in_feats, num_out_feats, combin, batch_size,
@@ -1305,9 +1314,12 @@
     if (m == 0 || e == 0) return 0;
     if (!out_grad) return MCCNN_E_BADARG;
     const float4* recIn = state ? reinterpret_cast<const float4*>(state) : nullptr;
-    if (mfma && f1_shape(num_in_feats, num_out_feats, combin))
+    if (mfma && f1_shape(num_in_feats, num_out_feats, combin)) {
+        if (shared) return f1_backward(a, out_grad, shared->in, state, feat_grad, dw1, db1, dw2, db2, dw3, db3, ws, ws_bytes, s);
         return f1_backward(a, out_grad, recIn, state ? (const char*)state + state_record_bytes(e) : nullptr, feat_grad, dw1, db1,
                            dw2, db2, dw3, db3, ws, ws_bytes, s);
+    }
+    if (shared) return MCCNN_E_SHAPE;
     if (mfma) {
         if (!ws || ws_bytes < mccnn_spatial_conv_bwd_workspace_bytes(n, m, e, num_in_feats, num_out_feats, combin))
             return MCCNN_E_WORKSPACE;
@@ -1432,3 +1444,29 @@
 }
 
 }
+
+namespace mccnn {
+bool f1_shares_records(int num_in_feats, int num_out_feats, int combin) { return f1_shape(num_in_feats, num_out_feats, combin); }
+size_t f1_shared_state_bytes(int m, int num_out_feats) { return m > 0 ? f1_state_bytes(m, (num_out_feats + 7) / 8) : 0; }
+int f1_conv_fwd_shared(const float* sorted_pts, const float* sorted_feats, const int* sorted_batch_ids, const float* pdfs,
+                       const float* samples, const int* start_idx, const int* packed, const float* aabb_min, const float* aabb_max,
+                       const float* w1, const float* b1, const float* w2, const float* b2, const float* w3, const float* b3, int n,
+                       int m, int e, int num_out_feats, int batch_size, float radius, int scale_inv, int avg, float* out,
+                       const void* rec_in, void* rec_out, void* state, void* ws, size_t ws_bytes, mccnn_stream_t stream) {
+    const SharedRecords sh = {reinterpret_cast<const float4*>(rec_in), reinterpret_cast<float4*>(rec_out)};
+    return conv_fwd_impl(sorted_pts, sorted_feats, sorted_batch_ids, pdfs, samples, start_idx, packed, aabb_min, aabb_max, w1, b1,
+                         w2, b2, w3, b3, n, m, e, 1, num_out_feats, 1, batch_size, radius, scale_inv, avg, out, state, ws, ws_bytes,
+                         stream, 0, &sh);
+}
+int f1_conv_bwd_shared(const float* sorted_pts, const float* sorted_feats, const int* sorted_batch_ids, const float* pdfs,
+                       const float* samples, const int* start_idx, const int* packed, const float* aabb_min, const float* aabb_max,
+                       const float* w1, const float* b1, const float* w2, const float* b2, const float* w3, const float* b3,
+                       const float* out_grad, int n, int m, int e, int num_out_feats, int batch_size, float radius, int scale_inv,
+                       int avg, const void* rec_in, const void* state, float* feat_grad, float* dw1, float* db1, float* dw2,
+                       float* db2, float* dw3, float* db3, void* ws, size_t ws_bytes, mccnn_stream_t stream) {
+    const SharedRecords sh = {reinterpret_cast<const float4*>(rec_in), nullptr};
+    return conv_bwd_impl(sorted_pts, sorted_feats, sorted_batch_ids, pdfs, samples, start_idx, packed, aabb_min, aabb_max, w1, b1,
+                         w2, b2, w3, b3, out_grad, n, m, e, 1, num_out_feats, 1, batch_size, radius, scale_inv, avg, state, nullptr,
+                         nullptr, feat_grad, dw1, db1, dw2, db2, dw3, db3, ws, ws_bytes, stream, 0, &sh);
+}
+}
diff --git a/mccnn_amd/csrc/conv_f1.hip b/mccnn_amd/csrc/conv_f1.hip
--- a/mccnn_amd/csrc/conv_f1.hip
+++ b/mccnn_amd/csrc/conv_f1.hip
@@ -15,8 +15,9 @@
     return v;
 }
 
+template <bool REC>
 __global__ __launch_bounds__(256) void f1_fwd_edges(ConvArgs a, float* __restrict__ A, float* __restrict__ S,
-                                                    int numWaves, float4* __restrict__ recOut) {
+                                                    int numWaves, float4* __restrict__ recOut, const float4* __restrict__ recIn) {
     extern __shared__ float lds[];
     const int wave = threadIdx.x >> 6, lane = threadIdx.x & 63, i4 = lane & 3;
     const int rowA = a.nb * 8;
@@ -46,26 +47,42 @@
     float carryS = 0.f;
     int2 prN = make_int2(0, cA);
     float pdfN = 1.0f;
-    if (eBeg + lane < eEnd) { prN = a.packed[eBeg + lane]; pdfN = a.pdfs[eBeg + lane]; }
+    float4 rcN = make_float4(0.f, 0.f, 0.f, 0.f);
+    if (eBeg + lane < eEnd) {
+        prN = a.packed[eBeg + lane];
+        if (REC) rcN = recIn[eBeg + lane];
+        else pdfN = a.pdfs[eBeg + lane];
+    }
     for (int base = eBeg; base < eEnd; base += 64) {
         const int t = base + lane;
         const int nIn = min(64, eEnd - base);
         const bool in = lane < nIn;
         const int2 pr = prN;
         const float pdf = pdfN;
-        if (t + 64 < eEnd) { prN = a.packed[t + 64]; pdfN = a.pdfs[t + 64]; }
+        const float4 rc = rcN;
+        if (t + 64 < eEnd) {
+            prN = a.packed[t + 64];
+            if (REC) rcN = recIn[t + 64];
+            else pdfN = a.pdfs[t + 64];
+        }
         const int ci = pr.y, j = pr.x;
-        float invR = a.invRadius;
-        if (a.scaleInv) invR = 1.0f / (a.radius * max_extent(a.mn, a.mx, clamp_batch(a.bids[j], a.B)));
-        const float* pp = a.pts + (size_t)j * 3;
-        const float* cc = a.samples + (size_t)ci * 3;
-        const float R = a.scaleInv ? a.radius * max_extent(a.mn, a.mx, clamp_batch(a.bids[j], a.B)) : a.radius;
-        const float d0 = div_exact(pp[0] - cc[0], R, invR), d1 = div_exact(pp[1] - cc[1], R, invR), d2 = div_exact(pp[2] - cc[2], R, invR);
-        float K = 1.0f;
-        if (a.avg) K = (float)(((ci + 1 < a.m) ? a.start[ci + 1] : a.e) - a.start[ci]);
-        const float inv = in ? __builtin_amdgcn_rcpf(pdf * K) : 0.0f;
+        float d0, d1, d2, inv;
+        if (REC) {
+            d0 = rc.x; d1 = rc.y; d2 = rc.z;
+            inv = in ? rc.w : 0.0f;
+        } else {
+            float invR = a.invRadius;
+            if (a.scaleInv) invR = 1.0f / (a.radius * max_extent(a.mn, a.mx, clamp_batch(a.bids[j], a.B)));
+            const float* pp = a.pts + (size_t)j * 3;
+            const float* cc = a.samples + (size_t)ci * 3;
+            const float R = a.scaleInv ? a.radius * max_extent(a.mn, a.mx, clamp_batch(a.bids[j], a.B)) : a.radius;
+            d0 = div_exact(pp[0] - cc[0], R, invR); d1 = div_exact(pp[1] - cc[1], R, invR); d2 = div_exact(pp[2] - cc[2], R, invR);
+            float K = 1.0f;
+            if (a.avg) K = (float)(((ci + 1 < a.m) ? a.start[ci + 1] : a.e) - a.start[ci]);
+            inv = in ? __builtin_amdgcn_rcpf(pdf * K) : 0.0f;
+            if (recOut && in) recOut[t] = make_float4(d0, d1, d2, inv);
+        }
         const float s = in ? a.feats[j] * inv : 0.0f;
-        if (recOut && in) recOut[t] = make_float4(d0, d1, d2, inv);
         const int key = in ? ci + 1 : 0;
         const int cLast = __builtin_amdgcn_readlane(ci, nIn - 1);
         const int rowEnd = (cLast + 1 < a.m) ? a.start[cLast + 1] : a.e;
@@ -146,8 +163,9 @@
 #else
 #define X4_PHASE() MCCNN_PHASE()
 #endif
+template <bool REC>
 __global__ __launch_bounds__(256, MCCNN_F1_X4_OCC) void f1_fwd_edges4(ConvArgs a, float* __restrict__ A, float* __restrict__ S,
-                                                     int numWaves, float4* __restrict__ recOut) {
+                                                     int numWaves, float4* __restrict__ recOut, const float4* __restrict__ recIn) {
     extern __shared__ float lds[];
     const int wave = threadIdx.x >> 6, lane = threadIdx.x & 63, i4 = lane & 3;
     const int rowA = a.nb * 8;
@@ -178,11 +196,13 @@
     float carryS = 0.f;
     int2 prN[4];
     float pdfN[4];
+    float4 rcN[4];
 #pragma unroll
     for (int u = 0; u < 4; ++u) {
         const int t = min(eBeg + 4 * lane + u, a.e - 1);
         prN[u] = a.packed[t];
-        pdfN[u] = a.pdfs[t];
+        if (REC) rcN[u] = recIn[t];
+        else pdfN[u] = a.pdfs[t];
     }
     for (int base = eBeg; base < eEnd; base += 256) {
         const int lastPos = min(base + 256, eEnd) - 1;
@@ -194,27 +214,36 @@
             const int t = base + 4 * lane + u;
             in[u] = t < eEnd;
             const int2 pr = prN[u];
-            const float pdf = pdfN[u];
             const int j = pr.x;
             ci[u] = pr.y;
-            float invR = a.invRadius, R = a.radius;
-            if (a.scaleInv) {
-                R = a.radius * max_extent(a.mn, a.mx, clamp_batch(a.bids[j], a.B));
-                invR = 1.0f / R;
-            }
-            const float* pp = a.pts + (size_t)j * 3;
-            const float* cc = a.samples + (size_t)pr.y * 3;
-            d0[u] = div_exact(pp[0] - cc[0], R, invR);
-            d1[u] = div_exact(pp[1] - cc[1], R, invR);
-            d2[u] = div_exact(pp[2] - cc[2], R, invR);
-            float K = 1.0f;
-            if (a.avg) K = (float)(((pr.y + 1 < a.m) ? a.start[pr.y + 1] : a.e) - a.start[pr.y]);
-            const float inv = in[u] ? __builtin_amdgcn_rcpf(pdf * K) : 0.0f;
+            float inv;
+            if (REC) {
+                const float4 rc = rcN[u];
+                d0[u] = rc.x;
+                d1[u] = rc.y;
+                d2[u] = rc.z;
+                inv = in[u] ? rc.w : 0.0f;
+            } else {
+                const float pdf = pdfN[u];
+                float invR = a.invRadius, R = a.radius;
+                if (a.scaleInv) {
+                    R = a.radius * max_extent(a.mn, a.mx, clamp_batch(a.bids[j], a.B));
+                    invR = 1.0f / R;
+                }
+                const float* pp = a.pts + (size_t)j * 3;
+                const float* cc = a.samples + (size_t)pr.y * 3;
+                d0[u] = div_exact(pp[0] - cc[0], R, invR);
+                d1[u] = div_exact(pp[1] - cc[1], R, invR);
+                d2[u] = div_exact(pp[2] - cc[2], R, invR);
+                float K = 1.0f;
+                if (a.avg) K = (float)(((pr.y + 1 < a.m) ? a.start[pr.y + 1] : a.e) - a.start[pr.y]);
+                inv = in[u] ? __builtin_amdgcn_rcpf(pdf * K) : 0.0f;
+                if (recOut) recStage[4 * lane + u] = make_float4(d0[u], d1[u], d2[u], inv);
+            }
             sE[u] = in[u] ? a.feats[j] * inv : 0.0f;
-            if (recOut) recStage[4 * lane + u] = make_float4(d0[u], d1[u], d2[u], inv);
             key[u] = in[u] ? pr.y + 1 : 0;
         }
-        if (recOut) {
+        if (!REC && recOut) {
 #pragma unroll
             for (int k = 0; k < 4; ++k) {
                 const int t = base + 64 * k + lane;
@@ -226,7 +255,8 @@
             for (int u = 0; u < 4; ++u) {
                 const int t = min(base + 256 + 4 * lane + u, a.e - 1);
                 prN[u] = a.packed[t];
-                pdfN[u] = a.pdfs[t];
+                if (REC) rcN[u] = recIn[t];
+                else pdfN[u] = a.pdfs[t];
             }
         }
         const int lp = lastPos - base;
@@ -676,40 +706,44 @@
     S = (float*)((char*)state + align_up((size_t)m * nb * 8 * sizeof(float)));
 }
 
-static int f1_run_edges(const ConvArgs& a, float* A, float* S, float4* recOut, hipStream_t s) {
+static int f1_run_edges(const ConvArgs& a, float* A, float* S, float4* recOut, const float4* recIn, hipStream_t s) {
     const size_t lds = ((size_t)a.nb * MCCNN_WQ_FWD + 4 * (size_t)a.nb * 8) * sizeof(float);
+    typedef void (*Kern)(ConvArgs, float*, float*, int, float4*, const float4*);
     if (a.e >= g_f1_x4_min_edges.load(std::memory_order_relaxed)) {
-        const size_t lds4 = lds + 4 * 256 * sizeof(float4);
-        const int perCU4 = cached_blocks_per_cu(reinterpret_cast<const void*>(f1_fwd_edges4), lds4);
+        const Kern fn4 = recIn ? f1_fwd_edges4<true> : f1_fwd_edges4<false>;
+        const size_t lds4 = lds + (recIn ? 0 : 4 * 256 * sizeof(float4));
+        const int perCU4 = cached_blocks_per_cu(reinterpret_cast<const void*>(fn4), lds4);
         const long long iters = ((long long)a.e + 255) / 256;
         static const int wpc = debug_int("f1_x4_waves_per_cu", 0);
         long long W4 = (long long)num_cus() * (wpc > 0 ? wpc : perCU4 * 4);
         if (W4 > (iters + 1) / 2) W4 = (iters + 1) / 2;
         if (W4 < 1) W4 = 1;
-        f1_fwd_edges4<<<(int)((W4 + 3) / 4), 256, lds4, s>>>(a, A, S, (int)W4, recOut);
+        fn4<<<(int)((W4 + 3) / 4), 256, lds4, s>>>(a, A, S, (int)W4, recOut, recIn);
         MCCNN_LAUNCHED();
         return 0;
     }
-    const int perCU = cached_blocks_per_cu(reinterpret_cast<const void*>(f1_fwd_edges), lds);
+    const Kern fn = recIn ? f1_fwd_edges<true> : f1_fwd_edges<false>;
+    const int perCU = cached_blocks_per_cu(reinterpret_cast<const void*>(fn), lds);
     const long long chunks = ((long long)a.e + 63) / 64;
     long long W = (long long)num_cus() * perCU * 4;
     if (W > (chunks + 1) / 2) W = (chunks + 1) / 2;
     if (W < 1) W = 1;
-    f1_fwd_edges<<<(int)((W + 3) / 4), 256, lds, s>>>(a, A, S, (int)W, recOut);
+    fn<<<(int)((W + 3) / 4), 256, lds, s>>>(a, A, S, (int)W, recOut, recIn);
     MCCNN_LAUNCHED();
     return 0;
 }
 
 size_t f1_fwd_workspace_bytes(int m, int nb) { return f1_state_bytes(m, nb) + 256; }
 
-int f1_forward(const ConvArgs& a, float* out, float4* rec_out, void* state, void* ws, size_t ws_bytes, hipStream_t s) {
+int f1_forward(const ConvArgs& a, float* out, float4* rec_out, const float4* rec_in, void* state, void* ws, size_t ws_bytes,
+               hipStream_t s) {
     if (!state) {
         if (!ws || ws_bytes < f1_fwd_workspace_bytes(a.m, a.nb)) return MCCNN_E_WORKSPACE;
         state = ws;
     }
     float *A, *S;
     f1_state_split(state, a.m, a.nb, A, S);
-    int rc = f1_run_edges(a, A, S, rec_out, s);
+    int rc = f1_run_edges(a, A, S, rec_out, rec_in, s);
     if (rc) return rc;
     f1_fwd_centres<<<ceil_div((long long)a.m * a.nb, 256), 256, (size_t)a.nb * 72 * sizeof(float), s>>>(a, A, S, out);
     MCCNN_LAUNCHED();
@@ -749,7 +783,7 @@
         f1_state_split(const_cast<void*>(state), a.m, a.nb, A, S);
     } else {
         f1_state_split(own, a.m, a.nb, A, S);
-        int rc = f1_run_edges(a, A, S, nullptr, s);
+        int rc = f1_run_edges(a, A, S, nullptr, rec_in, s);
         if (rc) return rc;
     }
     f1_bwd_centres<<<ceil_div((long long)wavesC * (a.nb + 1), 4), 256, 0, s>>>(a, out_grad, A, S, cPerWave, wavesC, G, gb, pc, feat_grad);
diff --git a/mccnn_amd/csrc/conv_mfma.h b/mccnn_amd/csrc/conv_mfma.h
--- a/mccnn_amd/csrc/conv_mfma.h
+++ b/mccnn_amd/csrc/conv_mfma.h
@@ -385,7 +385,8 @@
 size_t f1_state_bytes(int m, int nb);
 size_t f1_fwd_workspace_bytes(int m, int nb);
 size_t f1_bwd_workspace_bytes(int m, int e, int nb);
-int f1_forward(const ConvArgs& a, float* out, float4* rec_out, void* state, void* ws, size_t ws_bytes, hipStream_t s);
+int f1_forward(const ConvArgs& a, float* out, float4* rec_out, const float4* rec_in, void* state, void* ws, size_t ws_bytes,
+               hipStream_t s);
 int f1_backward(const ConvArgs& a, const float* out_grad, const float4* rec_in, const void* state, float* feat_grad, float* dw1, float* db1,
                 float* dw2, float* db2, float* dw3, float* db3, void* ws, size_t ws_bytes, hipStream_t s);
 
diff --git a/mccnn_amd/csrc/exec.hip b/mccnn_amd/csrc/exec.hip
--- a/mccnn_amd/csrc/exec.hip
+++ b/mccnn_amd/csrc/exec.hip
@@ -29,6 +29,19 @@
                          const int* cell_indexs, const float* aabb_min, const float* aabb_max, int batch_size, int num_cells,
                          float radius, int scale_inv, const int* centre_order, int* start_idx, int e_capacity, int* packed,
                          int* total_dev, int* total_host, void* ws, size_t ws_bytes, mccnn_stream_t stream);
+bool f1_shares_records(int num_in_feats, int num_out_feats, int combin);
+size_t f1_shared_state_bytes(int m, int num_out_feats);
+int f1_conv_fwd_shared(const float* sorted_pts, const float* sorted_feats, const int* sorted_batch_ids, const float* pdfs,
+                       const float* samples, const int* start_idx, const int* packed, const float* aabb_min, const float* aabb_max,
+                       const float* w1, const float* b1, const float* w2, const float* b2, const float* w3, const float* b3, int n,
+                       int m, int e, int num_out_feats, int batch_size, float radius, int scale_inv, int avg, float* out,
+                       const void* rec_in, void* rec_out, void* state, void* ws, size_t ws_bytes, mccnn_stream_t stream);
+int f1_conv_bwd_shared(const float* sorted_pts, const float* sorted_feats, const int* sorted_batch_ids, const float* pdfs,
+                       const float* samples, const int* start_idx, const int* packed, const float* aabb_min, const float* aabb_max,
+                       const float* w1, const float* b1, const float* w2, const float* b2, const float* w3, const float* b3,
+                       const float* out_grad, int n, int m, int e, int num_out_feats, int batch_size, float radius, int scale_inv,
+                       int avg, const void* rec_in, const void* state, float* feat_grad, float* dw1, float* db1, float* dw2,
+                       float* db2, float* dw3, float* db3, void* ws, size_t ws_bytes, mccnn_stream_t stream);
 }
 
 using namespace mccnn;
@@ -78,6 +91,8 @@
     char* rec_buf = nullptr;
     size_t rec_bytes = 0;
     int rec_avg = -1;
+    bool f1_private = false;
+    bool rec_used = false;
 };
 
 namespace {
@@ -258,6 +273,22 @@
     if (tr) g->tl_built = true;
     p.built = true;
     p.avg = avg;
+    return 0;
+}
+
+bool f1_shared(const mccnn_geometry* g, const Shape& s, int e) {
+    return e > 0 && g->m > 0 && s.combin && s.fin == 1 && !s.bf16 && !g->f1_private && g->rec_buf && g->rec_bytes >= (size_t)e * 16 &&
+           f1_shares_records(s.fin, s.fout, s.combin);
+}
+
+int ensure_records(mccnn_geometry* g, int e, int avg, mccnn_stream_t stream) {
+    if (g->rec_avg == avg) return 0;
+    if (!g->rec_buf || g->rec_bytes < (size_t)e * 16) return MCCNN_E_WORKSPACE;
+    const mccnn_geometry* go = grid_owner(g);
+    int rc = mccnn_edge_records(go->s_pts, go->s_bids, g->pdfs, g->centres, g->start, g->packed, g->mn, g->mx, g->n, g->m, e, g->B,
+                                g->radius, g->scale_inv, avg, g->rec_buf, stream);
+    if (rc) return rc;
+    g->rec_avg = avg;
     return 0;
 }
 
@@ -512,6 +543,8 @@
     return 0;
 }
 
+int mccnn_geometry_records_used(const mccnn_geometry_t* g) { return (g && g->rec_used) ? 1 : 0; }
+
 int mccnn_geometry_attach(mccnn_geometry_t* g, int what, void* buffer, size_t bytes) {
     if (!g || !g->built || !buffer || (((uintptr_t)buffer) & 255)) return MCCNN_E_BADARG;
     switch (what) {
@@ -579,6 +612,7 @@
     if (what & NEED_PLAN_FWD) rc = ensure_plan(g, 0, e, avg, ws, ws_bytes, stream);
     if (!rc && (what & NEED_PLAN_TR)) rc = ensure_plan(g, 1, e, avg, ws, ws_bytes, stream);
     if (!rc && (what & NEED_TLIST)) rc = ensure_tlist(g, e, ws, ws_bytes, stream);
+    if (!rc && (what & NEED_RECORDS)) rc = ensure_records(g, e, avg, stream);
     return rc;
 }
 
@@ -783,6 +817,12 @@
         if (!rc && (w & NEED_TLIST)) rc = ensure_tlist(g, e, sws, al(single), stream);
         if (rc) return rc;
     }
+    for (int k = 0; k < count; ++k) {
+        mccnn_geometry_t* g = geoms[k];
+        if (!(what[k] & NEED_RECORDS) || g->e <= 0 || g->e > g->e_cap) continue;
+        rc = ensure_records(g, g->e, avg, stream);
+        if (rc) return rc;
+    }
     return 0;
 }
 
@@ -828,7 +868,7 @@
         } else if (!s.bf16) {
             const size_t w = mccnn_spatial_conv_fwd_workspace_bytes(m, e, s.fin, s.fout, s.combin);
             if (w > ws) ws = w;
-            if (flags & 1) saved += al(mccnn_spatial_conv_state_bytes(m, e, s.fin, s.fout, s.combin));
+            if (flags & 1) saved += f1_shared(g, s, e) ? al(f1_shared_state_bytes(m, s.fout)) : al(mccnn_spatial_conv_state_bytes(m, e, s.fin, s.fout, s.combin));
         }
     } else {
         const bool rows_bwd = f.rows_bwd && m > 0;
@@ -929,6 +969,24 @@
                                            b1, w2, b2, w3, b3, n, m, e, s.fin, g->B, g->radius, g->scale_inv, avg, out, ws, ws_bytes,
                                            stream);
     void* state = nullptr;
+    if (f1_shared(g, s, e)) {
+        if (flags & 1) {
+            if (!saved || saved_bytes < sv_off + f1_shared_state_bytes(m, s.fout)) return MCCNN_E_WORKSPACE;
+            state = sv + sv_off;
+        }
+        const bool ready = g->rec_avg == avg, fresh = g->rec_avg < 0;
+        int rc = f1_conv_fwd_shared(go->s_pts, (const float*)rows_in, go->s_bids, g->pdfs, g->centres, g->start, g->packed, g->mn,
+                                    g->mx, w1, b1, w2, b2, w3, b3, n, m, e, s.fout, g->B, g->radius, g->scale_inv, avg, (float*)out,
+                                    ready ? g->rec_buf : nullptr, fresh ? g->rec_buf : nullptr, state, ws, ws_bytes, stream);
+        if (rc) return rc;
+        if (fresh) g->rec_avg = avg;
+        g->rec_used = true;
+        return 0;
+    }
+    if (e > 0 && m > 0 && !s.bf16 && f1_shares_records(s.fin, s.fout, s.combin)) {
+        g->rec_used = true;
+        if (flags & 1) g->f1_private = true;
+    }
     if (flags & 1) {
         const size_t sb = mccnn_spatial_conv_state_bytes(m, e, s.fin, s.fout, s.combin);
         if (sb) {
@@ -1027,6 +1085,13 @@
         rc = mccnn_spatial_conv_bwd_bf16(go->s_pts, rows_in, go->s_bids, g->pdfs, g->centres, g->start, g->packed, g->mn, g->mx, w1,
                                          b1, w2, b2, w3, b3, out_grad, n, m, e, s.fin, g->B, g->radius, g->scale_inv, avg, st, pt,
                                          fg, dw1, db1, dw2, db2, dw3, db3, w, wb, stream);
+    } else if (f1_shared(g, s, e)) {
+        const void* state = nullptr;
+        if ((flags & 1) && saved && saved_bytes >= sv_off + f1_shared_state_bytes(m, s.fout) && !f.unsorted) state = sv + sv_off;
+        rc = f1_conv_bwd_shared(go->s_pts, (const float*)rows_in, go->s_bids, g->pdfs, g->centres, g->start, g->packed, g->mn, g->mx,
+                                w1, b1, w2, b2, w3, b3, (const float*)out_grad, n, m, e, s.fout, g->B, g->radius, g->scale_inv, avg,
+                                g->rec_avg == avg ? g->rec_buf : nullptr, state, (float*)fg, dw1, db1, dw2, db2, dw3, db3, w, wb,
+                                stream);
     } else {
         const void* state = nullptr;
         if (flags & 1) {
diff --git a/mccnn_amd/csrc/torch_ext.cpp b/mccnn_amd/csrc/torch_ext.cpp
--- a/mccnn_amd/csrc/torch_ext.cpp
+++ b/mccnn_amd/csrc/torch_ext.cpp
@@ -8,6 +8,7 @@
 #include <ATen/hip/impl/HIPStreamMasqueradingAsCUDA.h>
 #include <hip/hip_runtime_api.h>
 
+#include <array>
 #include <atomic>
 #include <chrono>
 #include <condition_variable>
@@ -370,11 +371,13 @@
     int pre_avg = -1;
     int have = 0;
     int plan_side = -1;
+    int64_t rec_tail_off = 0, rec_tail_len = 0;
+    bool records_used = false;
 
     int issue_pieces(int what, bool avg, hipStream_t ss, void* ws, size_t wsb) {
         int rc = 0;
-        if (what & 1) {
-            rc = mccnn_geometry_prebuild(h, 1, avg ? 1 : 0, ws, wsb, (void*)ss);
+        if (what & 9) {
+            rc = mccnn_geometry_prebuild(h, what & 9, avg ? 1 : 0, ws, wsb, (void*)ss);
             if (!rc) {
                 if (!plan_event) plan_event = take_event();
                 if (hipEventRecord(plan_event, ss) != hipSuccess) rc = (int)hipErrorUnknown;
@@ -465,9 +468,9 @@
 struct PieceEntry {
     std::shared_ptr<Geo> g;
     int what;
-    bool avg;
-    char* base;
-    long long off[4], len[4];
+    bool avg, rec_asked;
+    char* ptr[4];
+    long long len[4];
 };
 struct GeoBatch {
     bool active = false;
@@ -558,11 +561,11 @@
             if (E <= 0 || E > g.e_cap) continue;
             int rc = 0;
             for (int k = 0; k < 4 && !rc; ++k)
-                if (pe.what & (1 << k)) rc = mccnn_geometry_attach(g.h, 1 << k, pe.base + pe.off[k], (size_t)pe.len[k]);
+                if (pe.what & (1 << k)) rc = mccnn_geometry_attach(g.h, 1 << k, pe.ptr[k], (size_t)pe.len[k]);
             if (rc) continue;
             g.have |= pe.what;
             hs.push_back(g.h);
-            whats.push_back(pe.what & 7);
+            whats.push_back((pe.what & 7) | (pe.rec_asked ? 8 : 0));
             live.push_back(&pe);
             if (g.event) last = g.event;
         }
@@ -581,7 +584,7 @@
             if (rc) fprintf(stderr, "mccnn: batch of row plans / transposed lists: error %d (the layers build what is missing)\n", rc);
             for (PieceEntry* pe : live) {
                 Geo& g = *pe->g;
-                if (pe->what & 1) {
+                if ((pe->what & 1) || pe->rec_asked) {
                     if (!g.plan_event) g.plan_event = take_event();
                     if (hipEventRecord(g.plan_event, ss) == hipSuccess) g.plan_wait = true;
                 }
@@ -599,7 +602,7 @@
 std::shared_ptr<Geo> build_geometry(const Tensor& pts, const Tensor& bids, const Tensor& centres, const Tensor& cbids,
                                     const Tensor& mn, const Tensor& mx, int64_t B, int64_t nc, double radius, bool scale_inv,
                                     double window, bool use_pdf, int64_t capacity, std::shared_ptr<Geo> grid_from,
-                                    int64_t side, bool fork, bool background, std::shared_ptr<HierFuture> after) {
+                                    int64_t side, bool fork, bool background, std::shared_ptr<HierFuture> after, bool records) {
     check_dev(pts, at::kFloat, "points");
     check_dev(centres, at::kFloat, "sample points");
     check_dev(bids, at::kInt, "batch ids");
@@ -612,6 +615,14 @@
     const size_t bytes = mccnn_geometry_bytes(n, m, (int)B, (int)nc, (int)capacity, grid_from ? 0 : 1);
     TORCH_CHECK(bytes > 0, "geometry: batch_size * num_cells^3 does not fit 32-bit keys");
     auto g = std::make_shared<Geo>();
+    size_t total_bytes = bytes;
+    if (records && side >= 0 && capacity > 0) {
+        long long rb = 0, rw = 0;
+        check(mccnn_geometry_piece_bound(n, m, (int)capacity, 8, &rb, &rw), "geometry_piece_bound");
+        g->rec_tail_off = (int64_t)((bytes + 255) / 256 * 256);
+        g->rec_tail_len = rb;
+        total_bytes = (size_t)(g->rec_tail_off + rb);
+    }
     g->h = mccnn_geometry_create();
     TORCH_CHECK(g->h, "mccnn_geometry_create failed");
     g->slot = take_slot();
@@ -639,8 +650,8 @@
         if (fork) fork_skipped = true;
         {
             const c10::hip::HIPStreamGuardMasqueradingAsCUDA own(as_torch_stream((void*)ss, (int)pts.device().index()));
-            if (batched) g->buf = arena_take(0, (int64_t)bytes, pts);
-            if (!g->buf.defined()) g->buf = at::empty({(int64_t)bytes}, pts.options().dtype(at::kByte));
+            if (batched) g->buf = arena_take(0, (int64_t)total_bytes, pts);
+            if (!g->buf.defined()) g->buf = at::empty({(int64_t)total_bytes}, pts.options().dtype(at::kByte));
         }
         g->own_pool = true;
         g->caller_stream = stream;
@@ -655,7 +666,7 @@
         g->side = sk;
         stream = ss;
     } else if (side >= 0) {
-        g->buf = at::empty({(int64_t)bytes}, pts.options().dtype(at::kByte));
+        g->buf = at::empty({(int64_t)total_bytes}, pts.options().dtype(at::kByte));
         hipStream_t ss = side_stream((int)side);
         if (ss) {
             static thread_local hipEvent_t fork_ev = nullptr;
@@ -738,44 +749,53 @@
 void prebuild_async(std::shared_ptr<Geo> g, int what, bool avg) {
     if (!g || g->side < 0 || !Issuer::enabled() || g->e_cap <= 0) return;
     const DevGuard device_guard((int)g->buf.device().index());
+    const bool rec_asked = (what & 8) != 0 && !(g->have & 8);
     if (what & 3) what |= 8;
     if (what & 2) what |= 4;
     what &= 15 & ~g->have;
     if (!what) return;
     long long off[4] = {0, 0, 0, 0}, len[4] = {0, 0, 0, 0}, total = 0, wsb = 256;
+    const bool rec_in_buf = (what & 8) && g->rec_tail_len > 0;
     for (int k = 0; k < 4; ++k) {
         if (!(what & (1 << k))) continue;
         long long b = 0, w = 0;
         check(mccnn_geometry_piece_bound(g->n, g->m, (int)g->e_cap, 1 << k, &b, &w), "geometry_piece_bound");
+        if (w > wsb) wsb = w;
+        if (k == 3 && rec_in_buf && g->rec_tail_len >= b) { len[k] = g->rec_tail_len; off[k] = -1; continue; }
         off[k] = total;
         len[k] = b;
         total += (b + 255) / 256 * 256;
-        if (w > wsb) wsb = w;
     }
     const bool batched = t_geo_batch.active && t_geo_batch.side >= 0 && g->plan_side >= 0;
     if (batched) g->plan_side = (t_geo_batch.side + 1) % kSideStreams;
     const bool other = g->plan_side >= 0 && g->plan_side != g->side;
     hipStream_t ss = side_stream(other ? g->plan_side : g->side);
     Tensor block;
-    if (g->own_pool) {
-        const c10::hip::HIPStreamGuardMasqueradingAsCUDA own(as_torch_stream((void*)ss, (int)g->buf.device().index()));
-        if (batched) block = arena_take(1, (int64_t)total, g->buf);
-        if (!block.defined()) block = at::empty({(int64_t)total}, g->buf.options());
-    } else {
-        block = at::empty({(int64_t)total}, g->buf.options());
-    }
-    g->attached.push_back(block);
+    if (total > 0) {
+        if (g->own_pool) {
+            const c10::hip::HIPStreamGuardMasqueradingAsCUDA own(as_torch_stream((void*)ss, (int)g->buf.device().index()));
+            if (batched) block = arena_take(1, (int64_t)total, g->buf);
+            if (!block.defined()) block = at::empty({(int64_t)total}, g->buf.options());
+        } else {
+            block = at::empty({(int64_t)total}, g->buf.options());
+        }
+        g->attached.push_back(block);
+    }
     g->pieces_issued.store(0, std::memory_order_release);
-    char* base = (char*)block.data_ptr();
+    std::array<char*, 4> ptrs = {nullptr, nullptr, nullptr, nullptr};
+    for (int k = 0; k < 4; ++k) {
+        if (!(what & (1 << k))) continue;
+        ptrs[k] = off[k] < 0 ? (char*)g->buf.data_ptr() + g->rec_tail_off : (char*)block.data_ptr() + off[k];
+    }
     Tensor like = g->buf;
     if (batched) {
         PieceEntry pe;
-        pe.g = g; pe.what = what; pe.avg = avg; pe.base = base;
-        for (int k = 0; k < 4; ++k) { pe.off[k] = off[k]; pe.len[k] = len[k]; }
+        pe.g = g; pe.what = what; pe.avg = avg; pe.rec_asked = rec_asked;
+        for (int k = 0; k < 4; ++k) { pe.ptr[k] = ptrs[k]; pe.len[k] = len[k]; }
         t_geo_batch.pieces.push_back(std::move(pe));
         return;
     }
-    Issuer::get(2).push([g, what, avg, base, off, len, wsb, ss, like, other]() mutable {
+    Issuer::get(2).push([g, what, avg, rec_asked, ptrs, len, wsb, ss, like, other]() mutable {
         enter_device((int)like.device().index());
         g->wait_build_issued_nothrow();
         if (g->build_rc == 0 && other && g->event && hipStreamWaitEvent(ss, g->event, 0) != hipSuccess) g->build_rc = (int)hipErrorUnknown;
@@ -787,12 +807,12 @@
             if (E > 0 && E <= g->e_cap) {
                 int rc = 0;
                 for (int k = 0; k < 4 && !rc; ++k)
-                    if (what & (1 << k)) rc = mccnn_geometry_attach(g->h, 1 << k, base + off[k], (size_t)len[k]);
+                    if (what & (1 << k)) rc = mccnn_geometry_attach(g->h, 1 << k, ptrs[k], (size_t)len[k]);
                 if (!rc) {
                     g->have |= what;
                     try {
                         Tensor& ws = scratch((size_t)wsb, like, (void*)ss);
-                        rc = g->issue_pieces(what & 7, avg, ss, ws.data_ptr(), (size_t)ws.numel());
+                        rc = g->issue_pieces((what & 7) | (rec_asked ? 8 : 0), avg, ss, ws.data_ptr(), (size_t)ws.numel());
                     } catch (const std::exception&) {
                         rc = (int)hipErrorUnknown;
                     }
@@ -946,6 +966,7 @@
                                  b3.data_ptr<float>(), out.data_ptr(), saved.defined() ? saved.data_ptr() : nullptr,
                                  (size_t)svb, ws.data_ptr(), (size_t)ws.numel(), st),
               "conv_forward");
+        if (combin && L.fin == 1 && !geo->records_used) geo->records_used = mccnn_geometry_records_used(geo->h) != 0;
     }
     if (need_grad) {
         auto node = std::shared_ptr<ConvBackward>(new ConvBackward(), torch::autograd::deleteNode);
@@ -1383,6 +1404,7 @@
         .def_readwrite("uses", &Geo::uses)
         .def_readonly("side", &Geo::side)
         .def_readonly("have", &Geo::have)
+        .def_readonly("records_used", &Geo::records_used)
         .def("join", [](Geo& g, const at::Tensor& like) { g.join(cur_stream(like)); }, py::call_guard<py::gil_scoped_release>())
         .def("prebuild", &Geo::prebuild, py::arg("what"), py::arg("avg"), py::arg("side"), py::arg("like"),
              py::call_guard<py::gil_scoped_release>())
@@ -1392,7 +1414,7 @@
             py::arg("mn"), py::arg("mx"), py::arg("B"), py::arg("nc"), py::arg("radius"), py::arg("scale_inv"),
             py::arg("window"), py::arg("use_pdf"), py::arg("capacity"), py::arg("grid_from").none(true),
             py::arg("side") = -1, py::arg("fork") = false, py::arg("background") = false,
-            py::arg("after").none(true) = py::none(), py::call_guard<py::gil_scoped_release>());
+            py::arg("after").none(true) = py::none(), py::arg("records") = false, py::call_guard<py::gil_scoped_release>());
     mod.def("sampled_features", &sampled_features, py::call_guard<py::gil_scoped_release>());
     mod.def("begin_geometry_batch", &begin_geometry_batch);
     mod.def("end_geometry_batch", &end_geometry_batch, py::call_guard<py::gil_scoped_release>());
diff --git a/mccnn_amd/native.py b/mccnn_amd/native.py
--- a/mccnn_amd/native.py
+++ b/mccnn_amd/native.py
@@ -187,6 +187,12 @@
     def have(self):
         return int(self.core.have) if self.core is not None else 0
 
+    @property
+    def records_used(self):
+        if self.core is not None:
+            return bool(self.core.records_used)
+        return bool(self.handle is not None and _lib.load().mccnn_geometry_records_used(self.handle))
+
     def prebuild_async(self, what, avg):
         if self.core is not None:
             _EXT.prebuild_async(self.core, int(what), bool(avg))
@@ -231,13 +237,13 @@
 
 
 def _build_into(g, inPts, inBids, centres, cbids, mn, mx, B, nc, radius, scaleInv, window, usePDF, capacity, grid_from,
-                side=-1, fork=False, background=False, after=None):
+                side=-1, fork=False, background=False, after=None, records=False):
     n, m = inPts.shape[0], centres.shape[0]
     if _EXT is not None:
         uses = g.core.uses if g.core is not None else 0
         g.core = _EXT.build_geometry(inPts, inBids, centres, cbids, mn, mx, B, nc, float(radius), bool(scaleInv), float(window),
                                      bool(usePDF), capacity, grid_from.core if grid_from is not None else None, side, fork,
-                                     background, after)
+                                     background, after, bool(records))
         g.core.uses = uses
         g.buf = g.core.buf
         g.grid_owner = grid_from
@@ -283,7 +289,7 @@
 
 
 def build_geometry(inPts, inBids, centres, cbids, mn, mx, B, nc, radius, scaleInv, window, usePDF, grid_from=None,
-                   side=-1, fork=False, background=False, after=None):
+                   side=-1, fork=False, background=False, after=None, records=False):
     n, m = inPts.shape[0], centres.shape[0]
     gkey = (inPts.device.index, n, m, float(radius), int(B), bool(scaleInv))
     g = Geometry()
@@ -292,7 +298,7 @@
         grid_from = grid_from.grid_owner
     _build_into(g, inPts, inBids, centres, cbids, mn, mx, B, nc, radius, scaleInv, window, usePDF,
                 _capacity_guess(gkey, m), grid_from, side if _EXT is not None else -1, fork, background,
-                after if _EXT is not None else None)
+                after if _EXT is not None else None, records)
     return g
 
 
```

Result: slower. 125.4 million points/s (-27.6%).
